# IamArmanNikkhah/viewport-entropy-toolkit

Measured on AMD Instinct MI355X. Metric: viewport samples/sec, higher is better.
Workload: dtype f64 (u32 block-floating-point table weights, u64 fixed-point histogram); 1 GPU; config3: 1 video(s) x 1024 users x 30000 frames, tile_counts=[500], spatial, use_weight_distribution=True, fov=120, W=100, H=200; users=1024, frames=30000, mode=spatial, videos_per_gpu=1, batched_launch=False, parallelism=one video per GPU x1

## Files before the change

include/vet.h:

```cpp
#ifndef VET_H_
#define VET_H_

#include <stddef.h>
#include <stdint.h>

#ifdef __cplusplus
extern "C" {
#endif

#define VET_VERSION 141
#define VET_STREAM_LEGACY ((void *)1)
#define VET_TABLE_SAMPLES_PER_DIRECTION 2

enum {
    VET_OK = 0,
    VET_ERR_INVALID = -1,
    VET_ERR_DEVICE = -2,
    VET_ERR_RANGE = -3,
    VET_ERR_EMPTY = -4,
    VET_ERR_UNSUPPORTED = -5
};

typedef struct vet_ctx vet_ctx;
typedef struct vet_plan vet_plan;

int vet_version(void);
const char *vet_last_error(void);
int vet_device_count(void);
int vet_create(int device_id, vet_ctx **out);
int vet_destroy(vet_ctx *ctx);
int vet_synchronize(vet_ctx *ctx);
int vet_device_pci_bus_id(vet_ctx *ctx, char *buf, int len);
int vet_profile_enable(vet_ctx *ctx, int on);
int vet_test_no_row_cap(vet_ctx *ctx, int on);
int vet_profile_reset(vet_ctx *ctx);
int vet_profile_get(vet_ctx *ctx, int kernel_id, double *total_ms, int64_t *launches);
const char *vet_kernel_name(int kernel_id);

int vet_malloc(vet_ctx *ctx, size_t bytes, void **d_ptr);
int vet_free(vet_ctx *ctx, void *d_ptr);
int vet_memcpy_h2d(vet_ctx *ctx, void *d_dst, const void *h_src, size_t bytes);
int vet_memcpy_d2h(vet_ctx *ctx, void *h_dst, const void *d_src, size_t bytes);

typedef struct vet_plan_desc {
    int video_width, video_height;
    const double *h_lon_cos, *h_lon_sin;
    const double *h_lat_sin, *h_lat_cos;
    const double *h_dir_table;
    int64_t n_dirs;
    int n_lattices;
    const int *n_tiles;
    const double *const *h_tiles;
    const double *h_max_entropy;
    double fov_angle;
    double max_angular_distance;
    double power_factor;
    int use_weight_distribution;
    const uint16_t *const *h_bin_lut;
    const int *n_norm_tiles;
} vet_plan_desc;

int vet_plan_create(vet_ctx *ctx, const vet_plan_desc *desc, vet_plan **out);
int vet_plan_destroy(vet_plan *plan);
int64_t vet_plan_n_dirs(const vet_plan *plan);
int vet_plan_set_table_policy(vet_plan *plan, int policy);
int vet_plan_set_fp64(vet_plan *plan, int on);
int vet_plan_set_raw_weights(vet_plan *plan, int on);
int vet_plan_table_stride(const vet_plan *plan, int lattice);
int64_t vet_plan_table_rows(const vet_plan *plan);
int vet_plan_table_cap(const vet_plan *plan, int lattice, int64_t *overflow_rows);
int vet_plan_last_formulation(const vet_plan *plan, int lattice);
int vet_plan_error_bounds(vet_plan *plan, int lattice, double *table_bound, double *sweep_bound);
int vet_plan_read_dirs(vet_plan *plan, double *h_xyz );
int vet_plan_read_nearest(vet_plan *plan, int lattice, int32_t *h_nearest );
int vet_plan_read_table(vet_plan *plan, int lattice, uint32_t *h_w, uint16_t *h_tile, uint32_t *h_meta, uint32_t *h_ovf_w,
                        uint16_t *h_ovf_tile, uint32_t *h_ovf_of_row);

int vet_spatial_entropy(vet_plan *plan, const double *d_mu, const double *d_mv,
                        int n_users, int n_frames,
                        double *d_entropy, int32_t *d_assign, double *d_weights,
                        int32_t *d_present, int32_t *d_status, void *stream);
int vet_spatial_entropy_ids(vet_plan *plan, const int32_t *d_ids, int n_users, int n_frames,
                            double *d_entropy, int32_t *d_assign, double *d_weights,
                            int32_t *d_present, int32_t *d_status, void *stream);

int64_t vet_window_rows(int n_frames, int window, int stride);
int vet_spatial_entropy_windowed(vet_plan *plan, const double *d_mu, const double *d_mv, int n_users, int n_frames,
                                 int window, int stride, double *d_entropy, double *d_weights, int32_t *d_samples,
                                 int32_t *d_status, void *stream);
int vet_spatial_entropy_windowed_ids(vet_plan *plan, const int32_t *d_ids, int n_users, int n_frames, int window, int stride,
                                     double *d_entropy, double *d_weights, int32_t *d_samples, int32_t *d_status,
                                     void *stream);
int vet_spatial_entropy_windowed_host(vet_plan *plan, const double *h_mu, const double *h_mv, const int32_t *h_ids,
                                      int n_users, int n_frames, int window, int stride, double *h_entropy,
                                      double *h_weights, int32_t *h_samples);

int vet_transition_entropy(vet_plan *plan, const double *d_mu, const double *d_mv,
                           int n_users, int n_frames,
                           double *d_entropy, int32_t *d_pairs, int32_t *d_srccount,
                           int32_t *d_common, int32_t *d_status, void *stream);
int vet_transition_entropy_ids(vet_plan *plan, const int32_t *d_ids, int n_users, int n_frames,
                               double *d_entropy, int32_t *d_pairs, int32_t *d_srccount,
                               int32_t *d_common, int32_t *d_status, void *stream);

typedef struct vet_video {
    const double *d_mu, *d_mv;
    int n_users, n_frames;
    double *d_entropy;
    int32_t *d_assign;
    int32_t *d_present;
} vet_video;
int vet_spatial_entropy_batch(vet_plan *plan, int n_videos, const vet_video *videos, int32_t *d_status,
                              void *stream);
int vet_spatial_entropy_batch_host(vet_plan *plan, int n_videos, const int *n_users, const int *n_frames,
                                   const double *h_mu, const double *h_mv, double *h_entropy,
                                   int32_t *h_assign, int32_t *h_present);
int vet_transition_entropy_batch(vet_plan *plan, int n_videos, const vet_video *videos, int32_t *d_status,
                                 void *stream);
int vet_transition_entropy_batch_host(vet_plan *plan, int n_videos, const int *n_users, const int *n_frames,
                                      const double *h_mu, const double *h_mv, double *h_entropy,
                                      int32_t *h_pairs, int32_t *h_common);

int vet_spatial_entropy_host(vet_plan *plan, const double *h_mu, const double *h_mv,
                             const int32_t *h_ids, int n_users, int n_frames,
                             double *h_entropy, int32_t *h_assign, double *h_weights,
                             int32_t *h_present);
int vet_transition_entropy_host(vet_plan *plan, const double *h_mu, const double *h_mv,
                                const int32_t *h_ids, int n_users, int n_frames,
                                double *h_entropy, int32_t *h_pairs, int32_t *h_srccount,
                                int32_t *h_common);

typedef struct vet_result vet_result;
int vet_spatial_entropy_host_resident(vet_plan *plan, const double *h_mu, const double *h_mv,
                                      const int32_t *h_ids, int n_users, int n_frames,
                                      double *h_entropy, int32_t *h_present, vet_result **out);
int vet_transition_entropy_host_resident(vet_plan *plan, const double *h_mu, const double *h_mv,
                                         const int32_t *h_ids, int n_users, int n_frames,
                                         double *h_entropy, int32_t *h_common, vet_result **out);
int vet_result_fetch(vet_result *result, int which, int64_t row0, int64_t n_rows, void *h_dst);
int vet_result_free(vet_result *result);

int vet_angular_distances(vet_ctx *ctx, const double *h_vectors, int64_t n_vectors, const double *h_tiles, int n_tiles,
                          double *h_out);

int vet_fb_tile_boundaries(vet_ctx *ctx, const double *h_tiles, int n_tiles, int max_edges,
                           double *h_edges, int32_t *h_count);

typedef struct vet_heatmap vet_heatmap;
int vet_heatmap_create(vet_ctx *ctx, const double *h_tiles , int n_tiles, int width,
                       int height, int video_width, int video_height, int marker_radius, vet_heatmap **out);
int vet_heatmap_destroy(vet_heatmap *hm);
int vet_heatmap_read_map(vet_heatmap *hm, int32_t *h_map );
int vet_heatmap_render(vet_heatmap *hm, const double *d_weights , const int32_t *d_present ,
                       const double *d_mu, const double *d_mv ,
                       int n_users, int n_frames, uint8_t *d_rgb , void *stream);
int vet_heatmap_render_result(vet_heatmap *hm, vet_result *r, const int32_t *h_present ,
                              const double *h_mu, const double *h_mv , int n_users,
                              int64_t row0, int64_t n_rows, uint8_t *h_rgb);
int vet_heatmap_render_counts(vet_heatmap *hm, const int32_t *d_counts , const int32_t *d_present ,
                              const double *d_mu, const double *d_mv ,
                              int n_users, int n_frames, uint8_t *d_rgb , void *stream);
int vet_heatmap_render_transition_result(vet_heatmap *hm, vet_result *r, const int32_t *h_present ,
                                         const double *h_mu, const double *h_mv , int n_users,
                                         int64_t row0, int64_t n_rows, uint8_t *h_rgb);
int vet_heatmap_create_latlon(vet_ctx *ctx, int tile_width, int tile_height, int width, int height, int video_width,
                              int video_height, int marker_radius, vet_heatmap **out);
int vet_heatmap_render_binned(vet_heatmap *hm, vet_plan *plan, const double *d_mu, const double *d_mv ,
                              int n_users, int n_frames, int markers, uint8_t *d_rgb , void *stream);
int vet_heatmap_render_binned_host(vet_heatmap *hm, vet_plan *plan, const double *h_mu, const double *h_mv ,
                                   int n_users, int n_frames, int markers, uint8_t *h_rgb );

typedef struct vet_tiling vet_tiling;
int vet_tiling_create(vet_ctx *ctx, const double *h_arcs , int n_arcs,
                      const double *h_centres , int n_centres, int width, int height,
                      vet_tiling **out);
int vet_tiling_destroy(vet_tiling *tl);
int vet_tiling_render(vet_tiling *tl, const double *h_cameras, int n_frames, const uint8_t *background, uint8_t *d_rgb,
                      void *stream);
int vet_tiling_render_host(vet_tiling *tl, const double *h_cameras, int n_frames, const uint8_t *background,
                           uint8_t *h_rgb);

#define VET_CSV_OK 0
#define VET_CSV_FALLBACK 1
#define VET_CSV_IO 2
typedef struct vet_track {
    double *time, *mu, *mv;
    int64_t n_rows;
    int status;
} vet_track;
int vet_csv_read_tracks(int n_files, const char *const *paths, vet_track *tracks, int n_threads);
void vet_csv_free_tracks(int n_files, vet_track *tracks);

#ifdef __cplusplus
}
#endif
#endif
```

viewport-entropy-toolkit_amd/csrc/vet_context.hip:

```cpp
#include "vet_host.hpp"
#include "vet_finalize.hpp"

#include <cstdarg>
#include <cstdio>
#include <cstdlib>
#include <cstring>

namespace vh {

namespace {
thread_local std::string g_err;
const char* const kKernelNames[KID_COUNT] = {"k_grid_dirs", "k_nearest_lut", "k_spatial", "k_transition",
                                             "k_finalize", "k_wtab", "k_weights"};

int env_flag(const char* name) { return getenv(name) ? 1 : 0; }
}

int fail(int code, const char* fmt, ...) {
    char buf[512];
    va_list ap;
    va_start(ap, fmt);
    vsnprintf(buf, sizeof buf, fmt, ap);
    va_end(ap);
    g_err = buf;
// ... 33 lines not shown
    HIP_TRY(hipMalloc(&c->ws, want));
    c->ws_bytes = want;
    return VET_OK;
}

int pooled(vet_ctx* c, int slot, size_t bytes, void** out) {
    if (bytes == 0) bytes = 8;
    if (c->pool_cap[slot] < bytes) {
        if (c->pool[slot]) {
            HIP_TRY(hipDeviceSynchronize());
            HIP_TRY(hipFree(c->pool[slot]));
        }
        c->pool[slot] = nullptr; c->pool_cap[slot] = 0;
        const size_t want = bytes + bytes / 8;
        HIP_TRY(hipMalloc(&c->pool[slot], want));
        c->pool_cap[slot] = want;
    }
    *out = c->pool[slot];
    return VET_OK;
}

int BatchBlob::acquire(vet_ctx* ctx, size_t nbytes) {
    c = ctx; bytes = nbytes ? nbytes : 8;
    BatchStage& t = c->stage[c->stage_next];
    c->stage_next = (c->stage_next + 1) % kBatchStages;
    if (t.pending) {
        HIP_TRY(hipEventSynchronize(t.done));
        t.pending = false;
    }
    if (!t.done) HIP_TRY(hipEventCreateWithFlags(&t.done, hipEventDisableTiming));
    if (t.cap < bytes) {
        if (t.h) { HIP_TRY(hipHostFree(t.h)); t.h = nullptr; }
        if (t.d) { HIP_TRY(hipFree(t.d)); t.d = nullptr; }
        t.cap = 0;
        const size_t want = bytes + bytes / 8;
        HIP_TRY(hipHostMalloc(&t.h, want, hipHostMallocDefault));
        HIP_TRY(hipMalloc(&t.d, want));
        t.cap = want;
    }
    st = &t;
    return VET_OK;
}

int BatchBlob::upload(hipStream_t stream) {
    s = stream;
    uploaded = true;
    HIP_TRY(hipMemcpyAsync(st->d, st->h, bytes, hipMemcpyHostToDevice, s));
    return VET_OK;
}

BatchBlob::~BatchBlob() {
    if (st && uploaded && hipEventRecord(st->done, s) == hipSuccess) st->pending = true;
}

int grid_for(long work, int block, int n_cu) {
    long b = (work + block - 1) / block;
    long cap = (long)n_cu * 8;
    if (b > cap) b = cap;
    if (b < 1) b = 1;
    return (int)b;
}

int check_run_args(const vet_plan* pl, int U, int T, const void* out) {
    if (!pl) return fail(VET_ERR_INVALID, "plan is NULL");
    if (U <= 0 || T <= 0) return fail(VET_ERR_INVALID, "n_users and n_frames must be positive (got %d, %d)", U, T);
    if (!out) return fail(VET_ERR_INVALID, "entropy output pointer is NULL");
    return VET_OK;
}

}

using namespace vh;

extern "C" {

int vet_version(void) { return VET_VERSION; }
const char* vet_last_error(void) { return vh::last_error(); }
const char* vet_kernel_name(int kid) { return (kid >= 0 && kid < KID_COUNT) ? kKernelNames[kid] : ""; }

int vet_device_count(void) {
    int n = 0;
    if (hipGetDeviceCount(&n) != hipSuccess) return 0;
    return n;
}

int vet_create(int device_id, vet_ctx** out) {
    if (!out) return fail(VET_ERR_INVALID, "out is NULL");
    int n = 0;
    hipError_t e = hipGetDeviceCount(&n);
    if (e != hipSuccess || n <= 0)
        return fail(VET_ERR_DEVICE, "no HIP device available (%s); this library has no CPU path",
                    e == hipSuccess ? "0 devices" : hipGetErrorString(e));
    if (device_id < 0 || device_id >= n) return fail(VET_ERR_INVALID, "device_id %d out of range [0,%d)", device_id, n);
    HIP_TRY(hipSetDevice(device_id));
    hipDeviceProp_t prop;
    HIP_TRY(hipGetDeviceProperties(&prop, device_id));
    vet_ctx* c = new vet_ctx();
    c->device = device_id;
    c->tune.from_environment();
    c->n_cu = prop.multiProcessorCount > 0 ? prop.multiProcessorCount : 256;
    c->lds_max = prop.sharedMemPerBlock >= 160 * 1024 ? 80 * 1024 : (size_t)prop.sharedMemPerBlock;
    e = hipStreamCreateWithFlags(&c->stream, hipStreamNonBlocking);
    if (e == hipSuccess) e = hipMalloc((void**)&c->d_log2, 4097 * sizeof(double));
    if (e == hipSuccess) {
        hipLaunchKernelGGL(vet::k_log2_table, dim3(17), dim3(256), 0, c->stream, c->d_log2, 4097);
        e = hipStreamSynchronize(c->stream);
    }
    if (e != hipSuccess) {
        if (c->d_log2) (void)hipFree(c->d_log2);
        if (c->stream) (void)hipStreamDestroy(c->stream);
        delete c;
        return fail(VET_ERR_DEVICE, "context set-up failed: %s", hipGetErrorString(e));
    }
    *out = c;
    return VET_OK;
}

int vet_device_pci_bus_id(vet_ctx* c, char* buf, int len) {
    if (!c || !buf || len < 16) return fail(VET_ERR_INVALID, "ctx or buf is NULL, or len < 16");
    HIP_TRY(hipDeviceGetPCIBusId(buf, len, c->device));
    return VET_OK;
}

int vet_destroy(vet_ctx* c) {
    if (!c) return VET_OK;
    (void)hipSetDevice(c->device);
    (void)hipStreamSynchronize(c->stream);
    for (auto& ep : c->pending) { (void)hipEventDestroy(ep.a); (void)hipEventDestroy(ep.b); }
    for (auto e : c->free_events) (void)hipEventDestroy(e);
    if (c->ws) (void)hipFree(c->ws);
    if (c->d_log2) (void)hipFree(c->d_log2);
    for (void* q : c->pool) if (q) (void)hipFree(q);
    for (auto& t : c->stage) {
        if (t.h) (void)hipHostFree(t.h);
        if (t.d) (void)hipFree(t.d);
        if (t.done) (void)hipEventDestroy(t.done);
    }
    (void)hipStreamDestroy(c->stream);
    delete c;
    return VET_OK;
}

int vet_synchronize(vet_ctx* c) {
    if (!c) return fail(VET_ERR_INVALID, "ctx is NULL");
    HIP_TRY(hipStreamSynchronize(c->stream));
    return VET_OK;
}

int vet_test_no_row_cap(vet_ctx* c, int on) {
    if (!c) return fail(VET_ERR_INVALID, "ctx is NULL");
    c->tune.no_row_cap = on != 0;
    return VET_OK;
}
int vet_profile_enable(vet_ctx* c, int on) {
    if (!c) return fail(VET_ERR_INVALID, "ctx is NULL");
    c->profiling = on != 0;
    return VET_OK;
}
int vet_profile_reset(vet_ctx* c) {
    if (!c) return fail(VET_ERR_INVALID, "ctx is NULL");
    int rc = collect_profile(c);
    if (rc) return rc;
    for (int i = 0; i < KID_COUNT; ++i) { c->prof_ms[i] = 0; c->prof_n[i] = 0; }
    return VET_OK;
}
int vet_profile_get(vet_ctx* c, int kid, double* total_ms, int64_t* launches) {
    if (!c || kid < 0 || kid >= KID_COUNT) return fail(VET_ERR_INVALID, "bad ctx or kernel id");
    int rc = collect_profile(c);
    if (rc) return rc;
    if (total_ms) *total_ms = c->prof_ms[kid];
    if (launches) *launches = c->prof_n[kid];
    return VET_OK;
}

int vet_malloc(vet_ctx* c, size_t bytes, void** d_ptr) {
    if (!c || !d_ptr) return fail(VET_ERR_INVALID, "ctx or d_ptr is NULL");
    HIP_TRY(hipSetDevice(c->device));
    HIP_TRY(hipMalloc(d_ptr, bytes ? bytes : 8));
    return VET_OK;
}
int vet_free(vet_ctx* c, void* d_ptr) {
    if (!c) return fail(VET_ERR_INVALID, "ctx is NULL");
    if (d_ptr) HIP_TRY(hipFree(d_ptr));
    return VET_OK;
}
int vet_memcpy_h2d(vet_ctx* c, void* d, const void* h, size_t bytes) {
    if (!c) return fail(VET_ERR_INVALID, "ctx is NULL");
    HIP_TRY(hipMemcpyAsync(d, h, bytes, hipMemcpyHostToDevice, c->stream));
    HIP_TRY(hipStreamSynchronize(c->stream));
    return VET_OK;
}
int vet_memcpy_d2h(vet_ctx* c, void* h, const void* d, size_t bytes) {
    if (!c) return fail(VET_ERR_INVALID, "ctx is NULL");
    HIP_TRY(hipMemcpyAsync(h, d, bytes, hipMemcpyDeviceToHost, c->stream));
    HIP_TRY(hipStreamSynchronize(c->stream));
    return VET_OK;
}

}
```

viewport-entropy-toolkit_amd/csrc/vet_host.hpp:

```cpp
#pragma once
#include "../../include/vet.h"
#include "vet_layout.hpp"

#include <hip/hip_runtime.h>

#include <cstdint>
#include <memory>
#include <string>
#include <vector>

namespace vh {

int fail(int code, const char* fmt, ...);
const char* last_error();

#define HIP_TRY(expr)                                                                             \
    do {                                                                                          \
        hipError_t e_ = (expr);                                                                   \
        if (e_ != hipSuccess)                                                                     \
            return vh::fail(VET_ERR_DEVICE, "%s failed: %s (%s:%d)", #expr, hipGetErrorString(e_), \
                            __FILE__, __LINE__);                                                  \
    } while (0)

struct DevBuf {
    void* p = nullptr;
    ~DevBuf() { if (p) (void)hipFree(p); }
    hipError_t alloc(size_t b) { return hipMalloc(&p, b ? b : 8); }
};

enum { KID_GRID = 0, KID_NEAREST = 1, KID_SPATIAL = 2, KID_TRANSITION = 3, KID_FINALIZE = 4, KID_WTAB = 5, KID_WEIGHTS = 6, KID_COUNT = 7 };

struct EventPair {
    int kid;
    hipEvent_t a, b;
};

struct WeightsCore {
    int device = 0;
    size_t lds_max = 64 * 1024;
    int n_cu = 256;
    std::shared_ptr<void> dir_unit;
    std::shared_ptr<void> tiles0;
    int n0 = 0;
    int64_t n_dirs = 0;
    double cos_cull = 0.0, max_ang = 0.0, power = 2.0;
    struct Exact {
        int state = 0;
        int stride = 0, n_rows = 0;
        std::shared_ptr<void> alias;
        std::shared_ptr<void> idx;
        std::shared_ptr<void> w;
        std::shared_ptr<void> len;
    } ex;
};

struct BatchStage {
    void* h = nullptr;
    void* d = nullptr;
    size_t cap = 0;
    hipEvent_t done = nullptr;
    bool pending = false;
};
constexpr int kBatchStages = 4;

struct Tuning {
    int no_fused = 0;
    int fused_single = 0;
    int t_global = 0;
    std::string lut_timeline;
    int no_exact_rows = 0;
    int no_row_cap = 0;
    void from_environment();
};

}

struct vet_ctx {
    int device = 0;
    hipStream_t stream = nullptr;
    int n_cu = 256;
    size_t lds_max = 64 * 1024;
    vh::Tuning tune;
    void* ws = nullptr;
    size_t ws_bytes = 0;
    double* d_log2 = nullptr;
    bool attrs_set = false;
    void* pool[12] = {};
    size_t pool_cap[12] = {};
    vh::BatchStage stage[vh::kBatchStages];
    int stage_next = 0;
    bool profiling = false;
    std::vector<vh::EventPair> pending;
    std::vector<hipEvent_t> free_events;
    double prof_ms[vh::KID_COUNT] = {};
    int64_t prof_n[vh::KID_COUNT] = {};
};

namespace vh {

struct Lattice {
    int n = 0;
    double* d_tiles = nullptr;
    std::vector<double> h_unit;
    uint16_t* d_nearest = nullptr;
    double hmax = 0.0;
    uint32_t* d_tab_w = nullptr;
    uint16_t* d_tab_i = nullptr;
    uint32_t* d_tab_meta = nullptr;
    uint8_t* d_row_s = nullptr;
    uint16_t* d_row_e = nullptr;
    bool fp_table = false;
    bool stats_done = false;
    double crit_tab = 0.0;
    double crit_base = 0.0;
    long ultra = 0;
    int markers = 0;
    int last_form = -1;
    int stride = 0;
    bool capped = false;
    int n_ovf = 0;
    uint32_t* d_ovf_w = nullptr;
    uint16_t* d_ovf_i = nullptr;
    uint32_t* d_ovf_of_row = nullptr;
    int gs_log2 = 4;
    bool interleaved = false;
    bool binned = false;
    int norm_n = 0;
    WeightsCore::Exact ex;
};

}

struct vet_plan {
    vet_ctx* ctx = nullptr;
    int W = 0, H = 0;
    bool grid = false;
    int64_t n_dirs = 0;
    double* d_dir_raw = nullptr;
    double* d_dir_unit = nullptr;
    std::vector<vh::Lattice> lat;
    double fov = 120.0, max_ang = 0.0, power = 2.0;
    int weighted = 1;
    double cos_cull = 0.0;
    int table_policy = 0;
    bool raw_weights = false;
    uint32_t* d_alias = nullptr;
    bool mirror = false;
    uint2* d_dirrec = nullptr;
    int n_rows = 0;
    int* d_canon = nullptr;
    struct Fused {
        int state = 0;
        int R = 0, stride = 0, gs_log2 = 4;
        bool interleaved = false;
        vet::FusedLayout lay;
        uint32_t* d_meta = nullptr;
        uint2* d_dirrec = nullptr;
        uint8_t* d_row_s = nullptr;
        uint32_t* d_w = nullptr;
        uint16_t* d_i = nullptr;
    } fused;
    std::shared_ptr<vh::WeightsCore> wcore;
    bool stats_all = false;
    bool ultra = false;
    bool fp64 = false;
    size_t exact_bytes = 0;
};

namespace vh {

struct ProfScope {
    vet_ctx* c;
    hipStream_t s;
    int kid;
    hipEvent_t a = nullptr, b = nullptr;
    ProfScope(vet_ctx* c_, hipStream_t s_, int kid_) : c(c_), s(s_), kid(kid_) {
        if (!c->profiling) return;
        auto get = [&]() {
            hipEvent_t e = nullptr;
            if (!c->free_events.empty()) { e = c->free_events.back(); c->free_events.pop_back(); }
            else (void)hipEventCreate(&e);
            return e;
        };
        a = get(); b = get();
        (void)hipEventRecord(a, s);
    }
    ~ProfScope() {
        if (!a) return;
        (void)hipEventRecord(b, s);
        c->pending.push_back({kid, a, b});
    }
};

struct BatchBlob {
    vet_ctx* c = nullptr;
    BatchStage* st = nullptr;
    hipStream_t s = nullptr;
    size_t bytes = 0;
    bool uploaded = false;
    int acquire(vet_ctx* ctx, size_t nbytes);
    void* host() const { return st->h; }
    void* dev() const { return st->d; }
    int upload(hipStream_t stream);
    ~BatchBlob();
};

int ensure_ws(vet_ctx* c, size_t bytes);
int pooled(vet_ctx* c, int slot, size_t bytes, void** out);
int grid_for(long work, int block, int n_cu);
int check_run_args(const vet_plan* pl, int U, int T, const void* out);

constexpr size_t kMaxTableBytes = (size_t)24 << 30;
constexpr double kContractMargin = 1e-7;
constexpr size_t kWholeLds = 160 * 1024 - 512;

int ensure_alias(vet_plan* pl);
int ensure_all_stats(vet_plan* pl, hipStream_t s);
int ensure_wtab(vet_plan* pl, int k, hipStream_t s);
int ensure_fused(vet_plan* pl, hipStream_t s);
bool any_binned(const vet_plan* pl);

int weights_pass_ids(const WeightsCore& w, const int32_t* d_ids, int U, int T, double* d_weights, hipStream_t s, vet_ctx* prof);
int ensure_exact_weights(vet_plan* pl, hipStream_t s);
int ensure_exact_rows(vet_plan* pl, int k, hipStream_t s);
const WeightsCore::Exact& exact_rows(const vet_plan* pl, int k);
int exact_frame_rows(vet_plan* pl, int k, const double* d_mu, const double* d_mv, const int32_t* d_ids, int U, int T, double* out,
                     hipStream_t s);
int sample_ids(const vet_plan* pl, const double* d_mu, const double* d_mv, long n, int32_t* d_out, hipStream_t s);

struct HeatmapGeom {
    const uint16_t* d_map = nullptr;
    int n = 0, W = 0, H = 0;
    int VW = 0, VH = 0, radius = 0;
};
int heatmap_map(vet_ctx* c, const double* d_unit_tiles, int n, int W, int H, uint16_t* d_map, hipStream_t s);
template <typename Wt>
int heatmap_render(vet_ctx* c, const HeatmapGeom& g, const Wt* d_weights, const int32_t* d_present, const double* d_mu,
                   const double* d_mv, int U, int T, uint32_t* d_pal, uint8_t* d_rgb, hipStream_t s);
struct BinLayout {
    bool ok = false, pack = false;
    int words = 0, FPW = 0;
    size_t lds = 0;
};
BinLayout heatmap_bin_layout(int n, int U);
int heatmap_map_latlon(vet_ctx* c, int tile_width, int tile_height, int W, int H, uint16_t* d_map, hipStream_t s);
int heatmap_bin_chunk(int n);
int heatmap_render_binned(vet_ctx* c, const HeatmapGeom& g, int n_lat, const uint16_t* d_lut, const double* d_mu,
                          const double* d_mv, int U, int T, bool markers, uint32_t* d_pal, uint8_t* d_rgb, hipStream_t s);

struct TilingCam {
    double F[3], r[3], u[3], nd[3];
    double s;
    double X0, Y0;
};
struct TilingGeom {
    const double* d_pts = nullptr;
    const double* d_centres = nullptr;
    long n_arcs = 0, n_centres = 0;
    int W = 0, H = 0;
    uint32_t colour[6] = {};
};
int tiling_chords(vet_ctx* c, const double* d_arcs, long n_arcs, double* d_pts, hipStream_t s);
int tiling_render(vet_ctx* c, const TilingGeom& g, const TilingCam* d_cam, int T, uint32_t* d_flags, uint8_t* d_rgb,
                  hipStream_t s);

int spatial_set_attrs(vet_ctx* c);
int transition_set_attrs(vet_ctx* c);
int window_set_attrs(vet_ctx* c);

}
```

viewport-entropy-toolkit_amd/csrc/vet_layout.hpp:

```cpp
#pragma once
#include <hip/hip_runtime.h>
#include <stdint.h>

namespace vet {

constexpr int WAVE = 64;
constexpr int MAX_LATTICES = 8;

constexpr int TAB_X = 16;
constexpr uint32_t MARKER_BITS = 0x80000000u;
constexpr int ROW_BITS = 19;
constexpr uint32_t ROW_MASK = (1u << ROW_BITS) - 1;
constexpr unsigned DEDUP_MAX_DIRS = (1u << ROW_BITS) - 1;
constexpr int DEDUP_MIN_USERS = 128;

constexpr int ROW_BLOCK = 64;
constexpr int MAX_CAP_BLOCKS = 3;
constexpr uint32_t META_OVERFLOW = 1u << 15;
constexpr uint32_t NO_OVERFLOW = 0xFFFFFFFFu;
__host__ __device__ __forceinline__ int lut_ovf_slots(int UC, int n_ovf, bool dedup) {
    if (n_ovf <= 0) return 0;
    const int most = dedup ? (2 * n_ovf > DEDUP_MIN_USERS ? 2 * n_ovf : DEDUP_MIN_USERS) : UC;
    return most < UC ? most : UC;
}

struct FusedLayout {
    int K;
    int n[MAX_LATTICES];
    int off[MAX_LATTICES];
    int Hs, N;
    int CF;
    double hmax[MAX_LATTICES];
};
__host__ __device__ __forceinline__ int fused_pos(const FusedLayout& L, int k, int i) {
    const int h = L.n[k] >> 1;
    if (i < h) return L.off[k] + i;
    if (i >= L.n[k] - h) return L.N - 1 - (L.off[k] + (L.n[k] - 1 - i));
    return 2 * L.K + L.Hs + k;
}

}
```

viewport-entropy-toolkit_amd/csrc/vet_plan.hip:

```cpp
#include "vet_host.hpp"
#include "vet_plan_kernels.hpp"
#include "vet_weight_table.hpp"
#include "vet_geometry.hpp"

#include <algorithm>
#include <array>
#include <cmath>
#include <cstring>
#include <limits>

namespace vh {

int ensure_alias(vet_plan* pl) {
    if (pl->d_alias) return VET_OK;
    vet_ctx* c = pl->ctx;
    const long D = (long)pl->n_dirs;
    if (D <= 0 || D >= (long)0x7FFFFFFF) return fail(VET_ERR_UNSUPPORTED, "direction table of %ld entries", D);
    bool mirror = pl->weighted;
    for (const auto& L : pl->lat) {
        if (L.binned || L.h_unit.empty()) { mirror = false; break; }
        for (int i = 0; i < L.n && mirror; ++i) {
            const double* a = &L.h_unit[3 * (size_t)i];
            const double* b = &L.h_unit[3 * (size_t)(L.n - 1 - i)];
            mirror = a[0] == b[0] && a[1] == -b[1] && a[2] == -b[2];
// ... 61 lines not shown
        (void)hipFree(d_crit);
        return fail(VET_ERR_DEVICE, "hipMalloc of the row shift table failed");
    }
    hipError_t e = hipMemsetAsync(d_crit, 0, 24, s);
    vet::StatsParams p{};
    p.dir_unit = pl->d_dir_unit; p.D = (long)pl->n_dirs;
    p.tiles = L.d_tiles; p.n = L.n;
    p.cos_cull = pl->cos_cull;
    p.wc.max_ang = pl->max_ang; p.wc.inv_max = 1.0 / pl->max_ang; p.wc.power = pl->power; p.wc.shift = 0;
    p.row_s = L.d_row_s; p.row_e = L.d_row_e; p.crit = d_crit;
    const int blocks = grid_for((long)pl->n_dirs * vet::WAVE, 256, c->n_cu * 2);
    {
        ProfScope ps(c, s, KID_WTAB);
        hipLaunchKernelGGL(vet::k_row_stats, dim3(blocks), dim3(256), 0, s, p);
    }
    unsigned long long bits[3] = {0, 0, 0};
    if (e == hipSuccess) e = hipMemcpyAsync(bits, d_crit, 24, hipMemcpyDeviceToHost, s);
    if (e == hipSuccess) e = hipStreamSynchronize(s);
    (void)hipFree(d_crit);
    if (e != hipSuccess) return fail(VET_ERR_DEVICE, "k_row_stats failed: %s", hipGetErrorString(e));
    memcpy(&L.crit_tab, &bits[0], 8);
    memcpy(&L.crit_base, &bits[1], 8);
    L.ultra = (long)bits[2];
    L.stats_done = true;
    return VET_OK;
}

int ensure_all_stats(vet_plan* pl, hipStream_t s) {
    if (pl->stats_all) return VET_OK;
    bool ultra = false;
    for (int k = 0; k < (int)pl->lat.size(); ++k) {
        if (!pl->weighted || pl->lat[k].binned) continue;
        int rc = ensure_stats(pl, k, s);
        if (rc) return rc;
        ultra = ultra || pl->lat[k].ultra > 0;
    }
    pl->ultra = ultra;
    pl->stats_all = true;
    return VET_OK;
}

int ensure_wtab(vet_plan* pl, int k, hipStream_t s) {
    Lattice& L = pl->lat[k];
    if (L.stride != 0) return VET_OK;
    vet_ctx* c = pl->ctx;
    int rc = ensure_all_stats(pl, s);
    if (rc) return rc;
    rc = ensure_alias(pl);
    if (rc) return rc;
    int* d_max = nullptr;
    HIP_TRY(hipMalloc((void**)&d_max, 2 * sizeof(int)));
    struct FreeMax { int* p; ~FreeMax() { (void)hipFree(p); } } free_max{d_max};
    hipError_t e = hipMemsetAsync(d_max, 0, 2 * sizeof(int), s);
    vet::WtabParams p{};
    const long R = pl->n_rows;
    p.dir_unit = pl->d_dir_unit; p.D = R;
    p.canon = pl->d_canon; p.shift_by_dir = 1; p.nl = 0;
    p.tiles = L.d_tiles; p.n = L.n;
    p.cos_cull = pl->cos_cull;
    p.wc.max_ang = pl->max_ang; p.wc.inv_max = 1.0 / pl->max_ang; p.wc.power = pl->power; p.wc.shift = 0;
    L.fp_table = pl->ultra || !(L.crit_tab <= kContractMargin);
    p.stride = 0; p.w = nullptr; p.idx = nullptr; p.meta = nullptr; p.row_s = L.d_row_s; p.row_e = L.d_row_e; p.fp = L.fp_table ? 1 : 0;
    p.maxcount = d_max; p.markers = nullptr; p.gs_log2 = -1;
    const int blocks = grid_for(R * vet::WAVE, 256, c->n_cu * 2);
    {
        ProfScope ps(c, s, KID_WTAB);
        hipLaunchKernelGGL(vet::k_wtab<false>, dim3(blocks), dim3(256), 0, s, p);
    }
    int longest = 0;
    if (e == hipSuccess) e = hipMemcpyAsync(&longest, d_max, sizeof(int), hipMemcpyDeviceToHost, s);
    if (e == hipSuccess) e = hipStreamSynchronize(s);
    if (e != hipSuccess) return fail(VET_ERR_DEVICE, "k_wtab<count> failed: %s", hipGetErrorString(e));
    int stride = ((longest > 0 ? longest : 1) + 63) / 64 * 64;
    const size_t rows = (size_t)R + 1;
    int cap = stride, n_ovf = 0;
    std::vector<uint32_t> ovf_of_row;
    if (!L.fp_table && pl->lat.size() == 1 && stride > vet::ROW_BLOCK && 4 * longest >= 3 * 64 && !c->tune.no_row_cap) {
        DevBuf d_len;
        HIP_TRY(d_len.alloc((size_t)R * sizeof(int)));
        p.row_len = (int*)d_len.p; p.gs_log2 = -1;
        {
            ProfScope ps(c, s, KID_WTAB);
            hipLaunchKernelGGL(vet::k_wtab<true>, dim3(blocks), dim3(256), 0, s, p);
        }
        std::vector<int> len((size_t)R);
        HIP_TRY(hipMemcpyAsync(len.data(), d_len.p, (size_t)R * sizeof(int), hipMemcpyDeviceToHost, s));
        HIP_TRY(hipStreamSynchronize(s));
        p.row_len = nullptr;
        int shortest = stride, most = 0;
        for (int v : len) { shortest = std::min(shortest, v); most = std::max(most, v); }
        for (int cnd = vet::ROW_BLOCK; cnd < stride && cnd <= vet::MAX_CAP_BLOCKS * vet::ROW_BLOCK; cnd += vet::ROW_BLOCK) {
            long longer = 0;
            for (int v : len) longer += v > cnd ? 1 : 0;
            if (longer * 32 > R) continue;
            if (shortest > cnd - vet::ROW_BLOCK && most <= cnd + vet::ROW_BLOCK) {
                cap = cnd;
                ovf_of_row.assign((size_t)R, vet::NO_OVERFLOW);
                for (long r = 0; r < R; ++r)
                    if (len[(size_t)r] > cap) ovf_of_row[(size_t)r] = (uint32_t)n_ovf++;
            }
            break;
        }
    }
    const bool capped = cap < stride;
    stride = cap;
    const size_t ovf_rows = capped ? (size_t)n_ovf + 1 : 0;
    const size_t bytes = rows * stride * 6 + rows * 4 + ovf_rows * vet::ROW_BLOCK * 6 + (capped ? (size_t)R * 4 : 0);
    size_t free_b = 0, total_b = 0;
    if (hipMemGetInfo(&free_b, &total_b) != hipSuccess) free_b = kMaxTableBytes;
    if (stride > 65535 || bytes > kMaxTableBytes || rows * (size_t)stride >= ((size_t)1 << 32) || bytes + ((size_t)64 << 20) > free_b) { L.stride = -1; return VET_OK; }
    auto drop = [&]() {
        if (L.d_tab_w) { (void)hipFree(L.d_tab_w); L.d_tab_w = nullptr; }
        if (L.d_tab_i) { (void)hipFree(L.d_tab_i); L.d_tab_i = nullptr; }
        if (L.d_tab_meta) { (void)hipFree(L.d_tab_meta); L.d_tab_meta = nullptr; }
        if (L.d_ovf_w) { (void)hipFree(L.d_ovf_w); L.d_ovf_w = nullptr; }
        if (L.d_ovf_i) { (void)hipFree(L.d_ovf_i); L.d_ovf_i = nullptr; }
        if (L.d_ovf_of_row) { (void)hipFree(L.d_ovf_of_row); L.d_ovf_of_row = nullptr; }
    };
    drop();
    if (hipMalloc((void**)&L.d_tab_w, rows * stride * 4) != hipSuccess ||
        hipMalloc((void**)&L.d_tab_i, rows * stride * 2) != hipSuccess ||
        hipMalloc((void**)&L.d_tab_meta, rows * 4) != hipSuccess ||
        (capped && (hipMalloc((void**)&L.d_ovf_w, ovf_rows * vet::ROW_BLOCK * 4) != hipSuccess ||
                    hipMalloc((void**)&L.d_ovf_i, ovf_rows * vet::ROW_BLOCK * 2) != hipSuccess ||
                    hipMalloc((void**)&L.d_ovf_of_row, (size_t)R * 4) != hipSuccess))) {
        (void)hipGetLastError();
        drop();
        L.stride = -1;
        return VET_OK;
    }
    struct DropOnError { decltype(drop)& d; bool armed = true; ~DropOnError() { if (armed) d(); } } guard{drop};
    L.gs_log2 = 1;
    while (L.gs_log2 < 4 && (4 << L.gs_log2) < longest) ++L.gs_log2;
    L.interleaved = L.gs_log2 == 4 && stride % 64 == 0 && 4 * longest >= 3 * 64;
    if (capped) {
        HIP_TRY(hipMemcpyAsync(L.d_ovf_of_row, ovf_of_row.data(), (size_t)R * 4, hipMemcpyHostToDevice, s));
        p.cap = cap; p.ovf_of_row = L.d_ovf_of_row; p.ow = L.d_ovf_w; p.oi = L.d_ovf_i; p.n_ovf = n_ovf;
    }
    p.stride = stride; p.w = L.d_tab_w; p.idx = L.d_tab_i; p.meta = L.d_tab_meta; p.maxcount = nullptr;
    p.markers = L.fp_table ? d_max + 1 : nullptr;
    p.gs_log2 = L.interleaved ? L.gs_log2 : -1;
    {
        ProfScope ps(c, s, KID_WTAB);
        hipLaunchKernelGGL(vet::k_wtab<true>, dim3(blocks), dim3(256), 0, s, p);
    }
    HIP_TRY(hipGetLastError());
    if (k == 0 && (uint64_t)pl->n_rows <= vet::DEDUP_MAX_DIRS) {
        if (!pl->d_dirrec) HIP_TRY(hipMalloc((void**)&pl->d_dirrec, (size_t)pl->n_dirs * sizeof(uint2)));
        ProfScope ps(c, s, KID_WTAB);
        hipLaunchKernelGGL(vet::k_dirrec, dim3(grid_for(pl->n_dirs, 256, c->n_cu)), dim3(256), 0, s, pl->d_alias,
                           L.d_nearest, L.d_tab_meta, (long)pl->n_dirs, pl->d_dirrec);
        HIP_TRY(hipGetLastError());
    }
    int markers = 0;
    HIP_TRY(hipMemcpyAsync(&markers, d_max + 1, sizeof(int), hipMemcpyDeviceToHost, s));
    HIP_TRY(hipStreamSynchronize(s));
    guard.armed = false;
    L.markers = markers;
    L.capped = capped; L.n_ovf = capped ? n_ovf : 0;
    L.stride = stride;
    return VET_OK;
}

int ensure_exact_rows(vet_plan* pl, int k, hipStream_t s) {
    WeightsCore::Exact& X = k == 0 ? pl->wcore->ex : pl->lat[k].ex;
    if (X.state != 0) return VET_OK;
    vet_ctx* c = pl->ctx;
    const Lattice& L = pl->lat[k];
    if (!pl->weighted || L.binned || !L.d_tiles || c->tune.no_exact_rows) { X.state = -1; return VET_OK; }
    int rc = ensure_alias(pl);
    if (rc) return rc;
    const long R = pl->n_rows;
    if (R <= 0) { X.state = -1; return VET_OK; }
    DevBuf d_max;
    HIP_TRY(d_max.alloc(sizeof(int)));
    HIP_TRY(hipMemsetAsync(d_max.p, 0, sizeof(int), s));
    vet::WtabParams p{};
    p.dir_unit = pl->d_dir_unit; p.D = R;
    p.canon = pl->d_canon; p.shift_by_dir = 1; p.nl = 0;
    p.tiles = L.d_tiles; p.n = L.n;
    p.cos_cull = pl->cos_cull;
    p.wc.max_ang = pl->max_ang; p.wc.inv_max = 1.0 / pl->max_ang; p.wc.power = pl->power; p.wc.shift = 0;
    p.maxcount = (int*)d_max.p; p.gs_log2 = -1;
    const int blocks = grid_for(R * vet::WAVE, 256, c->n_cu * 2);
    hipLaunchKernelGGL(vet::k_wtab<false>, dim3(blocks), dim3(256), 0, s, p);
    HIP_TRY(hipGetLastError());
    int longest = 0;
    HIP_TRY(hipMemcpyAsync(&longest, d_max.p, sizeof(int), hipMemcpyDeviceToHost, s));
    HIP_TRY(hipStreamSynchronize(s));
    const int stride = ((longest > 0 ? longest : 1) + 63) / 64 * 64;
    const size_t D = k == 0 ? (size_t)pl->n_dirs : 0, entries = (size_t)R * stride, bytes = entries * 10 + (size_t)R * 4 + D * 4;
    size_t free_b = 0, total_b = 0;
    if (hipMemGetInfo(&free_b, &total_b) != hipSuccess) free_b = 0;
    const size_t total = pl->exact_bytes + bytes;
    if (total > ((size_t)8 << 30) || total > (free_b + pl->exact_bytes) / 4 || stride > 65535) { X.state = -1; return VET_OK; }
    auto dev_free = [](void* q) { if (q) (void)hipFree(q); };
    auto dev_alloc = [&](size_t b) {
        void* q = nullptr;
        if (hipMalloc(&q, b ? b : 8) != hipSuccess) { (void)hipGetLastError(); q = nullptr; }
        return std::shared_ptr<void>(q, dev_free);
    };
    auto alias = k == 0 ? dev_alloc(D * 4) : std::shared_ptr<void>();
    auto idx = dev_alloc(entries * 2), w = dev_alloc(entries * 8), len = dev_alloc((size_t)R * 4);
    if ((k == 0 && !alias) || !idx || !w || !len) { X.state = -1; return VET_OK; }
    if (k == 0) HIP_TRY(hipMemcpyAsync(alias.get(), pl->d_alias, D * 4, hipMemcpyDeviceToDevice, s));
    vet::WexactParams q{};
    q.dir_unit = pl->d_dir_unit; q.canon = pl->d_canon; q.R = R; q.tiles = L.d_tiles; q.n = L.n;
    q.cos_cull = pl->cos_cull; q.wc = p.wc; q.stride = stride;
    q.idx = (uint16_t*)idx.get(); q.w = (double*)w.get(); q.len = (uint32_t*)len.get();
    {
        ProfScope ps(c, s, KID_WTAB);
        hipLaunchKernelGGL(vet::k_wexact, dim3(blocks), dim3(256), 0, s, q);
    }
    HIP_TRY(hipGetLastError());
    HIP_TRY(hipStreamSynchronize(s));
    X.alias = alias; X.idx = idx; X.w = w; X.len = len;
    X.stride = stride; X.n_rows = (int)R;
    X.state = 1;
    pl->exact_bytes = total;
    return VET_OK;
}

int ensure_exact_weights(vet_plan* pl, hipStream_t s) { return ensure_exact_rows(pl, 0, s); }

const WeightsCore::Exact& exact_rows(const vet_plan* pl, int k) { return k == 0 ? pl->wcore->ex : pl->lat[k].ex; }

bool any_binned(const vet_plan* pl) {
    for (const auto& L : pl->lat) if (L.binned) return true;
    return false;
}

int ensure_fused(vet_plan* pl, hipStream_t s) {
    auto& F = pl->fused;
    if (F.state != 0) return VET_OK;
    vet_ctx* c = pl->ctx;
    const int K = (int)pl->lat.size();
    auto unusable = [&]() { F.state = -1; return VET_OK; };
    if (K == 1 && !c->tune.fused_single) return unusable();
    if (!pl->weighted || K > vet::MAX_LATTICES || any_binned(pl) || c->tune.no_fused) return unusable();
    if ((uint64_t)pl->n_dirs > vet::DEDUP_MAX_DIRS) return unusable();
    int rc = ensure_all_stats(pl, s);
    if (rc) return rc;
    if (pl->ultra) return unusable();
    for (const auto& L : pl->lat)
        if (!(L.crit_tab <= kContractMargin) || !L.d_row_s) return unusable();
    rc = ensure_alias(pl);
    if (rc) return rc;
    const size_t D = (size_t)pl->n_dirs;
    const int R = pl->n_rows;
    if (R == 0) return unusable();
    vet::FusedLayout& lay = F.lay;
    lay.K = K; lay.Hs = 0; lay.CF = 0;
    for (int k = 0; k < K; ++k) {
        lay.n[k] = pl->lat[k].n; lay.off[k] = 2 * K + lay.Hs; lay.Hs += pl->lat[k].n >> 1; lay.hmax[k] = pl->lat[k].hmax;
        lay.CF += (pl->lat[k].n + vet::WAVE - 1) / vet::WAVE;
    }
    lay.N = 2 * (lay.Hs + K) + 4 * K;
    if (lay.N > 65535 || lay.N < 32) return unusable();

    auto drop = [&]() {
        for (void** q : {(void**)&F.d_row_s, (void**)&F.d_w, (void**)&F.d_i, (void**)&F.d_meta, (void**)&F.d_dirrec})
            if (*q) { (void)hipFree(*q); *q = nullptr; }
    };
    struct DropOnExit { decltype(drop)& d; bool armed = true; ~DropOnExit() { if (armed) d(); } } guard{drop};
    DevBuf ptrs_d, delta_d, max_d;
    HIP_TRY(ptrs_d.alloc(sizeof(void*) * vet::MAX_LATTICES));
    HIP_TRY(delta_d.alloc(sizeof(int) * vet::MAX_LATTICES));
    HIP_TRY(max_d.alloc(sizeof(int)));
    HIP_TRY(hipMalloc((void**)&F.d_row_s, (size_t)R + 1));
    const uint8_t* ptrs[vet::MAX_LATTICES] = {};
    for (int k = 0; k < K; ++k) ptrs[k] = pl->lat[k].d_row_s;
    HIP_TRY(hipMemcpyAsync(ptrs_d.p, ptrs, sizeof(ptrs), hipMemcpyHostToDevice, s));
    HIP_TRY(hipMemsetAsync(delta_d.p, 0, sizeof(int) * vet::MAX_LATTICES, s));
    HIP_TRY(hipMemsetAsync(max_d.p, 0, sizeof(int), s));
    HIP_TRY(hipMemsetAsync(F.d_row_s + R, vet::TAB_X, 1, s));
    hipLaunchKernelGGL(vet::k_fuse_shifts, dim3(grid_for(R, 256, c->n_cu)), dim3(256), 0, s, (const int*)pl->d_canon, R, K,
                       (const uint8_t* const*)ptrs_d.p, F.d_row_s, (int*)delta_d.p);
    vet::WtabParams p{};
    p.dir_unit = pl->d_dir_unit; p.D = R;
    p.tiles = nullptr; p.n = 0;
    p.cos_cull = pl->cos_cull;
    p.wc.max_ang = pl->max_ang; p.wc.inv_max = 1.0 / pl->max_ang; p.wc.power = pl->power; p.wc.shift = 0;
    p.stride = 0; p.w = nullptr; p.idx = nullptr; p.meta = nullptr; p.row_s = F.d_row_s; p.row_e = nullptr; p.fp = 0;
    p.markers = nullptr; p.maxcount = (int*)max_d.p; p.gs_log2 = -1;
    p.canon = pl->d_canon; p.shift_by_dir = 0; p.nl = K; p.Hs = lay.Hs; p.N = lay.N;
    for (int k = 0; k < 8; ++k) { p.tiles_v[k] = k < K ? pl->lat[k].d_tiles : nullptr; p.n_v[k] = k < K ? lay.n[k] : 0; p.off_v[k] = k < K ? lay.off[k] : 0; }
    const int blocks = grid_for((long)R * vet::WAVE, 256, c->n_cu * 2);
    {
        ProfScope ps(c, s, KID_WTAB);
        hipLaunchKernelGGL(vet::k_wtab<false>, dim3(blocks), dim3(256), 0, s, p);
    }
    int longest = 0, delta[vet::MAX_LATTICES] = {};
    HIP_TRY(hipMemcpyAsync(&longest, max_d.p, sizeof(int), hipMemcpyDeviceToHost, s));
    HIP_TRY(hipMemcpyAsync(delta, delta_d.p, sizeof(delta), hipMemcpyDeviceToHost, s));
    HIP_TRY(hipStreamSynchronize(s));
    for (int k = 0; k < K; ++k) {
        if (delta[k] == 0) continue;
        DevBuf crit;
        HIP_TRY(crit.alloc(24));
        HIP_TRY(hipMemsetAsync(crit.p, 0, 24, s));
        vet::StatsParams sp{};
        sp.dir_unit = pl->d_dir_unit; sp.D = R;
        sp.tiles = pl->lat[k].d_tiles; sp.n = pl->lat[k].n;
        sp.cos_cull = pl->cos_cull;
        sp.wc.max_ang = pl->max_ang; sp.wc.inv_max = 1.0 / pl->max_ang; sp.wc.power = pl->power; sp.wc.shift = 0;
        sp.row_s = nullptr; sp.row_e = nullptr; sp.crit = (unsigned long long*)crit.p;
        sp.canon = pl->d_canon; sp.shift_in = F.d_row_s;
        hipLaunchKernelGGL(vet::k_row_stats, dim3(grid_for((long)R * vet::WAVE, 256, c->n_cu * 2)), dim3(256), 0, s, sp);
        unsigned long long bits = 0;
// ... 45 lines not shown

extern "C" {

int vet_plan_create(vet_ctx* c, const vet_plan_desc* d, vet_plan** out) {
    if (!c || !d || !out) return fail(VET_ERR_INVALID, "ctx, desc or out is NULL");
    const bool grid = d->h_lon_cos && d->h_lon_sin && d->h_lat_sin && d->h_lat_cos;
    if (!grid && !(d->h_dir_table && d->n_dirs > 0))
        return fail(VET_ERR_INVALID, "plan needs the four axis tables or an explicit direction table");
    if (grid && (d->video_width <= 0 || d->video_height <= 0))
        return fail(VET_ERR_INVALID, "Video dimensions must be positive");
    if (d->n_lattices <= 0 || !d->n_tiles || !d->h_tiles || !d->h_max_entropy)
        return fail(VET_ERR_INVALID, "Must specify at least one tile count");
    if (!(d->fov_angle > 0.0 && d->fov_angle <= 360.0))
        return fail(VET_ERR_INVALID, "FOV angle must be between 0 and 360 degrees");
    if (!(d->power_factor > 0.0)) return fail(VET_ERR_INVALID, "Power factor must be positive");
    for (int k = 0; k < d->n_lattices; ++k) {
        const bool binned = d->h_bin_lut && d->h_bin_lut[k];
        if (d->n_tiles[k] <= 0 || d->n_tiles[k] > 65535 || (!binned && !d->h_tiles[k]))
            return fail(VET_ERR_INVALID, "lattice %d: tile count %d outside [1, 65535]", k, d->n_tiles[k]);
    }
    HIP_TRY(hipSetDevice(c->device));
    hipStream_t s = c->stream;
    vet_plan* pl = new vet_plan();
    pl->ctx = c;
    pl->grid = grid;
    pl->W = d->video_width; pl->H = d->video_height;
    pl->fov = d->fov_angle; pl->max_ang = d->max_angular_distance; pl->power = d->power_factor;
    pl->weighted = d->use_weight_distribution ? 1 : 0;
    pl->cos_cull = pl->max_ang >= 3.14159 ? -2.0 : std::cos(pl->max_ang) - 1e-9;
    pl->n_dirs = grid ? (int64_t)(pl->W + 1) * (pl->H + 1) : d->n_dirs;
    if (pl->n_dirs >= (1LL << 31)) { delete pl; return fail(VET_ERR_UNSUPPORTED, "direction table too large"); }

    auto cleanup = [&](int rc) { vet_plan_destroy(pl); return rc; };
#define PLAN_TRY(expr)                                                                           \
    do {                                                                                         \
        hipError_t e_ = (expr);                                                                  \
        if (e_ != hipSuccess)                                                                    \
            return cleanup(fail(VET_ERR_DEVICE, "%s failed: %s", #expr, hipGetErrorString(e_))); \
    } while (0)

    PLAN_TRY(hipMalloc((void**)&pl->d_dir_raw, (size_t)pl->n_dirs * 3 * sizeof(double)));
    PLAN_TRY(hipMalloc((void**)&pl->d_dir_unit, (size_t)pl->n_dirs * 3 * sizeof(double)));
    if (grid) {
        const size_t nw = (size_t)pl->W + 1, nh = (size_t)pl->H + 1;
        double* d_axes = nullptr;
        PLAN_TRY(hipMalloc((void**)&d_axes, (2 * nw + 2 * nh) * sizeof(double)));
        hipError_t e1 = hipMemcpyAsync(d_axes, d->h_lon_cos, nw * 8, hipMemcpyHostToDevice, s);
        hipError_t e2 = hipMemcpyAsync(d_axes + nw, d->h_lon_sin, nw * 8, hipMemcpyHostToDevice, s);
        hipError_t e3 = hipMemcpyAsync(d_axes + 2 * nw, d->h_lat_sin, nh * 8, hipMemcpyHostToDevice, s);
        hipError_t e4 = hipMemcpyAsync(d_axes + 2 * nw + nh, d->h_lat_cos, nh * 8, hipMemcpyHostToDevice, s);
        if (e1 || e2 || e3 || e4) { (void)hipFree(d_axes); return cleanup(fail(VET_ERR_DEVICE, "axis table upload failed")); }
        {
            ProfScope ps(c, s, KID_GRID);
            hipLaunchKernelGGL(vet::k_grid_dirs, dim3(grid_for(pl->n_dirs, 256, c->n_cu)), dim3(256), 0, s, d_axes,
                               d_axes + nw, d_axes + 2 * nw, d_axes + 2 * nw + nh, pl->W, pl->H, pl->d_dir_raw,
                               pl->d_dir_unit);
        }
        hipError_t e5 = hipStreamSynchronize(s);
        (void)hipFree(d_axes);
        if (e5 != hipSuccess) return cleanup(fail(VET_ERR_DEVICE, "k_grid_dirs failed: %s", hipGetErrorString(e5)));
    } else {
        PLAN_TRY(hipMemcpyAsync(pl->d_dir_raw, d->h_dir_table, (size_t)pl->n_dirs * 24, hipMemcpyHostToDevice, s));
        hipLaunchKernelGGL(vet::k_unit_dirs, dim3(grid_for(pl->n_dirs, 256, c->n_cu)), dim3(256), 0, s, pl->d_dir_raw,
                           (long)pl->n_dirs, pl->d_dir_unit);
        PLAN_TRY(hipStreamSynchronize(s));
    }
    pl->lat.resize(d->n_lattices);
    for (int k = 0; k < d->n_lattices; ++k) {
        Lattice& L = pl->lat[k];
        L.n = d->n_tiles[k];
        L.hmax = d->h_max_entropy[k];
        L.norm_n = d->n_norm_tiles ? d->n_norm_tiles[k] : L.n;
        if (d->h_bin_lut && d->h_bin_lut[k]) {
            L.binned = true;
            for (int64_t i = 0; i < pl->n_dirs; ++i)
                if (d->h_bin_lut[k][i] >= L.n)
                    return cleanup(fail(VET_ERR_INVALID, "lattice %d: bin %u of direction %lld >= %d bins", k,
                                        (unsigned)d->h_bin_lut[k][i], (long long)i, L.n));
            PLAN_TRY(hipMalloc((void**)&L.d_nearest, ((size_t)pl->n_dirs + 1) * sizeof(uint16_t)));
            PLAN_TRY(hipMemsetAsync(L.d_nearest + pl->n_dirs, 0, sizeof(uint16_t), s));
            PLAN_TRY(hipMemcpyAsync(L.d_nearest, d->h_bin_lut[k], (size_t)pl->n_dirs * sizeof(uint16_t),
                                    hipMemcpyHostToDevice, s));
            PLAN_TRY(hipStreamSynchronize(s));
            continue;
        }
        std::vector<double> unit((size_t)L.n * 3);
        for (int t = 0; t < L.n; ++t) {
            const double x = d->h_tiles[k][3 * t], y = d->h_tiles[k][3 * t + 1], z = d->h_tiles[k][3 * t + 2];
            const double len = std::sqrt(x * x + y * y + z * z);
            if (!(len > 0.0)) return cleanup(fail(VET_ERR_INVALID, "Vector cannot have zero length (lattice %d tile %d)", k, t));
            unit[3 * t] = x / len; unit[3 * t + 1] = y / len; unit[3 * t + 2] = z / len;
        }
        PLAN_TRY(hipMalloc((void**)&L.d_tiles, unit.size() * sizeof(double)));
        PLAN_TRY(hipMalloc((void**)&L.d_nearest, ((size_t)pl->n_dirs + 1) * sizeof(uint16_t)));
        PLAN_TRY(hipMemsetAsync(L.d_nearest + pl->n_dirs, 0, sizeof(uint16_t), s));
        PLAN_TRY(hipMemcpyAsync(L.d_tiles, unit.data(), unit.size() * sizeof(double), hipMemcpyHostToDevice, s));
        PLAN_TRY(hipStreamSynchronize(s));
        L.h_unit = unit;
        const size_t lds = (size_t)L.n * 3 * sizeof(double);
        if (lds > 160 * 1024 - 1024) return cleanup(fail(VET_ERR_UNSUPPORTED, "lattice of %d tiles exceeds the LDS tile cache", L.n));
        if (lds > 64 * 1024)
            PLAN_TRY(hipFuncSetAttribute((const void*)vet::k_nearest_lut, hipFuncAttributeMaxDynamicSharedMemorySize, (int)lds));
        {
            ProfScope ps(c, s, KID_NEAREST);
            hipLaunchKernelGGL(vet::k_nearest_lut, dim3(grid_for(pl->n_dirs, 64, c->n_cu * 4)), dim3(64), lds, s,
                               pl->d_dir_unit, (long)pl->n_dirs, L.d_tiles, L.n, L.d_nearest);
        }
        PLAN_TRY(hipGetLastError());
    }
    PLAN_TRY(hipStreamSynchronize(s));
    if (!c->attrs_set) {
        int rc = spatial_set_attrs(c);
        if (!rc) rc = transition_set_attrs(c);
        if (!rc) rc = window_set_attrs(c);
        if (rc) return cleanup(rc);
        c->attrs_set = true;
    }
#undef PLAN_TRY
    {
        auto dev_free = [](void* q) { if (q) (void)hipFree(q); };
        pl->wcore = std::make_shared<vh::WeightsCore>();
        vh::WeightsCore& w = *pl->wcore;
        w.device = c->device; w.lds_max = c->lds_max; w.n_cu = c->n_cu;
        w.dir_unit = std::shared_ptr<void>((void*)pl->d_dir_unit, dev_free);
        if (pl->lat[0].d_tiles) w.tiles0 = std::shared_ptr<void>((void*)pl->lat[0].d_tiles, dev_free);
        w.n0 = pl->lat[0].n; w.n_dirs = pl->n_dirs;
        w.cos_cull = pl->cos_cull; w.max_ang = pl->max_ang; w.power = pl->power;
    }
    *out = pl;
    return VET_OK;
}

int vet_plan_destroy(vet_plan* pl) {
    if (!pl) return VET_OK;
    (void)hipSetDevice(pl->ctx->device);
    (void)hipStreamSynchronize(pl->ctx->stream);
    if (pl->d_dir_raw) (void)hipFree(pl->d_dir_raw);
    if (pl->d_dir_unit && !(pl->wcore && pl->wcore->dir_unit)) (void)hipFree(pl->d_dir_unit);
    for (auto& L : pl->lat) {
        if (L.d_tiles && !(&L == &pl->lat[0] && pl->wcore && pl->wcore->tiles0)) (void)hipFree(L.d_tiles);
        if (L.d_nearest) (void)hipFree(L.d_nearest);
        if (L.d_tab_w) (void)hipFree(L.d_tab_w);
        if (L.d_tab_i) (void)hipFree(L.d_tab_i);
        if (L.d_tab_meta) (void)hipFree(L.d_tab_meta);
        if (L.d_ovf_w) (void)hipFree(L.d_ovf_w);
        if (L.d_ovf_i) (void)hipFree(L.d_ovf_i);
        if (L.d_ovf_of_row) (void)hipFree(L.d_ovf_of_row);
        if (L.d_row_s) (void)hipFree(L.d_row_s);
        if (L.d_row_e) (void)hipFree(L.d_row_e);
    }
    if (pl->d_alias) (void)hipFree(pl->d_alias);
    if (pl->d_canon) (void)hipFree(pl->d_canon);
    if (pl->d_dirrec) (void)hipFree(pl->d_dirrec);
    {
        auto& F = pl->fused;
        for (void* q : {(void*)F.d_row_s, (void*)F.d_w, (void*)F.d_i, (void*)F.d_meta, (void*)F.d_dirrec})
            if (q) (void)hipFree(q);
    }
    delete pl;
    return VET_OK;
}

int64_t vet_plan_n_dirs(const vet_plan* pl) { return pl ? pl->n_dirs : 0; }

int vet_plan_set_table_policy(vet_plan* pl, int policy) {
    if (!pl) return fail(VET_ERR_INVALID, "plan is NULL");
    pl->table_policy = policy > 0 ? 1 : (policy < 0 ? -1 : 0);
    return VET_OK;
}

int vet_plan_set_fp64(vet_plan* pl, int on) {
    if (!pl) return fail(VET_ERR_INVALID, "plan is NULL");
    pl->fp64 = on != 0;
    return VET_OK;
}

int vet_plan_set_raw_weights(vet_plan* pl, int on) {
    if (!pl) return fail(VET_ERR_INVALID, "plan is NULL");
    pl->raw_weights = on != 0;
    return VET_OK;
}

int64_t vet_plan_table_rows(const vet_plan* pl) { return pl ? pl->n_rows : 0; }

int vet_plan_table_stride(const vet_plan* pl, int k) {
    if (!pl || k < 0 || k >= (int)pl->lat.size()) return 0;
    if (pl->lat[k].stride == 0 && pl->fused.state == 1) return pl->fused.stride;
    return pl->lat[k].stride;
}

int vet_plan_table_cap(const vet_plan* pl, int k, int64_t* overflow_rows) {
    if (overflow_rows) *overflow_rows = 0;
    if (!pl || k < 0 || k >= (int)pl->lat.size() || pl->lat[k].stride <= 0) return 0;
    if (overflow_rows) *overflow_rows = pl->lat[k].n_ovf;
    return pl->lat[k].stride;
}

int vet_plan_read_table(vet_plan* pl, int k, uint32_t* h_w, uint16_t* h_tile, uint32_t* h_meta, uint32_t* h_ovf_w,
                        uint16_t* h_ovf_tile, uint32_t* h_ovf_of_row) {
    if (!pl) return fail(VET_ERR_INVALID, "plan is NULL");
    if (k < 0 || k >= (int)pl->lat.size()) return fail(VET_ERR_INVALID, "lattice index %d out of range", k);
    const vh::Lattice& L = pl->lat[k];
    if (L.stride <= 0) return fail(VET_ERR_INVALID, "lattice %d has no table of its own", k);
    HIP_TRY(hipSetDevice(pl->ctx->device));
    const size_t rows = (size_t)pl->n_rows + 1, ovf = (size_t)L.n_ovf + 1;
    if (h_w) HIP_TRY(hipMemcpy(h_w, L.d_tab_w, rows * L.stride * 4, hipMemcpyDeviceToHost));
    if (h_tile) HIP_TRY(hipMemcpy(h_tile, L.d_tab_i, rows * L.stride * 2, hipMemcpyDeviceToHost));
    if (h_meta) HIP_TRY(hipMemcpy(h_meta, L.d_tab_meta, rows * 4, hipMemcpyDeviceToHost));
    if ((h_ovf_w || h_ovf_tile || h_ovf_of_row) && !L.capped) return fail(VET_ERR_INVALID, "lattice %d has no overflow table", k);
    if (h_ovf_w) HIP_TRY(hipMemcpy(h_ovf_w, L.d_ovf_w, ovf * vet::ROW_BLOCK * 4, hipMemcpyDeviceToHost));
    if (h_ovf_tile) HIP_TRY(hipMemcpy(h_ovf_tile, L.d_ovf_i, ovf * vet::ROW_BLOCK * 2, hipMemcpyDeviceToHost));
    if (h_ovf_of_row) HIP_TRY(hipMemcpy(h_ovf_of_row, L.d_ovf_of_row, (size_t)pl->n_rows * 4, hipMemcpyDeviceToHost));
    return VET_OK;
}

int vet_angular_distances(vet_ctx* c, const double* h_vectors, int64_t m, const double* h_tiles, int n, double* h_out) {
    if (!c || !h_vectors || !h_tiles || !h_out) return fail(VET_ERR_INVALID, "ctx, vectors, tiles or output is NULL");
    if (m <= 0 || n <= 0) return fail(VET_ERR_INVALID, "need m > 0 vectors and n > 0 tile centres");
    HIP_TRY(hipSetDevice(c->device));
    hipStream_t s = c->stream;
    DevBuf vecs, tiles, out;
    HIP_TRY(vecs.alloc((size_t)m * 24));
    HIP_TRY(tiles.alloc((size_t)n * 24));
    HIP_TRY(out.alloc((size_t)m * n * 8));
    HIP_TRY(hipMemcpyAsync(vecs.p, h_vectors, (size_t)m * 24, hipMemcpyHostToDevice, s));
    HIP_TRY(hipMemcpyAsync(tiles.p, h_tiles, (size_t)n * 24, hipMemcpyHostToDevice, s));
    hipLaunchKernelGGL(vet::k_angular_distances, dim3(grid_for((long)m * n, 256, c->n_cu)), dim3(256), 0, s, (const double*)vecs.p,
                       (long)m, (const double*)tiles.p, n, (double*)out.p);
    HIP_TRY(hipGetLastError());
    HIP_TRY(hipMemcpyAsync(h_out, out.p, (size_t)m * n * 8, hipMemcpyDeviceToHost, s));
    HIP_TRY(hipStreamSynchronize(s));
    return VET_OK;
}

int vet_fb_tile_boundaries(vet_ctx* c, const double* h_tiles, int n, int max_edges, double* h_edges, int32_t* h_count) {
    if (!c || !h_tiles || !h_edges || !h_count) return fail(VET_ERR_INVALID, "ctx, tiles or an output is NULL");
    if (n <= 0 || max_edges <= 0) return fail(VET_ERR_INVALID, "need n > 0 tiles and max_edges > 0");
    HIP_TRY(hipSetDevice(c->device));
    hipStream_t s = c->stream;
    const size_t eb = (size_t)n * max_edges * 6 * sizeof(double);
    DevBuf tiles, edges, count, err;
    HIP_TRY(tiles.alloc((size_t)n * 24));
    HIP_TRY(edges.alloc(eb));
    HIP_TRY(count.alloc((size_t)n * 4));
    HIP_TRY(err.alloc(4));
    HIP_TRY(hipMemcpyAsync(tiles.p, h_tiles, (size_t)n * 24, hipMemcpyHostToDevice, s));
    HIP_TRY(hipMemsetAsync(edges.p, 0xFF, eb, s));
    HIP_TRY(hipMemsetAsync(err.p, 0, 4, s));
    hipLaunchKernelGGL(vet::k_fb_boundaries, dim3((n + 63) / 64), dim3(64), 0, s, (const double*)tiles.p, n, max_edges,
                       (double*)edges.p, (int32_t*)count.p, (int32_t*)err.p);
    HIP_TRY(hipGetLastError());
    int32_t bad = 0;
    HIP_TRY(hipMemcpyAsync(h_edges, edges.p, eb, hipMemcpyDeviceToHost, s));
    HIP_TRY(hipMemcpyAsync(h_count, count.p, (size_t)n * 4, hipMemcpyDeviceToHost, s));
    HIP_TRY(hipMemcpyAsync(&bad, err.p, 4, hipMemcpyDeviceToHost, s));
    HIP_TRY(hipStreamSynchronize(s));
    if (bad) return fail(VET_ERR_UNSUPPORTED, "%d tile(s) with more than %d neighbours or more than %d edges", bad,
                         vet::FB_MAX_NEIGHBOURS, max_edges);
    return VET_OK;
}

int vet_plan_last_formulation(const vet_plan* pl, int k) {
    if (!pl || k < 0 || k >= (int)pl->lat.size()) return -1;
    return pl->lat[k].last_form;
}

int vet_plan_error_bounds(vet_plan* pl, int k, double* table_bound, double* sweep_bound) {
    if (!pl) return fail(VET_ERR_INVALID, "plan is NULL");
    if (k < 0 || k >= (int)pl->lat.size()) return fail(VET_ERR_INVALID, "lattice index %d out of range", k);
    if (pl->lat[k].binned) return fail(VET_ERR_INVALID, "lattice %d is binned (integer counts, exact)", k);
    HIP_TRY(hipSetDevice(pl->ctx->device));
    int rc = ensure_all_stats(pl, pl->ctx->stream);
    if (rc) return rc;
    const double inf = std::numeric_limits<double>::infinity();
    if (table_bound) *table_bound = pl->ultra ? inf : pl->lat[k].crit_tab;
    if (sweep_bound) *sweep_bound = pl->ultra ? inf : pl->lat[k].crit_base * std::ldexp(1.0, -52);
    return VET_OK;
}

int vet_plan_read_dirs(vet_plan* pl, double* h_xyz) {
    if (!pl || !h_xyz) return fail(VET_ERR_INVALID, "plan or output is NULL");
    HIP_TRY(hipMemcpy(h_xyz, pl->d_dir_raw, (size_t)pl->n_dirs * 24, hipMemcpyDeviceToHost));
    return VET_OK;
}

int vet_plan_read_nearest(vet_plan* pl, int k, int32_t* h_nearest) {
    if (!pl || !h_nearest) return fail(VET_ERR_INVALID, "plan or output is NULL");
    if (k < 0 || k >= (int)pl->lat.size()) return fail(VET_ERR_INVALID, "lattice index %d out of range", k);
    std::vector<uint16_t> tmp((size_t)pl->n_dirs);
    HIP_TRY(hipMemcpy(tmp.data(), pl->lat[k].d_nearest, tmp.size() * 2, hipMemcpyDeviceToHost));
    for (size_t i = 0; i < tmp.size(); ++i) h_nearest[i] = tmp[i];
    return VET_OK;
}

}
```

viewport-entropy-toolkit_amd/csrc/vet_spatial.hip:

```cpp
#include "vet_host.hpp"
#include "vet_finalize.hpp"
#include "vet_spatial_sweep.hpp"
#include "vet_weights_pass.hpp"
#include "vet_spatial_dtable.hpp"
#include "vet_spatial_lut.hpp"
#include "vet_spatial_u.hpp"

#include <algorithm>
#include <cmath>
#include <cstring>

namespace vh {

namespace {

struct Geometry {
    int NW, FPW, G, UC, R;
    size_t lds;
};

int sweep_geometry(size_t lds_max, int n, int U, Geometry* g, bool one_frame = false) {
    g->R = n > vet::WAVE ? 2 : 1;
    g->G = (n + vet::WAVE * g->R - 1) / (vet::WAVE * g->R);
    if (g->G >= 4) { g->NW = g->G > 16 ? 16 : g->G; g->FPW = 1; }
    else { g->NW = 4; g->FPW = 4 / g->G; }
    if (one_frame) g->FPW = 1;
    g->UC = U < 1024 ? U : 1024;
    auto lds_of = [&](int fpw, int uc) {
        size_t b = (size_t)fpw * n * 8;
        b += (size_t)fpw * uc * 24;
        b += (size_t)g->NW * vet::WAVE * (g->R + 1) * (8 + 2);
        b += (size_t)2 * fpw * 4 + 64;
        return b;
    };
    while (lds_of(g->FPW, g->UC) > lds_max && g->FPW > 1) g->FPW /= 2;
    while (lds_of(g->FPW, g->UC) > lds_max && g->UC > 64) g->UC /= 2;
    g->lds = lds_of(g->FPW, g->UC);
    if (g->lds > lds_max)
        return fail(VET_ERR_UNSUPPORTED, "lattice of %d tiles does not fit the LDS histogram (%zu B)", n, g->lds);
    return VET_OK;
}

int spatial_geometry(const vet_ctx* c, int n, int U, bool weighted, Geometry* g, bool one_frame = false) {
    if (!weighted) {
        g->R = 1; g->G = 1; g->UC = 0;
        g->NW = 4;
        g->FPW = U >= 2048 ? 2 : (U >= 512 ? 4 : (U >= 128 ? 8 : 32));
        while ((size_t)g->FPW * n * 4 > c->lds_max && g->FPW > 1) g->FPW /= 2;
        g->lds = (size_t)g->FPW * n * 4;
        if (g->lds > c->lds_max)
            return fail(VET_ERR_UNSUPPORTED, "lattice of %d tiles does not fit the LDS histogram (%zu B)", n, g->lds);
        return VET_OK;
    }
    return sweep_geometry(c->lds_max, n, U, g, one_frame);
}

constexpr int kULdsThreads = 1024;
size_t u_lds_bytes(const vet_plan* pl, int U, int n, int fb) {
    return (((size_t)pl->n_dirs * 2 + 15) & ~(size_t)15) + (size_t)(U + 1) * 8 +
           ((((size_t)fb * n + 1) & ~(size_t)1) * 4) + (size_t)fb * (kULdsThreads / 64) * 8 + fb * 4 + 16;
}
int u_lds_frames(const vet_plan* pl, int U, int n, int fb) {
    while (fb > 1 && u_lds_bytes(pl, U, n, fb) > pl->ctx->lds_max) fb /= 2;
    return fb;
}
long u_lds_grid(const vet_ctx* c, long n_blocks) {
    long grid = (long)c->n_cu * 2;
    if (grid > n_blocks) grid = n_blocks;
    const long rounds = (n_blocks + grid - 1) / grid;
    return (n_blocks + rounds - 1) / rounds;
}

int weight_mode(const vet_plan* pl) {
    const bool fast_acos = pl->max_ang <= 1.0471975511965979;
    if (fast_acos && pl->power == 2.0) return 1;
    if (fast_acos && pl->power == 1.0) return 2;
    return 0;
}

template <bool FROM_IDS>
const void* spatial_w_kernel(int wmode, int R, bool precise = false) {
    if (precise) return R == 1 ? (const void*)vet::k_spatial_w<FROM_IDS, 0, 1, true> : (const void*)vet::k_spatial_w<FROM_IDS, 0, 2, true>;
#define VET_PICK(W, RR) if (wmode == W && R == RR) return (const void*)vet::k_spatial_w<FROM_IDS, W, RR, false>
    VET_PICK(0, 1); VET_PICK(0, 2); VET_PICK(1, 1); VET_PICK(1, 2); VET_PICK(2, 1); VET_PICK(2, 2);
#undef VET_PICK
    return nullptr;
}

template <bool FROM_IDS>
const void* lut_kernel_fused(bool il, bool occ8, bool dedup, bool narrow = false) {
    if (narrow) {
#define VET_PICKN(I, O, D) if (il == I && occ8 == O && dedup == D) return (const void*)vet::k_spatial_lut<FROM_IDS, 2, I, O, D, false, true>
        VET_PICKN(false, false, false); VET_PICKN(false, false, true); VET_PICKN(false, true, true);
        VET_PICKN(true, false, false); VET_PICKN(true, false, true); VET_PICKN(true, true, true);
#undef VET_PICKN
        return nullptr;
    }
    if (occ8) return nullptr;
#define VET_PICK(I, D) if (il == I && dedup == D) return (const void*)vet::k_spatial_lut<FROM_IDS, 4, I, false, D, false, true>
    VET_PICK(false, false); VET_PICK(true, false); VET_PICK(false, true); VET_PICK(true, true);
#undef VET_PICK
    return nullptr;
}

template <bool FROM_IDS>
const void* lut_kernel(bool il, bool occ8, bool dedup, bool fpt = false, int nb = 0) {
    if (nb) {
        if (!il || !occ8 || fpt) return nullptr;
#define VET_PICKC(N, D) if (nb == N && dedup == D) return (const void*)vet::k_spatial_lut<FROM_IDS, 2, true, true, D, false, false, N>
        VET_PICKC(1, false); VET_PICKC(1, true); VET_PICKC(2, false); VET_PICKC(2, true); VET_PICKC(3, false); VET_PICKC(3, true);
#undef VET_PICKC
        static_assert(vet::MAX_CAP_BLOCKS == 3, "one fixed-trip kernel per block count");
        return nullptr;
    }
    if (fpt) {
#define VET_PICKF(I, D) if (il == I && dedup == D) return (const void*)vet::k_spatial_lut<FROM_IDS, 2, I, false, D, true>
        VET_PICKF(false, false); VET_PICKF(true, false); VET_PICKF(false, true); VET_PICKF(true, true);
#undef VET_PICKF
        return nullptr;
    }
#define VET_PICK(I, O, D) if (il == I && occ8 == O && dedup == D) return (const void*)vet::k_spatial_lut<FROM_IDS, 2, I, O, D, false>
    VET_PICK(false, false, false); VET_PICK(false, true, false); VET_PICK(true, false, false); VET_PICK(true, true, false);
    VET_PICK(false, false, true); VET_PICK(false, true, true); VET_PICK(true, false, true); VET_PICK(true, true, true);
#undef VET_PICK
    return nullptr;
}

int lut_frames_per_wg(int U, long total_frames, int n_cu, int n_sum) {
    long f = 1024 / (U > 0 ? U : 1);
    const long by_grid = total_frames / (4L * n_cu);
    if (f > by_grid) f = by_grid;
    if (f > 4) f = 4;
    int fpw = 1;
    while (2 * fpw <= f) fpw *= 2;
    while (fpw > 1 && (size_t)fpw * n_sum * 8 > 20 * 1024) fpw /= 2;
    const long slots = 8L * n_cu;
    auto cost = [&](int f) { const long wgs = (total_frames + f - 1) / f; return (double)((wgs + slots - 1) / slots) * (f + 0.6); };
    for (int f = fpw / 2; f >= 1; f /= 2)
        if (cost(f) < cost(fpw)) fpw = f;
    return fpw;
}

enum { F_TABLE = 0, F_SWEEP = 1, F_PRECISE = 2, F_FTABLE = 3, F_DTABLE = 4 };

bool table_requested(const vet_plan* pl, long samples, int U) {
    if (!pl->weighted || pl->table_policy < 0 || any_binned(pl) || U >= 65536) return false;
    if ((int)pl->lat.size() > vet::MAX_LATTICES) return false;
    return pl->table_policy > 0 || samples >= (long)VET_TABLE_SAMPLES_PER_DIRECTION * (long)pl->n_dirs;
}

int sweep_shift(int U) {
    int ubits = 0;
    while ((1L << ubits) < (long)U) ++ubits;
    return ubits > 10 ? ubits - 10 : 0;
}

int sweep_formulation(const vet_plan* pl, const Lattice& L, int U) {
    if (pl->ultra) return F_PRECISE;
    double step = std::ldexp(1.0, sweep_shift(U) - 52);
    if (weight_mode(pl) != 0 && step < 4e-14) step = 4e-14;
    return L.crit_base * step <= kContractMargin ? F_SWEEP : F_PRECISE;
}

int weights_nw(size_t lds_max, int n) {
    int nw = 4;
    while (nw > 1 && (size_t)nw * n * 8 > lds_max) nw /= 2;
    return nw;
}

int fp64_formulation(vet_plan* pl, int k, bool want_table, hipStream_t s, int* out) {
    *out = F_PRECISE;
    if (!want_table) return VET_OK;
    int rc = ensure_exact_rows(pl, k, s);
    if (rc) return rc;
    const int n = pl->lat[k].n;
    if (exact_rows(pl, k).state == 1 && vet::dtable_lds_bytes(weights_nw(pl->ctx->lds_max, n), n) <= pl->ctx->lds_max)
        *out = F_DTABLE;
    return VET_OK;
}

template <bool FROM_IDS>
int launch_dtable(vet_plan* pl, const int* lat_idx, int K, int nw, const vet::SampleSrc& src, int U, int T, double* d_mean,
                  double* d_ent_k, int32_t* d_assign, double* d_weights, int32_t* d_present, int32_t* d_status, hipStream_t s) {
    vet_ctx* c = pl->ctx;
    if (T <= 0) return VET_OK;
    vet::DtableParams q{};
    q.src = src; q.U = U; q.T = T;
    q.alias = pl->d_alias; q.nearest = pl->lat[0].d_nearest;
    q.K = K; q.n_sum = 0;
    int max_stride = 0;
    auto chunk_class = [](int stride) { const int c = stride / vet::WAVE; return c <= 1 ? 1 : c <= 2 ? 2 : c <= 4 ? 4 : 0; };
    for (int j = 0; j < K; ++j) {
        const Lattice& L = pl->lat[lat_idx[j]];
        const WeightsCore::Exact& X = exact_rows(pl, lat_idx[j]);
        q.off[j] = q.n_sum; q.hmax[j] = L.hmax; q.chunk[j] = chunk_class(X.stride);
        q.lat[j] = vet::ExactRows{(const uint16_t*)X.idx.get(), (const double*)X.w.get(), (const uint32_t*)X.len.get(), X.stride, L.n};
        q.n_sum += L.n;
        max_stride = std::max(max_stride, X.stride);
    }
    q.entropy = d_mean; q.ent_k = d_ent_k;
    const bool first = lat_idx[0] == 0;
    q.assign = first ? d_assign : nullptr; q.weights = first ? d_weights : nullptr;
    q.present = first ? d_present : nullptr; q.status = first ? d_status : nullptr;
    const size_t lds = vet::dtable_lds_bytes(nw, q.n_sum);
    if (lds > c->lds_max) return fail(VET_ERR_UNSUPPORTED, "dtable: %zu B of LDS", lds);
    const int cls = chunk_class(max_stride);
    const void* fn = cls == 1 ? (const void*)vet::k_spatial_dtable<FROM_IDS, 1>
                   : cls == 2 ? (const void*)vet::k_spatial_dtable<FROM_IDS, 2>
                   : cls == 4 ? (const void*)vet::k_spatial_dtable<FROM_IDS, 4> : (const void*)vet::k_spatial_dtable<FROM_IDS, 0>;
    void* args[] = {(void*)&q};
    ProfScope ps(c, s, KID_SPATIAL);
    HIP_TRY(hipLaunchKernel(fn, dim3((unsigned)T), dim3(nw * vet::WAVE), args, lds, s));
    HIP_TRY(hipGetLastError());
    return VET_OK;
}

int choose_formulation(vet_plan* pl, int k, bool want_table, int U, hipStream_t s, int* out) {
    Lattice& L = pl->lat[k];
    int rc = ensure_all_stats(pl, s);
    if (rc) return rc;
    if (want_table) {
        rc = ensure_wtab(pl, k, s);
        if (rc) return rc;
        if (L.stride > 0) { *out = L.fp_table ? F_FTABLE : F_TABLE; return VET_OK; }
    }
    *out = sweep_formulation(pl, L, U);
    return VET_OK;
}

bool dedup_fused(int users) { return users >= vet::DEDUP_MIN_USERS; }
bool dedup_lattices(const vet_plan* pl, int users) {
    return (uint64_t)pl->n_rows <= vet::DEDUP_MAX_DIRS && pl->d_dirrec && dedup_fused(users);
}

template <bool FROM_IDS>
int launch_lut(vet_plan* pl, const int* lat_idx, int K, const vet::SampleSrc& src, int U, int T,
               const vet::VideoDesc* d_videos, int n_videos, int blocks_batch, size_t lds_batch, int batch_max_users,
               double* d_entropy, int32_t* d_assign, double* d_weights, int32_t* d_present, int32_t* d_status,
               hipStream_t s, bool* launched, uint32_t* d_resolve = nullptr) {
    vet_ctx* c = pl->ctx;
    *launched = false;
    vet::LutParams q{};
    q.resolve = d_resolve;
    q.dedup_min_users = vet::DEDUP_MIN_USERS;
    q.videos = d_videos; q.n_videos = n_videos;
    q.src = src; q.U = U; q.T = T;
    q.nearest = pl->lat[lat_idx[0]].d_nearest;
    q.alias = pl->d_alias;
    q.dirrec = pl->d_dirrec;
    q.rec_meta = lat_idx[0] == 0 ? 1 : 0;
    q.K = K; q.n_sum = 0;
    bool il = false;
    const bool fpt = pl->lat[lat_idx[0]].fp_table;
    for (int k = 0; k < K; ++k) {
        const Lattice& L = pl->lat[lat_idx[k]];
        q.lat[k].tab_w = L.d_tab_w; q.lat[k].tab_i = L.d_tab_i; q.lat[k].tab_meta = L.d_tab_meta;
        q.lat[k].stride = L.stride;
        q.lat[k].gs_log2 = L.gs_log2; q.lat[k].interleaved = L.interleaved ? 1 : 0;
        q.lat[k].n = L.n; q.lat[k].hmax = L.hmax;
        q.lat[k].zrow = (uint32_t)pl->n_rows;
        q.lat[k].ovf_w = L.d_ovf_w; q.lat[k].ovf_i = L.d_ovf_i; q.lat[k].ovf_of_row = L.d_ovf_of_row; q.lat[k].n_ovf = L.n_ovf;
        q.n_sum += L.n;
        il = il || L.interleaved;
    }
    const Lattice& L0 = pl->lat[lat_idx[0]];
    const int nb = L0.capped ? L0.stride / vet::ROW_BLOCK : 0;
    if (nb && (K != 1 || lat_idx[0] != 0)) return fail(VET_ERR_UNSUPPORTED, "capped rows in a launch of several lattices");
    q.entropy = d_entropy; q.assign = d_assign; q.weights = d_weights; q.present = d_present;
    q.status = d_status;
    const bool dedup = dedup_lattices(pl, d_videos ? batch_max_users : U);
    int blocks = blocks_batch;
    const int threads = 256;
    size_t lds = lds_batch;
    bool occ8 = true;
    q.sort_words = (fpt && dedup && 2 * pl->n_rows <= 65536) ? (int)((2 * pl->n_rows + 31) / 32) : 0;
    if (!d_videos) {
        q.UC = U < 2048 ? U : 2048;
        int fpw = lut_frames_per_wg(U, T, c->n_cu, q.n_sum);
        for (;; fpw /= 2) {
            lds = vet::lut_lds_bytes(U, q.UC, fpw, q.n_sum, dedup, d_resolve != nullptr, fpt ? threads / 64 : 1, q.sort_words,
                                     nb ? vet::lut_ovf_slots(q.UC, L0.n_ovf, dedup) : 0);
            if (lds <= c->lds_max || fpw == 1) break;
        }
        if (lds > c->lds_max) return VET_OK;
        q.FPW = fpw;
        blocks = (T + fpw - 1) / fpw;
        occ8 = K == 1;
    } else {
        q.FPW = 1; q.UC = 1;
    }
    ProfScope ps(c, s, KID_SPATIAL);
    void* args[] = {(void*)&q};
    const void* fn = lut_kernel<FROM_IDS>(il, occ8 && !fpt, dedup, fpt, nb);
    if (!fn) return fail(VET_ERR_UNSUPPORTED, "no table kernel for this launch");
    HIP_TRY(hipLaunchKernel(fn, dim3((unsigned)blocks), dim3(threads), args, lds, s));
    HIP_TRY(hipGetLastError());
    *launched = true;
    return VET_OK;
}

template <bool FROM_IDS>
int launch_lut_fused(vet_plan* pl, const vet::SampleSrc& src, int U, int T, const vet::VideoDesc* d_videos, int n_videos,
                     int blocks_batch, size_t lds_batch, int batch_max_users, double* d_entropy, int32_t* d_assign,
                     double* d_weights, int32_t* d_present, int32_t* d_status, hipStream_t s, bool* launched) {
    vet_ctx* c = pl->ctx;
    const auto& F = pl->fused;
    *launched = false;
    vet::LutParams q{};
    q.dedup_min_users = vet::DEDUP_MIN_USERS;
    q.videos = d_videos; q.n_videos = n_videos;
    q.src = src; q.U = U; q.T = T;
    q.nearest = pl->lat[0].d_nearest; q.alias = nullptr; q.dirrec = F.d_dirrec; q.rec_meta = 1;
    q.K = 1; q.n_sum = F.lay.N;
    q.lat[0].tab_w = F.d_w; q.lat[0].tab_i = F.d_i; q.lat[0].tab_meta = F.d_meta;
    q.lat[0].stride = F.stride; q.lat[0].gs_log2 = F.gs_log2; q.lat[0].interleaved = F.interleaved ? 1 : 0;
    q.lat[0].n = F.lay.N; q.lat[0].hmax = 0.0; q.lat[0].zrow = (uint32_t)F.R;
    q.lay = F.lay;
    q.entropy = d_entropy; q.assign = d_assign; q.weights = d_weights; q.present = d_present; q.status = d_status;
    const bool dedup = dedup_fused(d_videos ? batch_max_users : U);
    int blocks = blocks_batch, threads = 256;
    size_t lds = lds_batch;
    if (!d_videos) {
        q.UC = U < 2048 ? U : 2048;
        int fpw = lut_frames_per_wg(U, T, c->n_cu, q.n_sum);
        for (;; fpw /= 2) {
            lds = vet::lut_lds_bytes(U, q.UC, fpw, q.n_sum, dedup);
            if (lds <= c->lds_max || fpw == 1) break;
        }
        if (lds > c->lds_max) return VET_OK;
        q.FPW = fpw;
        blocks = (T + fpw - 1) / fpw;
    } else {
        q.FPW = 1; q.UC = 1;
    }
    const bool occ8 = F.gs_log2 == 3 && !d_videos && dedup;
#if VET_STAGE_CYCLES
    DevBuf dbg, tl;
    HIP_TRY(dbg.alloc(64));
    HIP_TRY(hipMemsetAsync(dbg.p, 0, 64, s));
    const char* tl_path = c->tune.lut_timeline.empty() ? nullptr : c->tune.lut_timeline.c_str();
    const long n_items_tl = blocks;
    if (tl_path) {
        HIP_TRY(tl.alloc((size_t)n_items_tl * 48));
        HIP_TRY(hipMemsetAsync(tl.p, 0, (size_t)n_items_tl * 48, s));
        q.timeline = (unsigned long long*)tl.p;
    } else {
        q.dbg = (unsigned long long*)dbg.p;
    }
#endif
    {
        ProfScope ps(c, s, KID_SPATIAL);
        void* args[] = {(void*)&q};
        HIP_TRY(hipLaunchKernel(lut_kernel_fused<FROM_IDS>(F.interleaved, occ8, dedup, F.gs_log2 == 3), dim3((unsigned)blocks), dim3(threads), args, lds, s));
        HIP_TRY(hipGetLastError());
    }
#if VET_STAGE_CYCLES
    if (tl_path) {
        std::vector<unsigned long long> h((size_t)n_items_tl * 6);
        HIP_TRY(hipMemcpyAsync(h.data(), tl.p, h.size() * 8, hipMemcpyDeviceToHost, s));
        HIP_TRY(hipStreamSynchronize(s));
        if (FILE* f = fopen(tl_path, "wb")) { fwrite(h.data(), 8, h.size(), f); fclose(f); }
    } else
    {
        unsigned long long t[8] = {};
        HIP_TRY(hipMemcpyAsync(t, dbg.p, 64, hipMemcpyDeviceToHost, s));
        HIP_TRY(hipStreamSynchronize(s));
        fprintf(stderr, "[k_spatial_lut fused] blocks %d FPW %d lds %zu | cycles per workgroup (thread 0): samples->set %.0f  lists %.0f  walk %.0f  entropy %.0f"
                        " | samples->set = init %.0f + sample loads %.0f + record gathers %.0f + inserts %.0f (+ barrier)\n",
                blocks, q.FPW, lds, (double)t[0] / blocks, (double)t[1] / blocks, (double)t[2] / blocks, (double)t[3] / blocks,
                (double)t[4] / blocks, (double)t[5] / blocks, (double)t[6] / blocks, (double)t[7] / blocks);
    }
#endif
    *launched = true;
    return VET_OK;
}

size_t batch_video_geometry(const vet_ctx* c, int U, long total_frames, int n_sum, bool dedup, int* fpw_out, int* uc_out,
                            int priv = 1, int sort_words = 0, int n_ovf = 0) {
    const int UC = U < 2048 ? U : 2048;
    int fpw = lut_frames_per_wg(U, total_frames, c->n_cu, n_sum);
    size_t lds = 0;
    for (;; fpw /= 2) {
        lds = vet::lut_lds_bytes(U, UC, fpw, n_sum, dedup, false, priv, sort_words, vet::lut_ovf_slots(UC, n_ovf, dedup));
        if (lds <= c->lds_max || fpw == 1) break;
    }
    *fpw_out = fpw; *uc_out = UC;
    return lds <= c->lds_max ? lds : 0;
}

int resolve_list_for(vet_plan* pl, const int* lat_idx, int K, int T, hipStream_t s, uint32_t** out) {
    *out = nullptr;
    bool any = false;
    for (int k = 0; k < K; ++k) any = any || (pl->lat[lat_idx[k]].fp_table && pl->lat[lat_idx[k]].markers > 0);
    if (!any) return VET_OK;
    void* buf = nullptr;
    int rc = pooled(pl->ctx, 9, ((size_t)T + 1) * sizeof(uint32_t), &buf);
    if (rc) return rc;
    HIP_TRY(hipMemsetAsync(buf, 0, sizeof(uint32_t), s));
    *out = (uint32_t*)buf;
    return VET_OK;
}

template <bool FROM_IDS>
int resolve_frames(vet_plan* pl, const int* lat_idx, int K, const vet::SampleSrc& src, int U, int T, double* out,
                   double* d_weights, const uint32_t* d_list, double* ws, hipStream_t s) {
    vet_ctx* c = pl->ctx;
    for (int k = 0; k < K; ++k) {
        const Lattice& L = pl->lat[lat_idx[k]];
        Geometry g;
        int rc = spatial_geometry(c, L.n, U, true, &g, true);
        if (rc) return rc;
        vet::SpatialParams p{};
        p.src = src; p.U = U; p.T = T;
        p.dir_unit = pl->d_dir_unit; p.nearest = L.d_nearest; p.tiles = L.d_tiles; p.n = L.n;
        p.cos_cull = pl->cos_cull;
        p.wc.max_ang = pl->max_ang; p.wc.inv_max = 1.0 / pl->max_ang; p.wc.power = pl->power; p.wc.shift = 0;
        p.hmax = L.hmax;
        p.ent_k = K == 1 ? out : ws + (size_t)k * T;
        p.assign = nullptr; p.present = nullptr; p.status = nullptr;
        p.weights = (k == 0 && lat_idx[0] == 0) ? d_weights : nullptr;
        p.FPW = 1; p.G = g.G; p.UC = g.UC;
        p.log2_tab = c->d_log2; p.full_norm = 0; p.norm_n = L.norm_n;
        p.frame_list = d_list;
        long grid = (long)c->n_cu * 4;
        if (grid > T) grid = T;
        void* args[] = {(void*)&p};
        ProfScope ps(c, s, KID_SPATIAL);
        auto lds_of = [&](int uc) { return g.lds - (size_t)g.UC * 24 + (size_t)uc * 28 + 16; };
        int uc = g.UC;
        while (lds_of(uc) > c->lds_max && uc > 64) uc /= 2;
        const size_t lds = lds_of(uc);
        if (lds > c->lds_max) return fail(VET_ERR_UNSUPPORTED, "resolver: %zu B of LDS", lds);
        p.UC = uc;
        HIP_TRY(hipLaunchKernel(spatial_w_kernel<FROM_IDS>(0, g.R, true), dim3((unsigned)grid), dim3(g.NW * vet::WAVE), args, lds, s));
    }
    if (K > 1) {
        ProfScope ps(c, s, KID_FINALIZE);
        hipLaunchKernelGGL(vet::k_finalize_list, dim3(grid_for(T, 256, c->n_cu)), dim3(256), 0, s, (const double*)ws, K, (long)T,
                           d_list, out);
        HIP_TRY(hipGetLastError());
    }
    return VET_OK;
}

template <bool FROM_IDS>
int launch_weights_pass(const WeightsCore& w, const vet::SampleSrc& src, int U, int T, double* d_weights, hipStream_t s,
                        vet_ctx* prof) {
    if (T <= 0) return VET_OK;
    if (w.ex.state == 1) {
        const int nw = weights_nw(w.lds_max, w.n0);
        if ((size_t)nw * w.n0 * 8 <= w.lds_max) {
            vet::WeightsGatherParams q{};
            q.src = src; q.U = U; q.T = T;
            q.alias = (const uint32_t*)w.ex.alias.get(); q.idx = (const uint16_t*)w.ex.idx.get();
            q.w = (const double*)w.ex.w.get(); q.len = (const uint32_t*)w.ex.len.get();
            q.stride = w.ex.stride; q.n = w.n0; q.out = d_weights;
            const int chunks = w.ex.stride / vet::WAVE;
            const void* fn = chunks <= 1 ? (const void*)vet::k_weights_gather<FROM_IDS, 1>
                           : chunks <= 2 ? (const void*)vet::k_weights_gather<FROM_IDS, 2>
                           : chunks <= 4 ? (const void*)vet::k_weights_gather<FROM_IDS, 4> : (const void*)vet::k_weights_gather<FROM_IDS, 0>;
            void* args[] = {(void*)&q};
            const size_t lds = (size_t)nw * w.n0 * 8;
            if (prof) {
                ProfScope ps(prof, s, KID_WEIGHTS);
                HIP_TRY(hipLaunchKernel(fn, dim3((unsigned)T), dim3(nw * vet::WAVE), args, lds, s));
            } else {
                HIP_TRY(hipLaunchKernel(fn, dim3((unsigned)T), dim3(nw * vet::WAVE), args, lds, s));
            }
            HIP_TRY(hipGetLastError());
            return VET_OK;
        }
    }
    Geometry g;
    int rc = sweep_geometry(w.lds_max, w.n0, U, &g);
    if (rc) return rc;
    vet::SpatialParams p{};
    p.src = src; p.U = U; p.T = T;
    p.dir_unit = (const double*)w.dir_unit.get(); p.nearest = nullptr; p.tiles = (const double*)w.tiles0.get(); p.n = w.n0;
    p.cos_cull = w.cos_cull;
    p.wc.max_ang = w.max_ang; p.wc.inv_max = 1.0 / w.max_ang; p.wc.power = w.power; p.wc.shift = 0;
    p.hmax = 1.0;
    p.ent_k = nullptr; p.assign = nullptr; p.present = nullptr; p.status = nullptr;
    p.weights = d_weights;
    p.FPW = g.FPW; p.G = g.G; p.UC = g.UC;
    p.norm_n = w.n0; p.frame_list = nullptr;
    const int blocks = (T + g.FPW - 1) / g.FPW;
    void* args[] = {(void*)&p};
    if (prof) {
        ProfScope ps(prof, s, KID_WEIGHTS);
        HIP_TRY(hipLaunchKernel(spatial_w_kernel<FROM_IDS>(0, g.R, true), dim3(blocks), dim3(g.NW * vet::WAVE), args, g.lds, s));
    } else {
        HIP_TRY(hipLaunchKernel(spatial_w_kernel<FROM_IDS>(0, g.R, true), dim3(blocks), dim3(g.NW * vet::WAVE), args, g.lds, s));
    }
    HIP_TRY(hipGetLastError());
    return VET_OK;
}

template <bool FROM_IDS>
int launch_spatial_main(vet_plan* pl, const vet::SampleSrc& src, int U, int T, double* d_entropy, int32_t* d_assign,
                        double* d_weights, int32_t* d_present, int32_t* d_status, hipStream_t s, double* d_wexact = nullptr,
                        bool* wrote_wexact = nullptr);

template <bool FROM_IDS>
int launch_spatial(vet_plan* pl, const vet::SampleSrc& src, int U, int T, double* d_entropy, int32_t* d_assign,
                   double* d_weights, int32_t* d_present, int32_t* d_status, hipStream_t s) {
    const bool exact = d_weights && pl->weighted && !pl->lat[0].binned && !pl->raw_weights;
    bool wrote = false;
    int rc = launch_spatial_main<FROM_IDS>(pl, src, U, T, d_entropy, d_assign, exact ? nullptr : d_weights, d_present, d_status, s,
                                           exact ? d_weights : nullptr, &wrote);
    if (rc || !exact || wrote) return rc;
    rc = ensure_exact_weights(pl, s);
    if (rc) return rc;
    return launch_weights_pass<FROM_IDS>(*pl->wcore, src, U, T, d_weights, s, pl->ctx);
}

template <bool FROM_IDS>
int launch_spatial_main(vet_plan* pl, const vet::SampleSrc& src, int U, int T, double* d_entropy, int32_t* d_assign,
                        double* d_weights, int32_t* d_present, int32_t* d_status, hipStream_t s, double* d_wexact,
                        bool* wrote_wexact) {
    vet_ctx* c = pl->ctx;
    const int K = (int)pl->lat.size();
    double* ent_k = d_entropy;
    int form[64];
    if (K > 64) return fail(VET_ERR_UNSUPPORTED, "more than 64 lattices in one plan");
    const bool want_table = table_requested(pl, (long)U * T, U);
    const bool fp64 = pl->fp64 && pl->weighted;
    double* const w0 = d_wexact ? d_wexact : d_weights;
    if (want_table && pl->weighted && !fp64) {
        int rc = ensure_fused(pl, s);
        if (rc) return rc;
        if (pl->fused.state == 1) {
            bool launched = false;
            rc = launch_lut_fused<FROM_IDS>(pl, src, U, T, nullptr, 0, 0, 0, 0, d_entropy, d_assign, d_weights, d_present,
                                            d_status, s, &launched);
            if (launched) for (int k = 0; k < K; ++k) pl->lat[k].last_form = F_TABLE;
            if (rc || launched) return rc;
// ... 295 lines not shown
        fb_max = std::max(fb_max, fb);
        frame0[v] = v ? frame0[v - 1] + videos[v - 1].n_frames : 0;
        outs[v] = x.d_entropy;
        vet::VideoDesc& d = desc[v];
        d.mu = x.d_mu; d.mv = x.d_mv; d.U = x.n_users; d.T = x.n_frames;
        d.entropy = x.d_entropy; d.assign = x.d_assign; d.present = x.d_present;
        d.FPW = fb; d.UC = 0; d.block0 = block; d.pad_ = 0;
        block += (x.n_frames + fb - 1) / fb;
    }
    frame0[n_videos] = frames;
    const size_t lds = u_lds_bytes(pl, max_users, n_max, fb_max);
    if (lds > c->lds_max) return VET_OK;
    double* ws = nullptr;
    if (K > 1) {
        int rc = ensure_ws(c, (size_t)K * frames * sizeof(double));
        if (rc) return rc;
        ws = (double*)c->ws;
        for (int k = 0; k < K; ++k)
            for (int v = 0; v < n_videos; ++v) {
                vet::VideoDesc& d = desc[(size_t)k * n_videos + v];
                d = desc[v];
                d.entropy = ws + (size_t)k * frames + frame0[v];
                if (k) { d.assign = nullptr; d.present = nullptr; }
            }
    }
    const size_t desc_b = desc.size() * sizeof(vet::VideoDesc), f0_b = frame0.size() * 8, outs_b = outs.size() * 8;
    BatchBlob blob;
    int rc = blob.acquire(c, desc_b + f0_b + outs_b);
    if (rc) return rc;
    memcpy(blob.host(), desc.data(), desc_b);
    memcpy((char*)blob.host() + desc_b, frame0.data(), f0_b);
    memcpy((char*)blob.host() + desc_b + f0_b, outs.data(), outs_b);
    char* base = (char*)blob.dev();
    long* d_frame0 = (long*)(base + desc_b);
    double** d_outs = (double**)(base + desc_b + f0_b);
    rc = blob.upload(s);
    if (rc) return rc;
    for (int k = 0; k < K; ++k) {
        const Lattice& L = pl->lat[k];
        vet::SpatialParams q{};
        q.src = vet::SampleSrc{nullptr, nullptr, nullptr, pl->W, pl->H, (long)pl->n_dirs};
        q.U = max_users; q.T = 0;
        q.nearest = L.d_nearest; q.n = L.n; q.hmax = L.hmax;
        q.status = k == 0 ? d_status : nullptr;
        q.FPW = fb_max;
        q.log2_tab = c->d_log2;
        q.full_norm = (L.binned && pl->weighted) ? 1 : 0;
        q.norm_n = L.norm_n;
        q.videos = (const vet::VideoDesc*)base + (size_t)k * n_videos;
        q.n_videos = n_videos; q.n_blocks = block;
        const long grid = u_lds_grid(c, block);
        ProfScope ps(c, s, KID_SPATIAL);
        const void* fn = pairs ? (const void*)vet::k_spatial_u_lds<false, true, true> : (const void*)vet::k_spatial_u_lds<false, false, true>;
        void* args[] = {(void*)&q};
        HIP_TRY(hipLaunchKernel(fn, dim3((unsigned)grid), dim3(kULdsThreads), args, lds, s));
        HIP_TRY(hipGetLastError());
    }
    if (K > 1) {
        ProfScope ps(c, s, KID_FINALIZE);
        hipLaunchKernelGGL(vet::k_finalize_batch, dim3(grid_for(frames, 256, c->n_cu)), dim3(256), 0, s, (const double*)ws, K, frames,
                           (const long*)d_frame0, (double* const*)d_outs, n_videos);
        HIP_TRY(hipGetLastError());
    }
    *launched = true;
    return VET_OK;
}

int vet_spatial_entropy_batch(vet_plan* pl, int n_videos, const vet_video* videos, int32_t* d_status, void* stream) {
    if (!pl) return fail(VET_ERR_INVALID, "plan is NULL");
    if (n_videos <= 0 || !videos) return fail(VET_ERR_INVALID, "need at least one video");
    if (!pl->grid) return fail(VET_ERR_INVALID, "plan has no pixel grid");
    vet_ctx* c = pl->ctx;
    hipStream_t s = stream ? (hipStream_t)stream : c->stream;
    const int K = (int)pl->lat.size();
    long total = 0, total_frames = 0;
    for (int v = 0; v < n_videos; ++v) {
        const vet_video& x = videos[v];
        if (x.n_users <= 0 || x.n_frames <= 0 || !x.d_mu || !x.d_mv || !x.d_entropy)
            return fail(VET_ERR_INVALID, "video %d: bad shape or NULL pointer", v);
        total += (long)x.n_users * x.n_frames;
        total_frames += x.n_frames;
    }
    int max_users = 0;
    for (int v = 0; v < n_videos; ++v) max_users = videos[v].n_users > max_users ? videos[v].n_users : max_users;
    if (!pl->weighted || any_binned(pl)) {
        bool all_counts = true;
        for (const auto& L : pl->lat) all_counts = all_counts && (!pl->weighted || L.binned);
        if (all_counts) {
            bool launched = false;
            int rc = batch_unweighted(pl, n_videos, videos, d_status, s, &launched);
            if (rc || launched) return rc;
        }
    }
    bool table = !(pl->fp64 && pl->weighted) && table_requested(pl, total, max_users);
    if (table) {
        int rc = ensure_fused(pl, s);
        if (rc) return rc;
        if (pl->fused.state == 1) {
            const int N = pl->fused.lay.N;
            const bool dedup = dedup_fused(max_users);
            std::vector<vet::VideoDesc> desc(n_videos);
            int block = 0;
            size_t lds_max = 0;
            bool fits = true;
            for (int v = 0; v < n_videos && fits; ++v) {
                const vet_video& x = videos[v];
                vet::VideoDesc& d = desc[v];
                d.mu = x.d_mu; d.mv = x.d_mv; d.U = x.n_users; d.T = x.n_frames;
                d.entropy = x.d_entropy; d.assign = x.d_assign; d.present = x.d_present;
                const size_t lds = batch_video_geometry(c, d.U, total_frames, N, dedup, &d.FPW, &d.UC);
                if (lds == 0) fits = false;
                d.block0 = block; d.pad_ = 0;
                block += (d.T + d.FPW - 1) / d.FPW;
                lds_max = lds > lds_max ? lds : lds_max;
            }
            if (fits) {
                BatchBlob blob;
                rc = upload_descriptors(c, desc, s, blob);
                if (rc) return rc;
                void* d_desc = blob.dev();
                const vet::SampleSrc src{nullptr, nullptr, nullptr, pl->W, pl->H, (long)pl->n_dirs};
                bool launched = false;
                rc = launch_lut_fused<false>(pl, src, 0, 0, (const vet::VideoDesc*)d_desc, n_videos, block, lds_max, max_users,
                                             nullptr, nullptr, nullptr, nullptr, d_status, s, &launched);
                if (launched) for (int k = 0; k < K; ++k) pl->lat[k].last_form = F_TABLE;
                if (rc || launched) return rc;
            }
        }
    }
    int form0 = F_SWEEP;
    for (int k = 0; k < K && table; ++k) {
        int form = F_SWEEP;
        int rc = choose_formulation(pl, k, true, max_users, s, &form);
        if (rc) return rc;
        if (k == 0) form0 = form;
        table = (form == F_TABLE || form == F_FTABLE) && form == form0;
        table = table && pl->lat[k].markers == 0;
    }
    int n_sum = 0;
    for (int k = 0; k < K; ++k) n_sum += pl->lat[k].n;
    std::vector<vet::VideoDesc> desc;
    size_t lds_max = 0;
    if (table) {
        const bool dedup = dedup_lattices(pl, max_users);
        desc.resize(n_videos);
        int block = 0;
        for (int v = 0; v < n_videos && table; ++v) {
            const vet_video& x = videos[v];
            vet::VideoDesc& d = desc[v];
            d.mu = x.d_mu; d.mv = x.d_mv; d.U = x.n_users; d.T = x.n_frames;
            d.entropy = x.d_entropy; d.assign = x.d_assign; d.present = x.d_present;
            const size_t lds = batch_video_geometry(c, d.U, total_frames, n_sum, dedup, &d.FPW, &d.UC, form0 == F_FTABLE ? 4 : 1,
                                                    (form0 == F_FTABLE && dedup && 2 * pl->n_rows <= 65536) ? (int)((2 * pl->n_rows + 31) / 32) : 0,
                                                    pl->lat[0].capped ? pl->lat[0].n_ovf : 0);
            if (lds == 0) table = false;
            d.block0 = block; d.pad_ = 0;
            block += (d.T + d.FPW - 1) / d.FPW;
            lds_max = lds > lds_max ? lds : lds_max;
        }
        if (table) {
            BatchBlob blob;
            int rc = upload_descriptors(c, desc, s, blob);
            if (rc) return rc;
            void* d_desc = blob.dev();
            int idx[vet::MAX_LATTICES];
            for (int k = 0; k < K; ++k) idx[k] = k;
            const vet::SampleSrc src{nullptr, nullptr, nullptr, pl->W, pl->H, (long)pl->n_dirs};
            bool launched = false;
            for (int k = 0; k < K; ++k) pl->lat[k].last_form = form0;
            return launch_lut<false>(pl, idx, K, src, 0, 0, (const vet::VideoDesc*)d_desc, n_videos, block, lds_max, max_users, nullptr,
                                     nullptr, nullptr, nullptr, d_status, s, &launched);
        }
    }
    for (int v = 0; v < n_videos; ++v) {
        const vet_video& x = videos[v];
        int rc = vet_spatial_entropy(pl, x.d_mu, x.d_mv, x.n_users, x.n_frames, x.d_entropy, x.d_assign, nullptr,
                                     x.d_present, d_status, s);
        if (rc) return rc;
    }
    return VET_OK;
}

}
```

viewport-entropy-toolkit_amd/csrc/vet_spatial_lut.hpp:

```cpp
#pragma once
#include "vet_common.hpp"

#ifndef VET_STAGE_CYCLES
#define VET_STAGE_CYCLES 0
#endif

namespace vet {


#define VET_DPP(v, ctrl, rmask) __builtin_amdgcn_update_dpp(0, (v), (ctrl), (rmask), 0xF, true)
__device__ __forceinline__ double wave_total(double v) {
    auto step = [&](auto mov) {
        const long long b = __double_as_longlong(v);
        const int lo = mov((int)(b & 0xFFFFFFFFll)), hi = mov((int)(b >> 32));
        return __longlong_as_double(((long long)hi << 32) | (unsigned)lo);
    };
    v += step([](int x) { return VET_DPP(x, 0xB1, 0xF); });
    v += step([](int x) { return VET_DPP(x, 0x4E, 0xF); });
    v += step([](int x) { return VET_DPP(x, 0x141, 0xF); });
    v += step([](int x) { return VET_DPP(x, 0x140, 0xF); });
    v += step([](int x) { return VET_DPP(x, 0x142, 0xA); });
    v += step([](int x) { return VET_DPP(x, 0x143, 0xC); });
    const long long b = __double_as_longlong(v);
    const int lo = __builtin_amdgcn_readlane((int)(b & 0xFFFFFFFFll), 63), hi = __builtin_amdgcn_readlane((int)(b >> 32), 63);
    return __longlong_as_double(((long long)hi << 32) | (unsigned)lo);
}
__device__ __forceinline__ unsigned long long wave_total(unsigned long long v) {
    auto step = [&](auto mov) {
        const int lo = mov((int)(v & 0xFFFFFFFFull)), hi = mov((int)(v >> 32));
        return ((unsigned long long)(unsigned)hi << 32) | (unsigned)lo;
    };
    v += step([](int x) { return VET_DPP(x, 0xB1, 0xF); });
    v += step([](int x) { return VET_DPP(x, 0x4E, 0xF); });
    v += step([](int x) { return VET_DPP(x, 0x141, 0xF); });
    v += step([](int x) { return VET_DPP(x, 0x140, 0xF); });
    v += step([](int x) { return VET_DPP(x, 0x142, 0xA); });
    v += step([](int x) { return VET_DPP(x, 0x143, 0xC); });
    const unsigned lo = (unsigned)__builtin_amdgcn_readlane((int)(v & 0xFFFFFFFFull), 63);
    const unsigned hi = (unsigned)__builtin_amdgcn_readlane((int)(v >> 32), 63);
    return ((unsigned long long)hi << 32) | lo;
}

template <bool HIGH>
__device__ __forceinline__ uint32_t lds_slot(uint32_t pair, int step, uint32_t base) {
    uint32_t a;
    if (HIGH) asm("v_mad_i32_i16 %0, %1, %2, %3 op_sel:[1,0,0,0]" : "=v"(a) : "v"(pair), "v"(step), "v"(base));
    else asm("v_mad_i32_i16 %0, %1, %2, %3" : "=v"(a) : "v"(pair), "v"(step), "v"(base));
    return a;
}
__device__ __forceinline__ void lds_add_u64(uint32_t lds_byte_address, unsigned long long v) {
    __hip_atomic_fetch_add((__attribute__((address_space(3))) unsigned long long*)(size_t)lds_byte_address, v, __ATOMIC_RELAXED,
                           __HIP_MEMORY_SCOPE_WORKGROUP);
}

template <int UN, bool INTERLEAVED, bool DEDUP, bool FPT, int GSL_IL = 4, int NB = 0>
__device__ __forceinline__ void walk_rows(const uint32_t* frows, const uint32_t* fmeta, int nu,
                                          unsigned long long* hrow, int n,
                                          const uint32_t* __restrict__ tab_w, const uint16_t* __restrict__ tab_i,
                                          int stride, int gs_log2_rt, uint32_t zero_row,
                                          uint32_t* marked = nullptr, int bit0 = 0) {
    const int NW = blockDim.x >> 6, lane = lane_id(), wv = wave_id();
    if constexpr (NB > 0) {
        static_assert(!FPT && INTERLEAVED && GSL_IL == 4, "capped rows: integer tables with 16-lane rows");
        constexpr int UPW = WAVE >> 4;
        int lane_here = lane;
        asm volatile("" : "+v"(lane_here));
        const int sub = lane_here >> 4, sl = lane_here & 15, step = NW * UPW;
        for (int j0 = wv * UPW; j0 < nu; j0 += UN * step) {
            uint32_t row[UN], mult[UN], hb32[UN];
            int sgn[UN];
#pragma unroll
            for (int k = 0; k < UN; ++k) {
                const int j = j0 + k * step + sub;
                const bool on = j < nu;
                const uint32_t pk = on ? frows[j] : 0u, m = on ? fmeta[j] : 0u;
                const uint32_t key = DEDUP ? pk >> 12 : pk;
                const bool flip = ((DEDUP ? key >> ROW_BITS : key >> 31) & 1u) != 0u;
                const uint32_t rid = DEDUP ? key & ROW_MASK : key & 0x7FFFFFFFu;
                row[k] = (on ? rid * (uint32_t)(NB * ROW_BLOCK) : zero_row) + (uint32_t)(4 * sl);
                const uint32_t cnt = DEDUP ? pk & 0xFFFu : (on ? 1u : 0u);
                mult[k] = cnt << ((m >> 16) & 0x1Fu);
                sgn[k] = flip ? -8 : 8;
                hb32[k] = (uint32_t)(size_t)(__attribute__((address_space(3))) char*)((char*)hrow + (flip ? (n - 1) * 8 : 0));
            }
#pragma unroll
            for (int b = 0; b < NB; ++b) {
                uint4 w[UN];
                uint2 tp[UN];
#pragma unroll
                for (int k = 0; k < UN; ++k) {
                    w[k] = *(const uint4*)(tab_w + row[k] + b * ROW_BLOCK);
                    tp[k] = *(const uint2*)(tab_i + row[k] + b * ROW_BLOCK);
                }
#pragma unroll
                for (int k = 0; k < UN; ++k) {
                    lds_add_u64(lds_slot<false>(tp[k].x, sgn[k], hb32[k]), (unsigned long long)w[k].x * mult[k]);
                    lds_add_u64(lds_slot<true>(tp[k].x, sgn[k], hb32[k]), (unsigned long long)w[k].y * mult[k]);
                    lds_add_u64(lds_slot<false>(tp[k].y, sgn[k], hb32[k]), (unsigned long long)w[k].z * mult[k]);
                    lds_add_u64(lds_slot<true>(tp[k].y, sgn[k], hb32[k]), (unsigned long long)w[k].w * mult[k]);
                }
            }
        }
        return;
    }
    const int gs_log2 = INTERLEAVED ? GSL_IL : gs_log2_rt;
    const int GS = 1 << gs_log2, UPW = WAVE >> gs_log2;
    const int sub = lane >> gs_log2, sl = lane & (GS - 1);
    const int step = NW * UPW;
    const int cut = INTERLEAVED ? min(4 * sl, 3 * GS - 1) : 4 * sl;
    for (int j0 = wv * UPW; j0 < nu; j0 += UN * step) {
        uint32_t row[UN];
        int lim[UN], sgn[UN];
        char* hb[UN];
        uint32_t mult[UN];
        double scale[UN];
        int longest = 0;
#pragma unroll
        for (int k = 0; k < UN; ++k) {
            const int j = j0 + k * step + sub;
            const bool on = j < nu;
            const uint32_t pk = on ? frows[j] : 0u, m = on ? fmeta[j] : 0u;
            const uint32_t key = DEDUP ? pk >> 12 : pk;
            const bool flip = ((DEDUP ? key >> ROW_BITS : key >> 31) & 1u) != 0u;
            const uint32_t rid = DEDUP ? key & ROW_MASK : key & 0x7FFFFFFFu;
            row[k] = on ? rid * (uint32_t)stride : zero_row;
            const int len = (int)(m & 0xFFFFu);
            lim[k] = len - cut;
            const uint32_t cnt = DEDUP ? pk & 0xFFFu : (on ? 1u : 0u);
            mult[k] = FPT ? cnt : cnt << ((m >> 16) & 0xFFFu);
            if (FPT) scale[k] = ldexp((double)cnt, -(int)((m >> 16) & 0xFFFu));
            sgn[k] = flip ? -8 : 8;
            hb[k] = (char*)hrow + (flip ? (n - 1) * 8 : 0);
            longest = max(longest, len);
        }
        for (int eb = 0; eb < longest; eb += 4 * GS) {
            uint32_t r[UN];
            bool any = false;
#pragma unroll
            for (int k = 0; k < UN; ++k) {
                const bool on = eb < lim[k];
                r[k] = (on ? row[k] : zero_row) + (uint32_t)(eb + 4 * sl);
                any = any || on;
            }
            if (!any) continue;
            uint4 w[UN];
            ushort4 t[UN];
#pragma unroll
            for (int k = 0; k < UN; ++k) {
                w[k] = *(const uint4*)(tab_w + r[k]);
                t[k] = *(const ushort4*)(tab_i + r[k]);
            }
#pragma unroll
            for (int k = 0; k < UN; ++k) {
                if (FPT) {
                    if (marked) {
                        const uint32_t wk[4] = {w[k].x, w[k].y, w[k].z, w[k].w};
                        const int tk[4] = {(int)t[k].x, (int)t[k].y, (int)t[k].z, (int)t[k].w};
#pragma unroll
                        for (int c = 0; c < 4; ++c)
                            if (wk[c] == MARKER_BITS) {
                                const int bit = bit0 + (sgn[k] < 0 ? n - 1 - tk[c] : tk[c]);
                                atomicOr(&marked[bit >> 5], 1u << (bit & 31));
                            }
                    }
                    atomicAdd((double*)(hb[k] + (int)t[k].x * sgn[k]), (double)__uint_as_float(w[k].x) * scale[k]);
                    atomicAdd((double*)(hb[k] + (int)t[k].y * sgn[k]), (double)__uint_as_float(w[k].y) * scale[k]);
                    atomicAdd((double*)(hb[k] + (int)t[k].z * sgn[k]), (double)__uint_as_float(w[k].z) * scale[k]);
                    atomicAdd((double*)(hb[k] + (int)t[k].w * sgn[k]), (double)__uint_as_float(w[k].w) * scale[k]);
                } else {
                    const uint32_t hb32 = (uint32_t)(size_t)(__attribute__((address_space(3))) char*)hb[k];
                    const uint2 tp = *(const uint2*)&t[k];
                    lds_add_u64(lds_slot<false>(tp.x, sgn[k], hb32), (unsigned long long)w[k].x * mult[k]);
                    lds_add_u64(lds_slot<true>(tp.x, sgn[k], hb32), (unsigned long long)w[k].y * mult[k]);
                    lds_add_u64(lds_slot<false>(tp.y, sgn[k], hb32), (unsigned long long)w[k].z * mult[k]);
                    lds_add_u64(lds_slot<true>(tp.y, sgn[k], hb32), (unsigned long long)w[k].w * mult[k]);
                }
            }
        }
    }
}

struct LutLattice {
    const uint32_t* tab_w;
    const uint16_t* tab_i;
    const uint32_t* tab_meta;
    int stride, gs_log2, n, interleaved;
    double hmax;
    uint32_t zrow;
    const uint32_t* ovf_w;
    const uint16_t* ovf_i;
    const uint32_t* ovf_of_row;
    int n_ovf;
};

struct VideoDesc {
    const double* mu;
    const double* mv;
    int U, T;
    double* entropy;
    int32_t* assign;
    int32_t* present;
    int FPW, UC, block0, pad_;
};

struct LutParams {
    const VideoDesc* videos;
    int n_videos;
    SampleSrc src;
    int U, T;
    const uint16_t* nearest;
    const uint32_t* alias;
    const uint2* dirrec;
    int rec_meta;
    int K;
    int n_sum;
    LutLattice lat[MAX_LATTICES];
    double* entropy;
    int32_t* assign;
    double* weights;
    int32_t* present;
    int32_t* status;
    int FPW, UC;
    int sort_words;
    int dedup_min_users;
    FusedLayout lay;
    unsigned long long* timeline;
    unsigned long long* dbg;
    uint32_t* resolve;
};

template <class V>
__device__ __forceinline__ double lattice_entropy_int(int n, V val, double hmax, double* wrow, double inv_unit) {
    const int lane = lane_id();
    unsigned long long hi = 0ull, lo = 0ull;
    double L = 0.0;
    for (int t = lane; t < n; t += WAVE) {
        const unsigned long long v = val(t);
        hi += v >> 32; lo += v & 0xFFFFFFFFull;
        const double vd = (double)v;
        if (v != 0ull) L += vd * log2(vd);
        if (wrow) __builtin_nontemporal_store(vd * inv_unit, wrow + t);
    }
    L = wave_total(L);
    hi = wave_total(hi); lo = wave_total(lo);
    const double S = (double)(hi + (lo >> 32)) * 4294967296.0 + (double)(lo & 0xFFFFFFFFull);
    if (!(S > 0.0)) return 0.0;
    double H = log2(S) - L / S;
    if (H < 1e-6) {
        double h = 0.0;
        for (int t = lane; t < n; t += WAVE) {
            const unsigned long long v = val(t);
            if (v != 0ull) { const double q = (double)v / S; h -= q * log2(q); }
        }
        H = wave_total(h);
    }
    return fmax(H, 0.0) / hmax;
}

template <class NOf, class HmaxOf>
__device__ __forceinline__ void lut_epilogue_int(const unsigned long long* hist, size_t frame_stride, int nf, long f0,
                                                 int K, NOf n_of, HmaxOf hmax_of, const int* np_of,
                                                 double* entropy, int32_t* present, double* weights, int32_t* status) {
    const int NW = blockDim.x >> 6, lane = lane_id(), wv = wave_id();
    const double inv_unit = 1.0 / (4294967296.0 * (double)(1u << TAB_X));
    for (int fl = wv; fl < nf; fl += NW) {
        const unsigned long long* hrow = hist + (size_t)fl * frame_stride;
        double total_entropy = 0.0;
        for (int k = 0; k < K; ++k) {
            const int n = n_of(k);
            total_entropy += lattice_entropy_int(n, [&](int t) { return hrow[t]; }, hmax_of(k),
                                                 (k == 0 && weights) ? weights + (f0 + fl) * (long)n : nullptr, inv_unit);
            hrow += n;
        }
        if (lane == 0) {
            const int np = np_of[fl];
            double e = total_entropy / (double)K;
            if (np == 0) {
                e = __builtin_nan("");
                if (status) atomicAdd(&status[1], 1);
            }
            entropy[f0 + fl] = e;
            if (present) present[f0 + fl] = np;
        }
    }
}

__device__ __forceinline__ void lut_epilogue_fused(const unsigned long long* hist, int nf, long f0, const FusedLayout& lay,
                                                   const int* np_of, double* entropy, int32_t* present, double* weights,
                                                   int32_t* status) {
    const int NW = blockDim.x >> 6, lane = lane_id(), wv = wave_id();
    const double inv_unit = 1.0 / (4294967296.0 * (double)(1u << TAB_X));
    const int N = lay.N, K = lay.K;
    for (int fl = wv; fl < nf; fl += NW) {
        const unsigned long long* hrow = hist + (size_t)fl * N;
        double total_entropy = 0.0;
        for (int k = 0; k < K; ++k) {
            const int n = lay.n[k], hh = n >> 1;
            auto val = [&](int t) {
                const int pos = fused_pos(lay, k, t);
                unsigned long long v = hrow[pos];
                if (t >= hh && t < n - hh) v += hrow[N - 1 - pos];
                return v;
            };
            total_entropy += lattice_entropy_int(n, val, lay.hmax[k], (k == 0 && weights) ? weights + (f0 + fl) * (long)n : nullptr,
                                                 inv_unit);
        }
        if (lane == 0) {
            const int np = np_of[fl];
            double e = total_entropy / (double)K;
            if (np == 0) {
                e = __builtin_nan("");
                if (status) atomicAdd(&status[1], 1);
            }
            entropy[f0 + fl] = e;
            if (present) present[f0 + fl] = np;
        }
    }
}

__host__ __device__ __forceinline__ int lut_hash_slots(int UC) {
    int hs = 64;
    while (hs < 2 * UC) hs <<= 1;
    return hs;
}
__host__ __device__ __forceinline__ int lut_marked_words(int n_sum) { return (n_sum + 31) >> 5; }
__host__ __device__ __forceinline__ size_t lut_lds_bytes(int U, int UC, int FPW, int n_sum, bool dedup, bool marked = false,
                                                         int priv = 1, int sort_words = 0, int ovf_slots = 0) {
    const size_t hist = (size_t)FPW * n_sum * 8 * priv, hash = dedup ? (size_t)FPW * lut_hash_slots(UC) * 4 : 0;
    const size_t srt = sort_words ? ((size_t)sort_words + 256) * 4 : 0;
    size_t a = (dedup && U <= UC) ? (hist > hash ? hist : hash) : hist + hash;
    if (dedup && U <= UC && srt > a) a = srt;
    return ((a + 15) & ~(size_t)15) + (size_t)FPW * UC * 8 + (size_t)2 * FPW * 4 + 64 +
           (marked ? (size_t)FPW * lut_marked_words(n_sum) * 4 : 0) + (ovf_slots ? (size_t)FPW * (4 + (size_t)ovf_slots * 8) : 0);
}

template <bool FROM_IDS, int UN, bool IL, bool OCC8, bool DEDUP, bool FPT, bool FUSED = false, int NB = 0>
__global__ __launch_bounds__(256, OCC8 ? 8 : (FPT ? 6 : 7)) void k_spatial_lut(const LutParams p) {
    extern __shared__ __attribute__((aligned(16))) unsigned char smem[];
    SampleSrc src = p.src;
    int U = p.U, T = p.T, FPW = p.FPW, UC = p.UC;
    double* entropy = p.entropy;
    int32_t* assign = p.assign;
    int32_t* present = p.present;
    double* weights = p.weights;
    long blk = blockIdx.x;
    if (p.videos) {
        int lo = 0, hi = p.n_videos - 1;
        while (lo < hi) {
            const int mid = (lo + hi + 1) >> 1;
            if (p.videos[mid].block0 <= (int)blockIdx.x) lo = mid; else hi = mid - 1;
        }
        const VideoDesc& d = p.videos[lo];
        src.mu = d.mu; src.mv = d.mv;
        U = d.U; T = d.T; FPW = d.FPW; UC = d.UC;
        entropy = d.entropy; assign = d.assign; present = d.present; weights = nullptr;
        blk -= d.block0;
    }
    const int HS = DEDUP ? lut_hash_slots(UC) : 0;
    const bool merge = DEDUP && U >= p.dedup_min_users;
    const bool overlay = DEDUP && U <= UC;
    const int PRIV = FPT ? (int)(blockDim.x >> 6) : 1;
    const size_t hist_bytes = (size_t)FPW * p.n_sum * 8 * PRIV, hash_bytes = (size_t)FPW * HS * 4;
    const size_t sort_bytes = (FPT && overlay && p.sort_words) ? ((size_t)p.sort_words + 256) * 4 : 0;
    size_t a_bytes = overlay ? (hist_bytes > hash_bytes ? hist_bytes : hash_bytes) : hist_bytes + hash_bytes;
    if (sort_bytes > a_bytes) a_bytes = sort_bytes;
    unsigned long long* hist = (unsigned long long*)smem;
    uint32_t* hash = (uint32_t*)(smem + (overlay ? 0 : hist_bytes));
    uint32_t* rows = (uint32_t*)(smem + ((a_bytes + 15) & ~(size_t)15));
    uint32_t* meta = rows + (size_t)FPW * UC;
    int* cnt_chunk = (int*)(meta + (size_t)FPW * UC);
    int* cnt_frame = cnt_chunk + FPW;
    const int MW = lut_marked_words(p.n_sum);
    uint32_t* marked = (FPT && p.resolve) ? (uint32_t*)(cnt_frame + FPW) : nullptr;
    int* const ovf_cnt = cnt_frame + FPW;
    auto ovf_slots = [&]() { return NB ? lut_ovf_slots(UC, p.lat[0].n_ovf, DEDUP) : 0; };
    auto note_overflow = [&](int fl, uint32_t word, uint32_t m) {
        if (!(m & META_OVERFLOW)) return;
        const int OC = ovf_slots();
        uint32_t* ovf_rows = (uint32_t*)(ovf_cnt + FPW);
        const uint32_t o = p.lat[0].ovf_of_row[DEDUP ? (word >> 12) & ROW_MASK : word & 0x7FFFFFFFu];
        const int pos = atomicAdd(&ovf_cnt[fl], 1);
        if (pos < OC) {
            ovf_rows[(size_t)fl * OC + pos] = DEDUP ? (word & ~(ROW_MASK << 12)) | (o << 12) : (word & 0x80000000u) | o;
            ovf_rows[(size_t)(FPW + fl) * OC + pos] = m;
        }
    };
    const int NW = blockDim.x >> 6;
    const int tid = threadIdx.x, lane = lane_id(), wv = wave_id();
    const long f0 = blk * FPW;
    const int nf = (int)min((long)FPW, (long)T - f0);
#if VET_STAGE_CYCLES
    unsigned long long tdbg[8] = {0, 0, 0, 0, 0, 0, 0, 0}, tlast = p.dbg ? __builtin_readcyclecounter() : 0ull, tsub = tlast;
    if (p.timeline && tid == 0) {
        p.timeline[(long)blockIdx.x * 6 + 0] = wall_clock64();
        p.timeline[(long)blockIdx.x * 6 + 5] = (unsigned long long)__builtin_amdgcn_s_getreg((31 << 11) | 4)  |
                                  ((unsigned long long)__builtin_amdgcn_s_getreg((31 << 11) | 20)  << 32);
    }
    auto stage = [&](int i) {
        if (p.timeline && tid == 0) p.timeline[(long)blockIdx.x * 6 + 1 + i] = wall_clock64();
        if (p.dbg) { const unsigned long long now = __builtin_readcyclecounter(); tdbg[i] += now - tlast; tlast = now; tsub = now; }
    };
    auto sub = [&](int i, bool wait_vm) {
        if (p.dbg) {
            if (wait_vm) asm volatile("s_waitcnt vmcnt(0)" ::: "memory");
            const unsigned long long now = __builtin_readcyclecounter(); tdbg[4 + i] += now - tsub; tsub = now;
        }
    };
#else
    auto stage = [](int) {};
    auto sub = [](int, bool) {};
#endif
    if (!overlay)
        for (int i = tid; i < FPW * p.n_sum * PRIV; i += blockDim.x) hist[i] = 0ull;
    for (int i = tid; i < 2 * FPW; i += blockDim.x) cnt_chunk[i] = 0;
    if (FPT && marked)
        for (int i = tid; i < FPW * MW; i += blockDim.x) marked[i] = 0u;
    bool bad = false;
    const int hs_shift = 32 - (31 - __clz(HS | 1));
    for (int u0 = 0; u0 < U; u0 += UC) {
        const int uc = min(UC, U - u0);
        __syncthreads();
        for (int i = tid; i < FPW; i += blockDim.x) {
            cnt_chunk[i] = 0;
            if (NB && p.lat[0].n_ovf) ovf_cnt[i] = 0;
        }
        if (merge)
            for (int i = tid; i < FPW * HS; i += blockDim.x) hash[i] = EMPTY_KEY;
        __syncthreads();
        constexpr int SPT = 4;
        const int total = nf * uc;
        sub(0, false);
        for (int i0 = tid; i0 < total; i0 += SPT * (int)blockDim.x) {
            int id[SPT], fls[SPT];
            long idxs[SPT];
            if (FROM_IDS) {
#pragma unroll
                for (int k = 0; k < SPT; ++k) {
                    const int i = i0 + k * (int)blockDim.x;
                    fls[k] = i / uc;
                    idxs[k] = (f0 + fls[k]) * (long)U + u0 + (i - fls[k] * uc);
                    id[k] = -1;
                    if (i < total) {
                        const int v = src.ids[idxs[k]];
                        if (v >= src.n_dirs) bad = true; else if (v >= 0) id[k] = v;
                    }
                }
            } else {
                double a[SPT], b[SPT];
#pragma unroll
                for (int k = 0; k < SPT; ++k) {
                    const int i = i0 + k * (int)blockDim.x;
                    fls[k] = i / uc;
                    idxs[k] = (f0 + fls[k]) * (long)U + u0 + (i - fls[k] * uc);
                    a[k] = b[k] = __builtin_nan("");
                    if (i < total) {
                        a[k] = __builtin_nontemporal_load(src.mu + idxs[k]);
                        b[k] = __builtin_nontemporal_load(src.mv + idxs[k]);
                    }
                }
                sub(1, true);
#pragma unroll
                for (int k = 0; k < SPT; ++k) id[k] = grid_dir(a[k], b[k], src.W, src.H, bad);
            }
            uint32_t row[SPT], m0[SPT];
            int near[SPT];
#pragma unroll
            for (int k = 0; k < SPT; ++k) {
                row[k] = 0u; near[k] = -1; m0[k] = 0u;
                if (id[k] >= 0) {
                    if (DEDUP) {
                        const uint2 rec = p.dirrec[id[k]];
                        row[k] = (rec.x & ROW_MASK) | ((rec.x >> 31) << ROW_BITS);
                        near[k] = (int)(((rec.x >> ROW_BITS) & 0xFFFu) | ((rec.y >> 28) << 12));
                        m0[k] = rec.y & 0xFFFFFFFu;
                    } else if (p.dirrec) {
                        const uint2 rec = p.dirrec[id[k]];
                        row[k] = (rec.x & ROW_MASK) | (rec.x & 0x80000000u);
                        near[k] = (int)(((rec.x >> ROW_BITS) & 0xFFFu) | ((rec.y >> 28) << 12));
                        m0[k] = rec.y & 0xFFFFFFFu;
                    } else {
                        row[k] = p.alias[id[k]];
                        if (assign) near[k] = (int)p.nearest[id[k]];
                    }
                }
            }
            sub(2, true);
            if (assign) {
#pragma unroll
                for (int k = 0; k < SPT; ++k)
                    if (i0 + k * (int)blockDim.x < total) __builtin_nontemporal_store(near[k], assign + idxs[k]);
            }
#pragma unroll
            for (int k = 0; k < SPT; ++k) {
                const bool valid = id[k] >= 0;
                const int fl = fls[k];
                const int fl0 = __builtin_amdgcn_readfirstlane(fl);
                const bool uniform = __ballot(fl != fl0) == 0ull;
                bool won = false;
                unsigned h = 0;
                if (merge) {
                    if (valid) {
                        uint32_t* tab = hash + (size_t)fl * HS;
                        h = (row[k] * 2654435761u) >> hs_shift;
                        for (;;) {
                            unsigned cur = tab[h];
                            if (cur == EMPTY_KEY) {
                                cur = atomicCAS(&tab[h], EMPTY_KEY, (row[k] << 12) | 1u);
                                if (cur == EMPTY_KEY) { won = true; break; }
                            }
                            if ((cur >> 12) == row[k]) { atomicAdd(&tab[h], 1u); break; }
                            h = (h + 1) & (unsigned)(HS - 1);
                        }
                    }
                } else {
                    won = valid;
                }
                const unsigned long long mv_ = __ballot(valid), mw = __ballot(won);
                if (uniform) {
                    int base = 0;
                    if (lane == 0) {
                        if (mv_) atomicAdd(&cnt_frame[fl0], (int)__popcll(mv_));
                        if (mw) base = atomicAdd(&cnt_chunk[fl0], (int)__popcll(mw));
                    }
                    base = __builtin_amdgcn_readfirstlane(base);
                    if (won) {
                        const size_t pos = (size_t)fl0 * UC + base + below(mw);
                        rows[pos] = merge ? h : (DEDUP ? (row[k] << 12) | 1u : row[k]);
                        meta[pos] = m0[k];
                    }
                } else {
                    if (valid) atomicAdd(&cnt_frame[fl], 1);
                    if (won) {
                        const size_t pos = (size_t)fl * UC + atomicAdd(&cnt_chunk[fl], 1);
                        rows[pos] = merge ? h : (DEDUP ? (row[k] << 12) | 1u : row[k]);
                        meta[pos] = m0[k];
                    }
                }
            }
        }
        sub(3, false);
        __syncthreads();
        stage(0);
        if (DEDUP) {
            if (merge)
                for (int i = tid; i < nf * UC; i += blockDim.x) {
                    const int fl = i / UC, j = i - fl * UC;
                    if (j < cnt_chunk[fl]) {
                        const uint32_t word = hash[(size_t)fl * HS + rows[i]];
                        rows[i] = word;
                        if (NB) note_overflow(fl, word, meta[i]);
                    }
                }
            if (overlay && !FPT) {
                __syncthreads();
                for (int i = tid; i < FPW * p.n_sum; i += blockDim.x) hist[i] = 0ull;
            }
        }
        if (FPT) {
            __syncthreads();
            constexpr int EPT = 8;
            const bool by_bitmap = merge && overlay && p.sort_words > 0;
            for (int fl = 0; fl < nf; ++fl) {
                const int cnt = cnt_chunk[fl];
                uint32_t* fr = rows + (size_t)fl * UC;
                uint32_t* fm = meta + (size_t)fl * UC;
                uint32_t key[EPT];
                int rank[EPT];
#pragma unroll
                for (int q = 0; q < EPT; ++q) {
                    const int e = tid + q * (int)blockDim.x;
                    key[q] = e < cnt ? fr[e] : 0xFFFFFFFFu;
                    rank[q] = 0;
                }
                if (by_bitmap) {
                    uint32_t* bm = (uint32_t*)smem;
                    uint32_t* toff = bm + p.sort_words;
                    const int SW = p.sort_words, WPT = (SW + (int)blockDim.x - 1) / (int)blockDim.x;
                    for (int i = tid; i < SW; i += blockDim.x) bm[i] = 0u;
                    __syncthreads();
#pragma unroll
                    for (int q = 0; q < EPT; ++q)
                        if (tid + q * (int)blockDim.x < cnt) {
                            const uint32_t k20 = key[q] >> 12, bit = (k20 & ROW_MASK) * 2u + ((k20 >> ROW_BITS) & 1u);
                            atomicOr(&bm[bit >> 5], 1u << (bit & 31));
                        }
                    __syncthreads();
                    int mine = 0;
                    for (int w = tid * WPT; w < min(SW, (tid + 1) * WPT); ++w) mine += __popc(bm[w]);
                    int incl = mine;
#pragma unroll
                    for (int o = 1; o < WAVE; o <<= 1) {
                        const int up = __shfl_up(incl, o, WAVE);
                        if (lane >= o) incl += up;
                    }
                    int* wtot = (int*)(toff + 252);
                    __syncthreads();
                    if (lane == WAVE - 1) wtot[wv] = incl;
                    __syncthreads();
                    int before = 0;
                    for (int w2 = 0; w2 < wv; ++w2) before += wtot[w2];
                    __syncthreads();
                    toff[tid] = (uint32_t)(before + incl - mine);
                    __syncthreads();
#pragma unroll
                    for (int q = 0; q < EPT; ++q)
                        if (tid + q * (int)blockDim.x < cnt) {
                            const uint32_t k20 = key[q] >> 12, bit = (k20 & ROW_MASK) * 2u + ((k20 >> ROW_BITS) & 1u);
                            const int w = (int)(bit >> 5), t0 = w / WPT;
                            int r = (int)toff[t0];
                            for (int w2 = t0 * WPT; w2 < w; ++w2) r += __popc(bm[w2]);
                            rank[q] = r + __popc(bm[w] & ((1u << (bit & 31)) - 1u));
                        }
                } else {
                    for (int j = 0; j < cnt; ++j) {
                        const uint32_t other = fr[j];
#pragma unroll
                        for (int q = 0; q < EPT; ++q) {
                            const int e = tid + q * (int)blockDim.x;
                            rank[q] += (other < key[q] || (other == key[q] && j < e)) ? 1 : 0;
                        }
                    }
                }
                uint32_t mk[EPT];
#pragma unroll
                for (int q = 0; q < EPT; ++q) mk[q] = tid + q * (int)blockDim.x < cnt ? fm[tid + q * (int)blockDim.x] : 0u;
                __syncthreads();
#pragma unroll
                for (int q = 0; q < EPT; ++q)
                    if (tid + q * (int)blockDim.x < cnt) { fr[rank[q]] = key[q]; fm[rank[q]] = mk[q]; }
                __syncthreads();
            }
            if (overlay) {
                for (int i = tid; i < FPW * p.n_sum * PRIV; i += blockDim.x) hist[i] = 0ull;
                __syncthreads();
            }
        }
        int hoff = 0;
        stage(1);
        for (int k = 0; k < p.K; ++k) {
            const LutLattice& L = p.lat[k];
            if (k) __syncthreads();
            if (!(k == 0 && p.rec_meta && (DEDUP || p.dirrec)))
                for (int i = tid; i < nf * UC; i += blockDim.x) {
                    const int fl = i / UC, j = i - fl * UC;
                    if (j < cnt_chunk[fl]) meta[i] = L.tab_meta[DEDUP ? (rows[i] >> 12) & ROW_MASK : rows[i] & 0x7FFFFFFFu];
                }
            if (NB && !merge)
                for (int i = tid; i < nf * UC; i += blockDim.x) {
                    const int fl = i / UC, j = i - fl * UC;
                    if (j < cnt_chunk[fl]) note_overflow(fl, rows[i], meta[i]);
                }
            __syncthreads();
            constexpr int GSL_IL = (FUSED && UN == 2) ? 3 : 4;
            for (int fl = 0; fl < nf; ++fl)
                if constexpr (NB > 0) {
                    unsigned long long* hrow = hist + (size_t)fl * p.n_sum + hoff;
                    walk_rows<UN, true, DEDUP, false, 4, NB>(rows + (size_t)fl * UC, meta + (size_t)fl * UC, cnt_chunk[fl], hrow, L.n,
                                                             L.tab_w, L.tab_i, L.stride, 4, L.zrow * (uint32_t)(NB * ROW_BLOCK));
                    if (const int OC = ovf_slots()) {
                        const uint32_t* ovf_rows = (const uint32_t*)(ovf_cnt + FPW);
                        walk_rows<UN, true, DEDUP, false, 4, 1>(ovf_rows + (size_t)fl * OC, ovf_rows + (size_t)(FPW + fl) * OC,
                                                                min(ovf_cnt[fl], OC), hrow, L.n, L.ovf_w, L.ovf_i, ROW_BLOCK, 4,
                                                                (uint32_t)L.n_ovf * (uint32_t)ROW_BLOCK);
                    }
                } else if (IL && L.interleaved)
                    walk_rows<UN, true, DEDUP, FPT, GSL_IL>(rows + (size_t)fl * UC, meta + (size_t)fl * UC, cnt_chunk[fl],
                                               hist + ((size_t)fl * PRIV + (FPT ? wv : 0)) * p.n_sum + hoff, L.n, L.tab_w, L.tab_i, L.stride, L.gs_log2,
                                               L.zrow * (uint32_t)L.stride, marked ? marked + (size_t)fl * MW : nullptr, hoff);
                else
                    walk_rows<UN, false, DEDUP, FPT>(rows + (size_t)fl * UC, meta + (size_t)fl * UC, cnt_chunk[fl],
                                                hist + ((size_t)fl * PRIV + (FPT ? wv : 0)) * p.n_sum + hoff, L.n, L.tab_w, L.tab_i, L.stride, L.gs_log2,
                                                L.zrow * (uint32_t)L.stride, marked ? marked + (size_t)fl * MW : nullptr, hoff);
            hoff += L.n;
        }
    }
    __syncthreads();
    stage(2);
    if (FUSED) {
        lut_epilogue_fused(hist, nf, f0, p.lay, cnt_frame, entropy, present, weights, p.status);
    } else if (!FPT) {
        lut_epilogue_int(hist, (size_t)p.n_sum, nf, f0, p.K, [&](int k) { return p.lat[k].n; }, [&](int k) { return p.lat[k].hmax; },
                         cnt_frame, entropy, present, weights, p.status);
    } else
    for (int fl = wv; fl < nf; fl += NW) {
        const unsigned long long* hrow = hist + (size_t)fl * PRIV * p.n_sum;
        auto fp_value = [&](const unsigned long long* h, int t) {
            double v = 0.0;
            for (int w = 0; w < PRIV; ++w) v += __longlong_as_double((long long)h[(size_t)w * p.n_sum + t]);
            return v;
        };
        double total_entropy = 0.0;
        bool unresolved = false;
        int bit0 = 0;
        for (int k = 0; k < p.K; ++k) {
            const int n = p.lat[k].n;
            double totd = 0.0;
            for (int t = lane; t < n; t += WAVE) totd += fp_value(hrow, t);
            totd = wave_sum(totd);
            double h = 0.0;
            for (int t = lane; t < n; t += WAVE) {
                const double v = fp_value(hrow, t);
                if (v != 0.0) {
                    const double q = v / totd;
                    h -= q * log2(q);
                }
                if (k == 0 && weights) __builtin_nontemporal_store(v, weights + (f0 + fl) * (long)n + t);
                if (marked && v == 0.0) {
                    const int bit = bit0 + t;
                    unresolved = unresolved || ((marked[(size_t)fl * MW + (bit >> 5)] >> (bit & 31)) & 1u) != 0u;
                }
            }
            h = wave_sum(h);
            total_entropy += h / p.lat[k].hmax;
            hrow += n;
            bit0 += n;
        }
        if (marked && __ballot(unresolved) != 0ull && lane == 0)
            p.resolve[1 + atomicAdd(&p.resolve[0], 1u)] = (uint32_t)(f0 + fl);
        if (lane == 0) {
            const int np = cnt_frame[fl];
            double e = total_entropy / (double)p.K;
            if (np == 0) {
                e = __builtin_nan("");
                if (p.status) atomicAdd(&p.status[1], 1);
            }
            entropy[f0 + fl] = e;
            if (present) present[f0 + fl] = np;
        }
    }
#if VET_STAGE_CYCLES
    if (p.timeline && !p.dbg) stage(3);
    if (p.dbg) {
        stage(3);
        if (tid == 0)
            for (int i = 0; i < 8; ++i) atomicAdd(&p.dbg[i], tdbg[i]);
    }
#endif
    if (p.status) {
        const unsigned long long anybad = __ballot(bad);
        if (anybad && lane == 0) atomicAdd(&p.status[0], (int)__popcll(anybad));
    }
}

}
```

viewport-entropy-toolkit_amd/csrc/vet_weight_table.hpp:

```cpp
#pragma once
#include "vet_weights.hpp"

namespace vet {


#define VET_ULTRA_TINY 0x1p-1048

struct StatsParams {
    const double* dir_unit;
    long D;
    const double* tiles;
    int n;
    double cos_cull;
    WeightCfg wc;
    uint8_t* row_s;
    uint16_t* row_e;
    unsigned long long* crit;
    const int* canon;
    const uint8_t* shift_in;
};

constexpr uint16_t ROW_E_FORCE_OK = 0x8000u;

__global__ void k_row_stats(const StatsParams p) {
// ... 156 lines not shown
            if (lane == 0 && p.row_len) p.row_len[d] = count;
        } else if (FILL) {
            for (int pos = count + lane; pos < p.stride; pos += WAVE) {
                p.w[d * p.stride + pos] = 0u;
                p.idx[d * p.stride + pos] = (uint16_t)(pos % slots);
            }
            if (ovf != NO_OVERFLOW)
                for (int pos = count - p.cap + lane; pos < ROW_BLOCK; pos += WAVE) {
                    p.ow[(size_t)ovf * ROW_BLOCK + pos] = 0u;
                    p.oi[(size_t)ovf * ROW_BLOCK + pos] = (uint16_t)((p.cap + pos) % slots);
                }
            const int main_count = p.cap ? min(count, p.cap) : count;
            if (lane == 0) {
                if (p.meta) p.meta[d] = (uint32_t)main_count | (ovf != NO_OVERFLOW ? META_OVERFLOW : 0u) | ((uint32_t)row_shift << 16);
            }
            if (p.gs_log2 == 4 || p.gs_log2 == 3) {
                const int GSL = p.gs_log2, GS = 1 << GSL, B = 4 * GS;
                const bool active = lane < B;
                for (int eb = 0; eb < main_count; eb += B) {
                    if (!block_interleaved(main_count, eb, GSL)) continue;
                    __threadfence_block();
                    const bool real = active && eb + lane < main_count;
                    uint32_t wv = 0; uint16_t iv = 0;
                    if (real) { wv = p.w[d * p.stride + eb + lane]; iv = p.idx[d * p.stride + eb + lane]; }
                    asm volatile("s_waitcnt vmcnt(0)" ::: "memory");
                    const int cls = iv & 15;
                    int r = 0;
                    for (int c = 0; c < 16; ++c) {
                        const unsigned long long m = __ballot(real && cls == c);
                        if (real && cls == c) r = below(m);
                    }
                    int comp = (r * (16 >> GSL) + (cls >> GSL)) & 3, q = 0, used[4], freeb[5];
                    for (int k = 0; k < 4; ++k) {
                        const unsigned long long m = __ballot(real && comp == k);
                        if (real && comp == k) q = below(m);
                        used[k] = min(GS, (int)__popcll(m));
                    }
                    const bool placed = real && q < GS;
                    unsigned usedmask[4];
                    for (int k = 0; k < 4; ++k) {
                        usedmask[k] = 0;
                        for (int c = 0; c < 16; ++c)
                            if (__ballot(placed && comp == k && cls == c)) usedmask[k] |= 1u << c;
                    }
                    freeb[0] = 0;
                    for (int k = 0; k < 4; ++k) freeb[k + 1] = freeb[k] + GS - used[k];
                    const bool leftover = active && !placed;
                    const unsigned long long lm = __ballot(leftover);
                    if (leftover) {
                        const int j = below(lm);
                        int k = 0;
                        while (k < 3 && j >= freeb[k + 1]) ++k;
                        const int jj = j - freeb[k];
                        comp = k; q = used[k] + jj;
                        if (!real) {
                            int seen = 0, c = 0;
                            for (; c < 15; ++c) {
                                if (!((usedmask[k] >> c) & 1u)) { if (seen == jj) break; ++seen; }
                            }
                            iv = (uint16_t)c;
                        }
                    }
                    if (active) {
                        p.w[d * p.stride + eb + q * 4 + comp] = wv;
                        p.idx[d * p.stride + eb + q * 4 + comp] = iv;
                    }
                }
            }
        }
        longest = max(longest, count);
    }
    if (!FILL && lane == 0 && longest > *(volatile int*)p.maxcount) atomicMax(p.maxcount, longest);
    if (FILL && p.markers) {
        nmark = wave_sum(nmark);
        if (lane == 0 && nmark) atomicAdd(p.markers, nmark);
    }
    if (FILL && wave == 0 && p.ow)
        for (int pos = lane; pos < ROW_BLOCK; pos += WAVE) {
            p.ow[(size_t)p.n_ovf * ROW_BLOCK + pos] = 0u;
            p.oi[(size_t)p.n_ovf * ROW_BLOCK + pos] = (uint16_t)((pos >> 2) & 15);
        }
    if (FILL && wave == 0 && p.w) {
        for (int pos = lane; pos < p.stride; pos += WAVE) {
            p.w[p.D * p.stride + pos] = 0u;
            p.idx[p.D * p.stride + pos] = (uint16_t)(p.gs_log2 >= 3 ? (pos >> 2) & 15 : pos % slots);
        }
        if (lane == 0) {
            if (p.meta) p.meta[p.D] = p.fp ? 0u : (uint32_t)TAB_X << 16;
        }
    }
}


struct WexactParams {
    const double* dir_unit;
    const int* canon;
    long R;
    const double* tiles;
    int n;
    double cos_cull;
    WeightCfg wc;
    int stride;
    uint16_t* idx;
    double* w;
    uint32_t* len;
};
__global__ void k_wexact(const WexactParams p) {
    const int lane = lane_id();
    const long wave = ((long)blockIdx.x * blockDim.x + threadIdx.x) >> 6;
    const long nwaves = ((long)gridDim.x * blockDim.x) >> 6;
    for (long r = wave; r < p.R; r += nwaves) {
        const long dd = (long)p.canon[r];
        const double dx = p.dir_unit[3 * dd], dy = p.dir_unit[3 * dd + 1], dz = p.dir_unit[3 * dd + 2];
        int count = 0;
        for (int t0 = 0; t0 < p.n; t0 += WAVE) {
            const int t = t0 + lane;
            const bool valid = t < p.n;
            const int ts = valid ? t : 0;
            const double c = fma(dz, p.tiles[3 * ts + 2], fma(dy, p.tiles[3 * ts + 1], dx * p.tiles[3 * ts]));
            double wt = 0.0;
            const bool in = valid && (c > p.cos_cull) && fov_weight_cone(c, p.wc, wt);
            const unsigned long long mask = __ballot(in);
            if (in) {
                const size_t pos = (size_t)r * p.stride + count + below(mask);
                p.idx[pos] = (uint16_t)t;
                p.w[pos] = wt;
            }
            count += __popcll(mask);
        }
        if (lane == 0) p.len[r] = (uint32_t)count;
    }
}

__global__ void k_fuse_shifts(const int* __restrict__ canon, int R, int nl, const uint8_t* const* __restrict__ row_s,
                              uint8_t* __restrict__ out, int* __restrict__ delta) {
    for (int r = blockIdx.x * blockDim.x + threadIdx.x; r < R; r += gridDim.x * blockDim.x) {
        const int d = canon[r];
        int s = 0;
        for (int k = 0; k < nl; ++k) s = max(s, (int)row_s[k][d]);
        out[r] = (uint8_t)s;
        for (int k = 0; k < nl; ++k)
            if (s > (int)row_s[k][d]) atomicMax(&delta[k], s - (int)row_s[k][d]);
    }
}

__global__ void k_dirrec(const uint32_t* __restrict__ alias, const uint16_t* __restrict__ nearest,
                         const uint32_t* __restrict__ meta0, long D, uint2* __restrict__ rec) {
    for (long d = blockIdx.x * (long)blockDim.x + threadIdx.x; d < D; d += (long)gridDim.x * blockDim.x) {
        const uint32_t a = alias[d], near = nearest[d], row = a & 0x7FFFFu;
        rec[d] = make_uint2(row | ((near & 0xFFFu) << 19) | (a & 0x80000000u), (meta0[row] & 0xFFFFFFFu) | ((near >> 12) << 28));
    }
}

}
```

viewport-entropy-toolkit_amd/viewport_entropy_toolkit/_native.py:

```python

from __future__ import annotations

import ctypes as C
import os
import threading
from pathlib import Path
from typing import Optional, Sequence

import numpy as np

from . import _quantiser

_PKG_DIR = Path(__file__).resolve().parent
LIB_PATH = Path(os.environ.get("VET_HIP_LIBRARY", _PKG_DIR.parent / "lib" / "libvet_hip.so"))

VET_OK, VET_ERR_INVALID, VET_ERR_DEVICE, VET_ERR_RANGE, VET_ERR_EMPTY, VET_ERR_UNSUPPORTED = 0, -1, -2, -3, -4, -5
KERNEL_IDS = {"k_grid_dirs": 0, "k_nearest_lut": 1, "k_spatial": 2, "k_transition": 3, "k_finalize": 4,
              "k_wtab": 5, "k_weights": 6}


class NativeUnavailable(RuntimeError):
    """The HIP extension is missing or no MI355X is visible."""


class NativeError(RuntimeError):

    def __init__(self, code: int, message: str):
        super().__init__(message)
        self.code = code


class Video(C.Structure):
    _fields_ = [("d_mu", C.c_void_p), ("d_mv", C.c_void_p), ("n_users", C.c_int), ("n_frames", C.c_int),
                ("d_entropy", C.c_void_p), ("d_assign", C.c_void_p), ("d_present", C.c_void_p)]


class Track(C.Structure):
    _fields_ = [("time", C.POINTER(C.c_double)), ("mu", C.POINTER(C.c_double)), ("mv", C.POINTER(C.c_double)),
                ("n_rows", C.c_int64), ("status", C.c_int)]


VET_CSV_OK, VET_CSV_FALLBACK, VET_CSV_IO = 0, 1, 2


class _PlanDesc(C.Structure):
    _fields_ = [
        ("video_width", C.c_int), ("video_height", C.c_int),
        ("h_lon_cos", C.c_void_p), ("h_lon_sin", C.c_void_p),
        ("h_lat_sin", C.c_void_p), ("h_lat_cos", C.c_void_p),
        ("h_dir_table", C.c_void_p), ("n_dirs", C.c_int64),
        ("n_lattices", C.c_int), ("n_tiles", C.c_void_p),
        ("h_tiles", C.c_void_p), ("h_max_entropy", C.c_void_p),
        ("fov_angle", C.c_double), ("max_angular_distance", C.c_double),
        ("power_factor", C.c_double), ("use_weight_distribution", C.c_int),
        ("h_bin_lut", C.c_void_p), ("n_norm_tiles", C.c_void_p),
    ]


_P, _I, _I64, _D, _SZ = C.c_void_p, C.c_int, C.c_int64, C.c_double, C.c_size_t
SIGNATURES = {
    "vet_version": (_I, []),
    "vet_last_error": (C.c_char_p, []),
    "vet_device_count": (_I, []),
    "vet_create": (_I, [_I, C.POINTER(_P)]),
    "vet_destroy": (_I, [_P]),
    "vet_synchronize": (_I, [_P]),
    "vet_device_pci_bus_id": (_I, [_P, C.c_char_p, _I]),
    "vet_profile_enable": (_I, [_P, _I]),
    "vet_test_no_row_cap": (_I, [_P, _I]),
    "vet_profile_reset": (_I, [_P]),
    "vet_profile_get": (_I, [_P, _I, C.POINTER(_D), C.POINTER(_I64)]),
    "vet_kernel_name": (C.c_char_p, [_I]),
    "vet_malloc": (_I, [_P, _SZ, C.POINTER(_P)]),
    "vet_free": (_I, [_P, _P]),
    "vet_memcpy_h2d": (_I, [_P, _P, _P, _SZ]),
    "vet_memcpy_d2h": (_I, [_P, _P, _P, _SZ]),
    "vet_plan_create": (_I, [_P, C.POINTER(_PlanDesc), C.POINTER(_P)]),
    "vet_plan_destroy": (_I, [_P]),
    "vet_plan_n_dirs": (_I64, [_P]),
    "vet_plan_set_table_policy": (_I, [_P, _I]),
    "vet_plan_set_fp64": (_I, [_P, _I]),
    "vet_plan_set_raw_weights": (_I, [_P, _I]),
    "vet_plan_table_stride": (_I, [_P, _I]),
    "vet_plan_table_rows": (_I64, [_P]),
    "vet_plan_table_cap": (_I, [_P, _I, C.POINTER(_I64)]),
    "vet_plan_last_formulation": (_I, [_P, _I]),
    "vet_plan_error_bounds": (_I, [_P, _I, C.POINTER(_D), C.POINTER(_D)]),
    "vet_plan_read_dirs": (_I, [_P, _P]),
    "vet_plan_read_nearest": (_I, [_P, _I, _P]),
    "vet_plan_read_table": (_I, [_P, _I, _P, _P, _P, _P, _P, _P]),
    "vet_spatial_entropy": (_I, [_P, _P, _P, _I, _I, _P, _P, _P, _P, _P, _P]),
    "vet_spatial_entropy_ids": (_I, [_P, _P, _I, _I, _P, _P, _P, _P, _P, _P]),
    "vet_window_rows": (_I64, [_I, _I, _I]),
    "vet_spatial_entropy_windowed": (_I, [_P, _P, _P, _I, _I, _I, _I, _P, _P, _P, _P, _P]),
    "vet_spatial_entropy_windowed_ids": (_I, [_P, _P, _I, _I, _I, _I, _P, _P, _P, _P, _P]),
    "vet_spatial_entropy_windowed_host": (_I, [_P, _P, _P, _P, _I, _I, _I, _I, _P, _P, _P]),
    "vet_transition_entropy": (_I, [_P, _P, _P, _I, _I, _P, _P, _P, _P, _P, _P]),
    "vet_transition_entropy_ids": (_I, [_P, _P, _I, _I, _P, _P, _P, _P, _P, _P]),
    "vet_spatial_entropy_batch": (_I, [_P, _I, _P, _P, _P]),
    "vet_spatial_entropy_batch_host": (_I, [_P, _I, _P, _P, _P, _P, _P, _P, _P]),
    "vet_transition_entropy_batch": (_I, [_P, _I, _P, _P, _P]),
    "vet_transition_entropy_batch_host": (_I, [_P, _I, _P, _P, _P, _P, _P, _P, _P]),
    "vet_spatial_entropy_host": (_I, [_P, _P, _P, _P, _I, _I, _P, _P, _P, _P]),
    "vet_transition_entropy_host": (_I, [_P, _P, _P, _P, _I, _I, _P, _P, _P, _P]),
    "vet_spatial_entropy_host_resident": (_I, [_P, _P, _P, _P, _I, _I, _P, _P, C.POINTER(_P)]),
    "vet_transition_entropy_host_resident": (_I, [_P, _P, _P, _P, _I, _I, _P, _P, C.POINTER(_P)]),
    "vet_result_fetch": (_I, [_P, _I, _I64, _I64, _P]),
    "vet_result_free": (_I, [_P]),
    "vet_fb_tile_boundaries": (_I, [_P, _P, _I, _I, _P, _P]),
    "vet_angular_distances": (_I, [_P, _P, _I64, _P, _I, _P]),
    "vet_heatmap_create": (_I, [_P, _P, _I, _I, _I, _I, _I, _I, C.POINTER(_P)]),
    "vet_heatmap_destroy": (_I, [_P]),
    "vet_heatmap_read_map": (_I, [_P, _P]),
    "vet_heatmap_render": (_I, [_P, _P, _P, _P, _P, _I, _I, _P, _P]),
    "vet_heatmap_render_result": (_I, [_P, _P, _P, _P, _P, _I, _I64, _I64, _P]),
    "vet_heatmap_render_counts": (_I, [_P, _P, _P, _P, _P, _I, _I, _P, _P]),
    "vet_heatmap_render_transition_result": (_I, [_P, _P, _P, _P, _P, _I, _I64, _I64, _P]),
    "vet_heatmap_create_latlon": (_I, [_P, _I, _I, _I, _I, _I, _I, _I, C.POINTER(_P)]),
    "vet_heatmap_render_binned": (_I, [_P, _P, _P, _P, _I, _I, _I, _P, _P]),
    "vet_heatmap_render_binned_host": (_I, [_P, _P, _P, _P, _I, _I, _I, _P]),
    "vet_tiling_create": (_I, [_P, _P, _I, _P, _I, _I, _I, C.POINTER(_P)]),
    "vet_tiling_destroy": (_I, [_P]),
    "vet_tiling_render": (_I, [_P, _P, _I, _P, _P, _P]),
    "vet_tiling_render_host": (_I, [_P, _P, _I, _P, _P]),
    "vet_csv_read_tracks": (_I, [_I, C.POINTER(C.c_char_p), C.POINTER(Track), _I]),
    "vet_csv_free_tracks": (None, [_I, C.POINTER(Track)]),
}

FORMULATIONS = {0: "table", 1: "sweep", 2: "precise", 3: "ftable", 4: "dtable"}

_lib = None
_lib_lock = threading.Lock()


def _preload_hip_runtime() -> Optional[str]:
    if os.environ.get("VET_HIP_RUNTIME", "").lower() == "system":
        return None
    try:
        import importlib.util
        spec = importlib.util.find_spec("torch")
    except (ImportError, ValueError):
        spec = None
    if spec is None or not spec.origin:
        return None
    cand = Path(spec.origin).parent / "lib" / "libamdhip64.so"
    if not cand.exists():
        return None
    try:
        C.CDLL(str(cand), mode=C.RTLD_GLOBAL)
    except OSError:
        return None
    return str(cand)


HIP_RUNTIME_PRELOADED: Optional[str] = None


def load_library():
    global _lib, HIP_RUNTIME_PRELOADED
    with _lib_lock:
        if _lib is not None:
            return _lib
        if not LIB_PATH.exists():
            raise NativeUnavailable(
                f"HIP extension not found at {LIB_PATH}. Build it with "
                f"`make -C {_PKG_DIR.parent / 'csrc'}` (or __graft_entry__.build()); "
                "this package has no CPU compute path.")
        HIP_RUNTIME_PRELOADED = _preload_hip_runtime()
        try:
            lib = C.CDLL(str(LIB_PATH))
        except OSError as e:
            raise NativeUnavailable(f"cannot load {LIB_PATH}: {e}") from e
        for name, (res, args) in SIGNATURES.items():
            fn = getattr(lib, name)
            fn.restype, fn.argtypes = res, args
        _lib = lib
        return lib


def read_tracks(paths: Sequence, n_threads: int = 0):
    lib = load_library()
    n = len(paths)
    if n == 0:
        return []
    c_paths = (C.c_char_p * n)(*[os.fsencode(str(p)) for p in paths])
    tracks = (Track * n)()
    rc = lib.vet_csv_read_tracks(n, c_paths, tracks, int(n_threads))
    if rc != VET_OK:
        raise NativeError(rc, "vet_csv_read_tracks failed")
    try:
        out = []
        for t in tracks:
            if t.status == VET_CSV_OK:
                m = int(t.n_rows)
                cols = [np.frombuffer(C.string_at(ptr, m * 8), dtype=np.float64).copy() if m else np.empty(0)
                        for ptr in (t.time, t.mu, t.mv)]
                out.append((VET_CSV_OK, *cols))
            else:
                out.append((int(t.status), None, None, None))
        return out
    finally:
        lib.vet_csv_free_tracks(n, tracks)


def _check(lib, rc: int):
    if rc != VET_OK:
        msg = lib.vet_last_error()
        raise NativeError(rc, (msg or b"").decode("utf-8", "replace") or f"vet error {rc}")


def _ptr(a: Optional[np.ndarray]):
    return None if a is None else a.ctypes.data_as(C.c_void_p)


VET_STREAM_LEGACY = 1
TABLE_SAMPLES_PER_DIRECTION = 2


def _stream(handle):
    if handle is None:
        return None
    return C.c_void_p(VET_STREAM_LEGACY if int(handle) == 0 else int(handle))


class Engine:

    _default = None
    _default_lock = threading.Lock()

    def __init__(self, device_id: int = 0):
        self.lib = load_library()
        h = C.c_void_p()
        rc = self.lib.vet_create(device_id, C.byref(h))
        if rc == VET_ERR_DEVICE:
            raise NativeUnavailable((self.lib.vet_last_error() or b"").decode())
        _check(self.lib, rc)
        self.handle = h
        self.device_id = device_id

    @staticmethod
    def default_device_id(n_devices: int) -> int:
        for var in ("VET_DEVICE", "LOCAL_RANK"):
            raw = os.environ.get(var)
            if raw is None:
                continue
            try:
                dev = int(raw)
            except ValueError:
                raise NativeUnavailable(f"{var}={raw!r} is not a device index") from None
            if not 0 <= dev < n_devices:
                raise NativeUnavailable(
                    f"{var}={dev} names no visible device ({n_devices} visible): refusing to fall back to device 0 "
                    "(the ranks of a multi-GPU job would share one GPU); fix the launcher's device visibility or set VET_DEVICE")
            return dev
        return 0

    @classmethod
    def default(cls) -> "Engine":
        with cls._default_lock:
            if cls._default is None:
                n = load_library().vet_device_count()
                if n <= 0:
                    raise NativeUnavailable("no HIP device available; this package has no CPU compute path")
                cls._default = cls(cls.default_device_id(n))
            return cls._default

    def pci_bus_id(self) -> str:
        buf = C.create_string_buffer(64)
        _check(self.lib, self.lib.vet_device_pci_bus_id(self.handle, buf, 64))
        return buf.value.decode()

    def close(self):
        if getattr(self, "handle", None):
            self.lib.vet_destroy(self.handle)
            self.handle = None

    def synchronize(self):
        _check(self.lib, self.lib.vet_synchronize(self.handle))

    def fb_tile_boundaries(self, tiles: np.ndarray, max_edges: int = 16):
        tiles = np.ascontiguousarray(tiles, dtype=np.float64).reshape(-1, 3)
        n = len(tiles)
        edges = np.empty((n, max_edges, 2, 3), dtype=np.float64)
        count = np.empty(n, dtype=np.int32)
        _check(self.lib, self.lib.vet_fb_tile_boundaries(self.handle, _ptr(tiles), n, max_edges, _ptr(edges), _ptr(count)))
        return edges, count

    def angular_distances(self, vectors: np.ndarray, tiles: np.ndarray) -> np.ndarray:
        vectors = np.ascontiguousarray(vectors, dtype=np.float64).reshape(-1, 3)
        tiles = np.ascontiguousarray(tiles, dtype=np.float64).reshape(-1, 3)
        out = np.empty((len(vectors), len(tiles)), dtype=np.float64)
        if out.size:
            _check(self.lib, self.lib.vet_angular_distances(self.handle, _ptr(vectors), len(vectors), _ptr(tiles), len(tiles), _ptr(out)))
        return out

    def test_no_row_cap(self, on: bool = True):
        _check(self.lib, self.lib.vet_test_no_row_cap(self.handle, int(on)))

    def profile_enable(self, on: bool = True):
        _check(self.lib, self.lib.vet_profile_enable(self.handle, int(on)))

    def profile_reset(self):
        _check(self.lib, self.lib.vet_profile_reset(self.handle))

    def profile_get(self, kernel: str):
        ms, n = C.c_double(), C.c_int64()
        _check(self.lib, self.lib.vet_profile_get(self.handle, KERNEL_IDS[kernel], C.byref(ms), C.byref(n)))
        return ms.value, n.value


class DeviceResult:

    def __init__(self, lib, handle, n_rows, shapes, dtypes, engine=None):
        self.lib, self.handle, self.n_rows = lib, handle, int(n_rows)
        self.shapes, self.dtypes = shapes, dtypes
        self.engine = engine

    def rows(self, which: int, row0: int, n: int) -> np.ndarray:
        if self.handle is None:
            raise RuntimeError("the device-resident result has been released")
        out = np.empty((n,) + tuple(self.shapes[which]), dtype=self.dtypes[which])
        _check(self.lib, self.lib.vet_result_fetch(self.handle, which, row0, n, _ptr(out)))
        return out

    def close(self):
        if getattr(self, "handle", None):
            self.lib.vet_result_free(self.handle)
            self.handle = None

    def __del__(self):
        try:
            self.close()
        except Exception:
            pass


class Plan:

    def __init__(self, engine: Engine, tile_xyz: Sequence[np.ndarray], fov_angle: float, power_factor: float,
                 use_weight_distribution: bool, video_width: int = 0, video_height: int = 0,
                 dir_table: Optional[np.ndarray] = None, bin_luts: Optional[Sequence] = None,
                 bin_counts: Optional[Sequence[int]] = None, bin_max_entropy: Optional[Sequence[float]] = None,
                 bin_norm_tiles: Optional[Sequence[int]] = None):
        self.engine = engine
        self.lib = engine.lib
        bin_luts = list(bin_luts) if bin_luts is not None else [None] * len(tile_xyz)
        self.tiles = [np.ascontiguousarray(t, dtype=np.float64) if t is not None else np.zeros((1, 3))
                      for t in tile_xyz]
        self.n_tiles = [len(t) if b is None else int(bin_counts[k])
                        for k, (t, b) in enumerate(zip(self.tiles, bin_luts))]
        self.weighted = bool(use_weight_distribution)
        self.width, self.height = int(video_width), int(video_height)
        d = _PlanDesc()
        keep = []
        if dir_table is None:
            axes = _quantiser.axis_trig(self.width, self.height)
            keep.extend(axes)
            d.video_width, d.video_height = self.width, self.height
            d.h_lon_cos, d.h_lon_sin, d.h_lat_sin, d.h_lat_cos = (a.ctypes.data for a in axes)
        else:
            tab = np.ascontiguousarray(dir_table, dtype=np.float64).reshape(-1, 3)
            keep.append(tab)
            d.h_dir_table, d.n_dirs = tab.ctypes.data, len(tab)
        n_arr = np.asarray(self.n_tiles, dtype=np.int32)
        ptrs = (C.c_void_p * len(self.tiles))(*[t.ctypes.data for t in self.tiles])
        hmax = np.asarray([_quantiser.max_entropy(n) if b is None else float(bin_max_entropy[k])
                           for k, (n, b) in enumerate(zip(self.n_tiles, bin_luts))], dtype=np.float64)
        keep.extend([n_arr, ptrs, hmax])
        if any(b is not None for b in bin_luts):
            luts = [None if b is None else np.ascontiguousarray(b, dtype=np.uint16).reshape(-1) for b in bin_luts]
            lut_ptrs = (C.c_void_p * len(luts))(*[None if b is None else b.ctypes.data for b in luts])
            norm = np.asarray([n if b is None else int(bin_norm_tiles[k])
                               for k, (n, b) in enumerate(zip(self.n_tiles, bin_luts))], dtype=np.int32)
            keep.extend([luts, lut_ptrs, norm])
            d.h_bin_lut = C.cast(lut_ptrs, C.c_void_p)
            d.n_norm_tiles = norm.ctypes.data
        d.n_lattices = len(self.tiles)
        d.n_tiles = n_arr.ctypes.data
        d.h_tiles = C.cast(ptrs, C.c_void_p)
        d.h_max_entropy = hmax.ctypes.data
        d.fov_angle = float(fov_angle)
        d.max_angular_distance = float(np.radians(fov_angle / 2.0))
        d.power_factor = float(power_factor)
        d.use_weight_distribution = int(self.weighted)
        h = C.c_void_p()
        _check(self.lib, self.lib.vet_plan_create(engine.handle, C.byref(d), C.byref(h)))
        self.handle = h
        self.n_dirs = int(self.lib.vet_plan_n_dirs(h))

    def close(self):
        if getattr(self, "handle", None):
            self.lib.vet_plan_destroy(self.handle)
            self.handle = None

    def __del__(self):
        try:
            self.close()
        except Exception:
            pass

    def set_table_policy(self, policy: int):
        _check(self.lib, self.lib.vet_plan_set_table_policy(self.handle, int(policy)))

    def set_fp64(self, on: bool = True):
        _check(self.lib, self.lib.vet_plan_set_fp64(self.handle, 1 if on else 0))

    def set_raw_weights(self, on: bool = True):
        _check(self.lib, self.lib.vet_plan_set_raw_weights(self.handle, 1 if on else 0))

    def table_stride(self, lattice: int = 0) -> int:
        return int(self.lib.vet_plan_table_stride(self.handle, lattice))

    def table_rows(self) -> int:
        return int(self.lib.vet_plan_table_rows(self.handle))

    def table_cap(self, lattice: int = 0):
        n = C.c_int64()
        return int(self.lib.vet_plan_table_cap(self.handle, lattice, C.byref(n))), int(n.value)

    def last_formulation(self, lattice: int = 0) -> str:
        return FORMULATIONS.get(int(self.lib.vet_plan_last_formulation(self.handle, lattice)), "")

    def error_bounds(self, lattice: int = 0):
        a, b = C.c_double(), C.c_double()
        _check(self.lib, self.lib.vet_plan_error_bounds(self.handle, lattice, C.byref(a), C.byref(b)))
        return a.value, b.value

    def read_dirs(self) -> np.ndarray:
        out = np.empty((self.n_dirs, 3), dtype=np.float64)
        _check(self.lib, self.lib.vet_plan_read_dirs(self.handle, _ptr(out)))
        return out

    def read_nearest(self, lattice: int = 0) -> np.ndarray:
        out = np.empty(self.n_dirs, dtype=np.int32)
        _check(self.lib, self.lib.vet_plan_read_nearest(self.handle, lattice, _ptr(out)))
        return out

    def read_table(self, lattice: int = 0) -> dict:
        cap, n_ovf = self.table_cap(lattice)
        if cap <= 0:
            raise ValueError("the lattice has no table of its own (yet)")
        rows = self.table_rows()
        out = {"w": np.empty((rows + 1, cap), np.uint32), "tile": np.empty((rows + 1, cap), np.uint16),
               "meta": np.empty(rows + 1, np.uint32)}
        if n_ovf:
            out.update(ovf_w=np.empty((n_ovf + 1, 64), np.uint32), ovf_tile=np.empty((n_ovf + 1, 64), np.uint16),
                       ovf_of_row=np.empty(rows, np.uint32))
        _check(self.lib, self.lib.vet_plan_read_table(self.handle, lattice, _ptr(out["w"]), _ptr(out["tile"]), _ptr(out["meta"]),
                                                      _ptr(out["ovf_w"]) if "ovf_w" in out else None,
                                                      _ptr(out["ovf_tile"]) if "ovf_tile" in out else None,
                                                      _ptr(out["ovf_of_row"]) if "ovf_of_row" in out else None))
        return out

    @staticmethod
    def _samples(mu, mv, ids):
        if ids is not None:
            ids = np.ascontiguousarray(ids, dtype=np.int32)
            return None, None, ids, ids.shape
        mu = np.ascontiguousarray(mu, dtype=np.float64)
        mv = np.ascontiguousarray(mv, dtype=np.float64)
        if mu.shape != mv.shape or mu.ndim != 2:
            raise ValueError("mu and mv must be [n_frames, n_users] arrays of equal shape")
        return mu, mv, None, mu.shape

    def spatial(self, mu=None, mv=None, ids=None, want_assign=True, want_weights=False, check=True):
        mu, mv, ids, (T, U) = self._samples(mu, mv, ids)
        ent = np.empty(T, dtype=np.float64)
        assign = np.empty((T, U), dtype=np.int32) if want_assign else None
        weights = np.empty((T, self.n_tiles[0]), dtype=np.float64) if want_weights else None
        present = np.empty(T, dtype=np.int32)
        rc = self.lib.vet_spatial_entropy_host(self.handle, _ptr(mu), _ptr(mv), _ptr(ids), U, T, _ptr(ent),
                                               _ptr(assign), _ptr(weights), _ptr(present))
        if rc not in (VET_OK, VET_ERR_EMPTY, VET_ERR_RANGE) or (check and rc != VET_OK):
            _check(self.lib, rc)
        return dict(entropy=ent, assign=assign, weights=weights, present=present, code=rc)

    def spatial_windowed(self, mu=None, mv=None, ids=None, window=None, stride=1, want_weights=False, check=True):
        mu, mv, ids, (T, U) = self._samples(mu, mv, ids)
        if window is None:
            raise ValueError("window (a number of frames) is required")
        window, stride = int(window), int(stride)
        R = int(self.lib.vet_window_rows(T, window, stride))
        if R < 0:
            raise ValueError(f"need 1 <= window <= n_frames and stride >= 1 (got window={window}, stride={stride}, {T} frames)")
        ent = np.empty(R, dtype=np.float64)
        weights = np.empty((R, self.n_tiles[0]), dtype=np.float64) if want_weights else None
        samples = np.empty(R, dtype=np.int32)
        rc = self.lib.vet_spatial_entropy_windowed_host(self.handle, _ptr(mu), _ptr(mv), _ptr(ids), U, T, window, stride,
                                                        _ptr(ent), _ptr(weights), _ptr(samples))
        if rc not in (VET_OK, VET_ERR_EMPTY, VET_ERR_RANGE) or (check and rc != VET_OK):
            _check(self.lib, rc)
        return dict(entropy=ent, weights=weights, samples=samples, code=rc)

    def transition(self, mu=None, mv=None, ids=None, want_pairs=True, want_srccount=False, check=True):
        mu, mv, ids, (T, U) = self._samples(mu, mv, ids)
        R = max(T - 1, 0)
        ent = np.empty(R, dtype=np.float64)
        pairs = np.empty((R, U, 2), dtype=np.int32) if want_pairs else None
        src = np.empty((R, self.n_tiles[0]), dtype=np.int32) if want_srccount else None
        common = np.empty(R, dtype=np.int32)
        rc = self.lib.vet_transition_entropy_host(self.handle, _ptr(mu), _ptr(mv), _ptr(ids), U, T, _ptr(ent),
                                                  _ptr(pairs), _ptr(src), _ptr(common))
        if rc not in (VET_OK, VET_ERR_EMPTY, VET_ERR_RANGE) or (check and rc != VET_OK):
            _check(self.lib, rc)
        return dict(entropy=ent, pairs=pairs, srccount=src, common=common, code=rc)

    def spatial_resident(self, mu=None, mv=None, ids=None, check=True):
        mu, mv, ids, (T, U) = self._samples(mu, mv, ids)
        ent = np.empty(T, dtype=np.float64)
        present = np.empty(T, dtype=np.int32)
        h = C.c_void_p()
        rc = self.lib.vet_spatial_entropy_host_resident(self.handle, _ptr(mu), _ptr(mv), _ptr(ids), U, T, _ptr(ent),
                                                        _ptr(present), C.byref(h))
        result = DeviceResult(self.lib, h, T, [(U,), (self.n_tiles[0],)], [np.int32, np.float64], self.engine) if h.value else None
        if rc not in (VET_OK, VET_ERR_EMPTY, VET_ERR_RANGE) or (check and rc != VET_OK):
            if result is not None:
                result.close()
            _check(self.lib, rc)
        return dict(entropy=ent, present=present, result=result, code=rc)

    def transition_resident(self, mu=None, mv=None, ids=None, check=True):
        mu, mv, ids, (T, U) = self._samples(mu, mv, ids)
        R = max(T - 1, 0)
        ent = np.empty(R, dtype=np.float64)
        common = np.empty(R, dtype=np.int32)
        h = C.c_void_p()
        rc = self.lib.vet_transition_entropy_host_resident(self.handle, _ptr(mu), _ptr(mv), _ptr(ids), U, T, _ptr(ent),
                                                           _ptr(common), C.byref(h))
        result = DeviceResult(self.lib, h, R, [(U, 2), (self.n_tiles[0],)], [np.int32, np.int32], self.engine) if h.value else None
        if rc not in (VET_OK, VET_ERR_EMPTY, VET_ERR_RANGE) or (check and rc != VET_OK):
            if result is not None:
                result.close()
            _check(self.lib, rc)
        return dict(entropy=ent, common=common, result=result, code=rc)

    def spatial_batch(self, videos, want_assign=False, check=True):
        mus = [np.ascontiguousarray(m, dtype=np.float64) for m, _ in videos]
        mvs = [np.ascontiguousarray(v, dtype=np.float64) for _, v in videos]
        T = np.asarray([m.shape[0] for m in mus], dtype=np.int32)
        U = np.asarray([m.shape[1] for m in mus], dtype=np.int32)
        mu = np.concatenate([m.ravel() for m in mus])
        mv = np.concatenate([v.ravel() for v in mvs])
        ent = np.empty(int(T.sum()), dtype=np.float64)
        present = np.empty(int(T.sum()), dtype=np.int32)
        assign = np.empty(mu.size, dtype=np.int32) if want_assign else None
        rc = self.lib.vet_spatial_entropy_batch_host(self.handle, len(mus), _ptr(U), _ptr(T), _ptr(mu), _ptr(mv),
                                                     _ptr(ent), _ptr(assign), _ptr(present))
        if rc not in (VET_OK, VET_ERR_EMPTY, VET_ERR_RANGE) or (check and rc != VET_OK):
            _check(self.lib, rc)
        out, so, ro = [], 0, 0
        for t, u in zip(T.tolist(), U.tolist()):
            out.append(dict(entropy=ent[ro:ro + t], present=present[ro:ro + t],
                            assign=assign[so:so + t * u].reshape(t, u) if want_assign else None))
            so += t * u
            ro += t
        return out

    def transition_batch(self, videos, want_pairs=False, check=True):
        mus = [np.ascontiguousarray(m, dtype=np.float64) for m, _ in videos]
        mvs = [np.ascontiguousarray(v, dtype=np.float64) for _, v in videos]
        T = np.asarray([m.shape[0] for m in mus], dtype=np.int32)
        U = np.asarray([m.shape[1] for m in mus], dtype=np.int32)
        mu = np.concatenate([m.ravel() for m in mus])
        mv = np.concatenate([v.ravel() for v in mvs])
        R = int((T - 1).sum())
        ent = np.empty(R, dtype=np.float64)
        common = np.empty(R, dtype=np.int32)
        pairs = np.empty(int(((T - 1) * U).sum()) * 2, dtype=np.int32) if want_pairs else None
        rc = self.lib.vet_transition_entropy_batch_host(self.handle, len(mus), _ptr(U), _ptr(T), _ptr(mu), _ptr(mv),
                                                        _ptr(ent), _ptr(pairs), _ptr(common))
        if rc not in (VET_OK, VET_ERR_EMPTY, VET_ERR_RANGE) or (check and rc != VET_OK):
            _check(self.lib, rc)
# ... 193 lines not shown
```

Baseline: 29.51 billion samples/s.

## Pack direction records and per-user row list into one 32-bit word

Adds a compact 32-bit direction record (row, mirror bit, tile, shift, overflow flag) built at plan time when row and tile counts fit, and a capped dedup kernel variant that uses it. The kernel's per-user row list in shared memory stores a single walk word holding row, multiplicity and shift, so the separate meta array and its fill pass go away. This halves the record gather from global memory and the LDS footprint per row, which may allow more frames per workgroup. It adds a new kernel instantiation and packing and unpacking bit logic, and falls back to 8-byte records when the fields do not fit.

```diff
diff --git a/include/vet.h b/include/vet.h
--- a/include/vet.h
+++ b/include/vet.h
@@ -33,6 +33,7 @@
 int vet_device_pci_bus_id(vet_ctx *ctx, char *buf, int len);
 int vet_profile_enable(vet_ctx *ctx, int on);
 int vet_test_no_row_cap(vet_ctx *ctx, int on);
+int vet_test_rec8(vet_ctx *ctx, int on);
 int vet_profile_reset(vet_ctx *ctx);
 int vet_profile_get(vet_ctx *ctx, int kernel_id, double *total_ms, int64_t *launches);
 const char *vet_kernel_name(int kernel_id);
@@ -69,6 +70,8 @@
 int vet_plan_table_stride(const vet_plan *plan, int lattice);
 int64_t vet_plan_table_rows(const vet_plan *plan);
 int vet_plan_table_cap(const vet_plan *plan, int lattice, int64_t *overflow_rows);
+int vet_plan_record_bytes(const vet_plan *plan);
+int vet_plan_read_records(vet_plan *plan, uint32_t *h_rec32);
 int vet_plan_last_formulation(const vet_plan *plan, int lattice);
 int vet_plan_error_bounds(vet_plan *plan, int lattice, double *table_bound, double *sweep_bound);
 int vet_plan_read_dirs(vet_plan *plan, double *h_xyz );
diff --git a/viewport-entropy-toolkit_amd/csrc/vet_context.hip b/viewport-entropy-toolkit_amd/csrc/vet_context.hip
--- a/viewport-entropy-toolkit_amd/csrc/vet_context.hip
+++ b/viewport-entropy-toolkit_amd/csrc/vet_context.hip
@@ -209,6 +209,11 @@
     c->tune.no_row_cap = on != 0;
     return VET_OK;
 }
+int vet_test_rec8(vet_ctx* c, int on) {
+    if (!c) return fail(VET_ERR_INVALID, "ctx is NULL");
+    c->tune.rec8 = on != 0;
+    return VET_OK;
+}
 int vet_profile_enable(vet_ctx* c, int on) {
     if (!c) return fail(VET_ERR_INVALID, "ctx is NULL");
     c->profiling = on != 0;
diff --git a/viewport-entropy-toolkit_amd/csrc/vet_host.hpp b/viewport-entropy-toolkit_amd/csrc/vet_host.hpp
--- a/viewport-entropy-toolkit_amd/csrc/vet_host.hpp
+++ b/viewport-entropy-toolkit_amd/csrc/vet_host.hpp
@@ -70,6 +70,7 @@
     std::string lut_timeline;
     int no_exact_rows = 0;
     int no_row_cap = 0;
+    int rec8 = 0;
     void from_environment();
 };
 
@@ -147,6 +148,7 @@
     uint32_t* d_alias = nullptr;
     bool mirror = false;
     uint2* d_dirrec = nullptr;
+    uint32_t* d_dirrec32 = nullptr;
     int n_rows = 0;
     int* d_canon = nullptr;
     struct Fused {
@@ -168,6 +170,10 @@
 };
 
 namespace vh {
+
+inline bool use_rec32(const vet_plan* pl) {
+    return pl->d_dirrec32 && !pl->ctx->tune.rec8 && !pl->lat.empty() && pl->lat[0].capped;
+}
 
 struct ProfScope {
     vet_ctx* c;
diff --git a/viewport-entropy-toolkit_amd/csrc/vet_layout.hpp b/viewport-entropy-toolkit_amd/csrc/vet_layout.hpp
--- a/viewport-entropy-toolkit_amd/csrc/vet_layout.hpp
+++ b/viewport-entropy-toolkit_amd/csrc/vet_layout.hpp
@@ -18,6 +18,24 @@
 constexpr int MAX_CAP_BLOCKS = 3;
 constexpr uint32_t META_OVERFLOW = 1u << 15;
 constexpr uint32_t NO_OVERFLOW = 0xFFFFFFFFu;
+
+constexpr int REC32_ROW_BITS = 15;
+constexpr int REC32_TILE_BITS = 10;
+constexpr int REC32_SHIFT_BITS = 5;
+constexpr uint32_t REC32_ROW_MASK = (1u << REC32_ROW_BITS) - 1;
+constexpr uint32_t REC32_KEY_MASK = (1u << (REC32_ROW_BITS + 1)) - 1;
+constexpr int REC32_TILE_POS = REC32_ROW_BITS + 1;
+constexpr int REC32_SHIFT_POS = REC32_TILE_POS + REC32_TILE_BITS;
+constexpr uint32_t REC32_OVERFLOW = 1u << 31;
+constexpr uint32_t REC32_AUX_MASK = ~((1u << REC32_SHIFT_POS) - 1);
+static_assert(REC32_SHIFT_POS + REC32_SHIFT_BITS == 31, "row, mirror, tile, shift and the overflow bit fill 32 bits");
+static_assert(TAB_X < (1 << REC32_SHIFT_BITS), "-shift in [0, TAB_X] fits its field");
+static_assert(REC32_ROW_BITS <= ROW_BITS, "a compact row is a row of the set");
+constexpr int WALK32_CNT_POS = 5, WALK32_CNT_BITS = 11, WALK32_ROW_POS = 16;
+constexpr int REC32_MAX_CHUNK = 1 << WALK32_CNT_BITS;
+constexpr uint32_t WALK32_OVF_TMP = 1u << WALK32_CNT_POS;
+static_assert(WALK32_CNT_POS + WALK32_CNT_BITS == WALK32_ROW_POS && WALK32_ROW_POS + REC32_ROW_BITS + 1 == 32, "walk word");
+static_assert(TAB_X < (1 << WALK32_CNT_POS), "the left shift fits below the multiplicity");
 __host__ __device__ __forceinline__ int lut_ovf_slots(int UC, int n_ovf, bool dedup) {
     if (n_ovf <= 0) return 0;
     const int most = dedup ? (2 * n_ovf > DEDUP_MIN_USERS ? 2 * n_ovf : DEDUP_MIN_USERS) : UC;
diff --git a/viewport-entropy-toolkit_amd/csrc/vet_plan.hip b/viewport-entropy-toolkit_amd/csrc/vet_plan.hip
--- a/viewport-entropy-toolkit_amd/csrc/vet_plan.hip
+++ b/viewport-entropy-toolkit_amd/csrc/vet_plan.hip
@@ -237,9 +237,22 @@
                            L.d_nearest, L.d_tab_meta, (long)pl->n_dirs, pl->d_dirrec);
         HIP_TRY(hipGetLastError());
     }
-    int markers = 0;
-    HIP_TRY(hipMemcpyAsync(&markers, d_max + 1, sizeof(int), hipMemcpyDeviceToHost, s));
+    const bool rec32 = k == 0 && capped && pl->d_dirrec && (uint64_t)pl->n_rows + 1 <= ((uint64_t)1 << vet::REC32_ROW_BITS) &&
+                       L.n <= (1 << vet::REC32_TILE_BITS);
+    if (pl->d_dirrec32) { (void)hipFree(pl->d_dirrec32); pl->d_dirrec32 = nullptr; }
+    if (rec32) {
+        HIP_TRY(hipMalloc((void**)&pl->d_dirrec32, (size_t)pl->n_dirs * sizeof(uint32_t)));
+        HIP_TRY(hipMemsetAsync(d_max, 0, sizeof(int), s));
+        ProfScope ps(c, s, KID_WTAB);
+        hipLaunchKernelGGL(vet::k_dirrec32, dim3(grid_for(pl->n_dirs, 256, c->n_cu)), dim3(256), 0, s, pl->d_alias,
+                           L.d_nearest, L.d_tab_meta, (long)pl->n_dirs, pl->d_dirrec32, d_max);
+        HIP_TRY(hipGetLastError());
+    }
+    int counts[2] = {0, 0};
+    HIP_TRY(hipMemcpyAsync(counts, d_max, sizeof(counts), hipMemcpyDeviceToHost, s));
     HIP_TRY(hipStreamSynchronize(s));
+    const int markers = counts[1];
+    if (rec32 && counts[0] != 0) { (void)hipFree(pl->d_dirrec32); pl->d_dirrec32 = nullptr; }
     guard.armed = false;
     L.markers = markers;
     L.capped = capped; L.n_ovf = capped ? n_ovf : 0;
@@ -591,6 +604,7 @@
     if (pl->d_alias) (void)hipFree(pl->d_alias);
     if (pl->d_canon) (void)hipFree(pl->d_canon);
     if (pl->d_dirrec) (void)hipFree(pl->d_dirrec);
+    if (pl->d_dirrec32) (void)hipFree(pl->d_dirrec32);
     {
         auto& F = pl->fused;
         for (void* q : {(void*)F.d_row_s, (void*)F.d_w, (void*)F.d_i, (void*)F.d_meta, (void*)F.d_dirrec})
@@ -633,6 +647,20 @@
     if (!pl || k < 0 || k >= (int)pl->lat.size() || pl->lat[k].stride <= 0) return 0;
     if (overflow_rows) *overflow_rows = pl->lat[k].n_ovf;
     return pl->lat[k].stride;
+}
+
+int vet_plan_record_bytes(const vet_plan* pl) {
+    if (!pl || pl->lat.empty()) return 0;
+    if (pl->lat[0].stride <= 0 || !pl->d_dirrec) return pl->fused.state == 1 && pl->fused.d_dirrec ? 8 : 0;
+    return vh::use_rec32(pl) ? 4 : 8;
+}
+
+int vet_plan_read_records(vet_plan* pl, uint32_t* h_rec32) {
+    if (!pl || !h_rec32) return fail(VET_ERR_INVALID, "plan or output is NULL");
+    if (!pl->d_dirrec32) return fail(VET_ERR_INVALID, "the plan has no compact record table");
+    HIP_TRY(hipSetDevice(pl->ctx->device));
+    HIP_TRY(hipMemcpy(h_rec32, pl->d_dirrec32, (size_t)pl->n_dirs * 4, hipMemcpyDeviceToHost));
+    return VET_OK;
 }
 
 int vet_plan_read_table(vet_plan* pl, int k, uint32_t* h_w, uint16_t* h_tile, uint32_t* h_meta, uint32_t* h_ovf_w,
diff --git a/viewport-entropy-toolkit_amd/csrc/vet_spatial.hip b/viewport-entropy-toolkit_amd/csrc/vet_spatial.hip
--- a/viewport-entropy-toolkit_amd/csrc/vet_spatial.hip
+++ b/viewport-entropy-toolkit_amd/csrc/vet_spatial.hip
@@ -104,9 +104,12 @@
 }
 
 template <bool FROM_IDS>
-const void* lut_kernel(bool il, bool occ8, bool dedup, bool fpt = false, int nb = 0) {
+const void* lut_kernel(bool il, bool occ8, bool dedup, bool fpt = false, int nb = 0, bool rec32 = false) {
     if (nb) {
-        if (!il || !occ8 || fpt) return nullptr;
+        if (!il || !occ8 || fpt || (rec32 && !dedup)) return nullptr;
+#define VET_PICKR(N) if (rec32 && nb == N) return (const void*)vet::k_spatial_lut<FROM_IDS, 2, true, true, true, false, false, N, true>
+        VET_PICKR(1); VET_PICKR(2); VET_PICKR(3);
+#undef VET_PICKR
 #define VET_PICKC(N, D) if (nb == N && dedup == D) return (const void*)vet::k_spatial_lut<FROM_IDS, 2, true, true, D, false, false, N>
         VET_PICKC(1, false); VET_PICKC(1, true); VET_PICKC(2, false); VET_PICKC(2, true); VET_PICKC(3, false); VET_PICKC(3, true);
 #undef VET_PICKC
@@ -248,6 +251,7 @@
     q.nearest = pl->lat[lat_idx[0]].d_nearest;
     q.alias = pl->d_alias;
     q.dirrec = pl->d_dirrec;
+    q.dirrec32 = pl->d_dirrec32;
     q.rec_meta = lat_idx[0] == 0 ? 1 : 0;
     q.K = K; q.n_sum = 0;
     bool il = false;
@@ -269,6 +273,8 @@
     q.entropy = d_entropy; q.assign = d_assign; q.weights = d_weights; q.present = d_present;
     q.status = d_status;
     const bool dedup = dedup_lattices(pl, d_videos ? batch_max_users : U);
+    const bool rec32 = nb && dedup && use_rec32(pl);
+    static_assert(2048 <= vet::REC32_MAX_CHUNK, "a chunk's multiplicities fit the walk word");
     int blocks = blocks_batch;
     const int threads = 256;
     size_t lds = lds_batch;
@@ -279,7 +285,7 @@
         int fpw = lut_frames_per_wg(U, T, c->n_cu, q.n_sum);
         for (;; fpw /= 2) {
             lds = vet::lut_lds_bytes(U, q.UC, fpw, q.n_sum, dedup, d_resolve != nullptr, fpt ? threads / 64 : 1, q.sort_words,
-                                     nb ? vet::lut_ovf_slots(q.UC, L0.n_ovf, dedup) : 0);
+                                     nb ? vet::lut_ovf_slots(q.UC, L0.n_ovf, dedup) : 0, rec32);
             if (lds <= c->lds_max || fpw == 1) break;
         }
         if (lds > c->lds_max) return VET_OK;
@@ -291,7 +297,7 @@
     }
     ProfScope ps(c, s, KID_SPATIAL);
     void* args[] = {(void*)&q};
-    const void* fn = lut_kernel<FROM_IDS>(il, occ8 && !fpt, dedup, fpt, nb);
+    const void* fn = lut_kernel<FROM_IDS>(il, occ8 && !fpt, dedup, fpt, nb, rec32);
     if (!fn) return fail(VET_ERR_UNSUPPORTED, "no table kernel for this launch");
     HIP_TRY(hipLaunchKernel(fn, dim3((unsigned)blocks), dim3(threads), args, lds, s));
     HIP_TRY(hipGetLastError());
@@ -376,12 +382,12 @@
 }
 
 size_t batch_video_geometry(const vet_ctx* c, int U, long total_frames, int n_sum, bool dedup, int* fpw_out, int* uc_out,
-                            int priv = 1, int sort_words = 0, int n_ovf = 0) {
+                            int priv = 1, int sort_words = 0, int n_ovf = 0, bool rec32 = false) {
     const int UC = U < 2048 ? U : 2048;
     int fpw = lut_frames_per_wg(U, total_frames, c->n_cu, n_sum);
     size_t lds = 0;
     for (;; fpw /= 2) {
-        lds = vet::lut_lds_bytes(U, UC, fpw, n_sum, dedup, false, priv, sort_words, vet::lut_ovf_slots(UC, n_ovf, dedup));
+        lds = vet::lut_lds_bytes(U, UC, fpw, n_sum, dedup, false, priv, sort_words, vet::lut_ovf_slots(UC, n_ovf, dedup), rec32);
         if (lds <= c->lds_max || fpw == 1) break;
     }
     *fpw_out = fpw; *uc_out = UC;
@@ -983,7 +989,8 @@
             d.entropy = x.d_entropy; d.assign = x.d_assign; d.present = x.d_present;
             const size_t lds = batch_video_geometry(c, d.U, total_frames, n_sum, dedup, &d.FPW, &d.UC, form0 == F_FTABLE ? 4 : 1,
                                                     (form0 == F_FTABLE && dedup && 2 * pl->n_rows <= 65536) ? (int)((2 * pl->n_rows + 31) / 32) : 0,
-                                                    pl->lat[0].capped ? pl->lat[0].n_ovf : 0);
+                                                    pl->lat[0].capped ? pl->lat[0].n_ovf : 0,
+                                                    pl->lat[0].capped && dedup && use_rec32(pl));
             if (lds == 0) table = false;
             d.block0 = block; d.pad_ = 0;
             block += (d.T + d.FPW - 1) / d.FPW;
diff --git a/viewport-entropy-toolkit_amd/csrc/vet_spatial_lut.hpp b/viewport-entropy-toolkit_amd/csrc/vet_spatial_lut.hpp
--- a/viewport-entropy-toolkit_amd/csrc/vet_spatial_lut.hpp
+++ b/viewport-entropy-toolkit_amd/csrc/vet_spatial_lut.hpp
@@ -53,7 +53,7 @@
                            __HIP_MEMORY_SCOPE_WORKGROUP);
 }
 
-template <int UN, bool INTERLEAVED, bool DEDUP, bool FPT, int GSL_IL = 4, int NB = 0>
+template <int UN, bool INTERLEAVED, bool DEDUP, bool FPT, int GSL_IL = 4, int NB = 0, bool REC32 = false>
 __device__ __forceinline__ void walk_rows(const uint32_t* frows, const uint32_t* fmeta, int nu,
                                           unsigned long long* hrow, int n,
                                           const uint32_t* __restrict__ tab_w, const uint16_t* __restrict__ tab_i,
@@ -62,6 +62,7 @@
     const int NW = blockDim.x >> 6, lane = lane_id(), wv = wave_id();
     if constexpr (NB > 0) {
         static_assert(!FPT && INTERLEAVED && GSL_IL == 4, "capped rows: integer tables with 16-lane rows");
+        static_assert(!REC32 || DEDUP, "the one-word row list belongs to the kernels with the set");
         constexpr int UPW = WAVE >> 4;
         int lane_here = lane;
         asm volatile("" : "+v"(lane_here));
@@ -73,13 +74,23 @@
             for (int k = 0; k < UN; ++k) {
                 const int j = j0 + k * step + sub;
                 const bool on = j < nu;
-                const uint32_t pk = on ? frows[j] : 0u, m = on ? fmeta[j] : 0u;
-                const uint32_t key = DEDUP ? pk >> 12 : pk;
-                const bool flip = ((DEDUP ? key >> ROW_BITS : key >> 31) & 1u) != 0u;
-                const uint32_t rid = DEDUP ? key & ROW_MASK : key & 0x7FFFFFFFu;
-                row[k] = (on ? rid * (uint32_t)(NB * ROW_BLOCK) : zero_row) + (uint32_t)(4 * sl);
-                const uint32_t cnt = DEDUP ? pk & 0xFFFu : (on ? 1u : 0u);
-                mult[k] = cnt << ((m >> 16) & 0x1Fu);
+                bool flip;
+                if constexpr (REC32) {
+                    const uint32_t pk = on ? frows[j] : 0u;
+                    flip = (int)pk < 0;
+                    const uint32_t rid = (pk >> WALK32_ROW_POS) & REC32_ROW_MASK;
+                    row[k] = (on ? rid * (uint32_t)(NB * ROW_BLOCK) : zero_row) + (uint32_t)(4 * sl);
+                    const uint32_t cnt = on ? ((pk >> WALK32_CNT_POS) & ((1u << WALK32_CNT_BITS) - 1)) + 1u : 0u;
+                    mult[k] = cnt << (pk & 0x1Fu);
+                } else {
+                    const uint32_t pk = on ? frows[j] : 0u, m = on ? fmeta[j] : 0u;
+                    const uint32_t key = DEDUP ? pk >> 12 : pk;
+                    flip = ((DEDUP ? key >> ROW_BITS : key >> 31) & 1u) != 0u;
+                    const uint32_t rid = DEDUP ? key & ROW_MASK : key & 0x7FFFFFFFu;
+                    row[k] = (on ? rid * (uint32_t)(NB * ROW_BLOCK) : zero_row) + (uint32_t)(4 * sl);
+                    const uint32_t cnt = DEDUP ? pk & 0xFFFu : (on ? 1u : 0u);
+                    mult[k] = cnt << ((m >> 16) & 0x1Fu);
+                }
                 sgn[k] = flip ? -8 : 8;
                 hb32[k] = (uint32_t)(size_t)(__attribute__((address_space(3))) char*)((char*)hrow + (flip ? (n - 1) * 8 : 0));
             }
@@ -227,6 +238,7 @@
     unsigned long long* timeline;
     unsigned long long* dbg;
     uint32_t* resolve;
+    const uint32_t* dirrec32;
 };
 
 template <class V>
@@ -318,6 +330,11 @@
     }
 }
 
+__device__ __forceinline__ uint32_t walk32_single(uint32_t key, uint32_t aux) {
+    return (key << WALK32_ROW_POS) | ((uint32_t)TAB_X - ((aux >> REC32_SHIFT_POS) & ((1u << REC32_SHIFT_BITS) - 1))) |
+           ((aux & REC32_OVERFLOW) ? WALK32_OVF_TMP : 0u);
+}
+
 __host__ __device__ __forceinline__ int lut_hash_slots(int UC) {
     int hs = 64;
     while (hs < 2 * UC) hs <<= 1;
@@ -325,17 +342,19 @@
 }
 __host__ __device__ __forceinline__ int lut_marked_words(int n_sum) { return (n_sum + 31) >> 5; }
 __host__ __device__ __forceinline__ size_t lut_lds_bytes(int U, int UC, int FPW, int n_sum, bool dedup, bool marked = false,
-                                                         int priv = 1, int sort_words = 0, int ovf_slots = 0) {
+                                                         int priv = 1, int sort_words = 0, int ovf_slots = 0, bool rec32 = false) {
     const size_t hist = (size_t)FPW * n_sum * 8 * priv, hash = dedup ? (size_t)FPW * lut_hash_slots(UC) * 4 : 0;
     const size_t srt = sort_words ? ((size_t)sort_words + 256) * 4 : 0;
     size_t a = (dedup && U <= UC) ? (hist > hash ? hist : hash) : hist + hash;
     if (dedup && U <= UC && srt > a) a = srt;
-    return ((a + 15) & ~(size_t)15) + (size_t)FPW * UC * 8 + (size_t)2 * FPW * 4 + 64 +
-           (marked ? (size_t)FPW * lut_marked_words(n_sum) * 4 : 0) + (ovf_slots ? (size_t)FPW * (4 + (size_t)ovf_slots * 8) : 0);
-}
-
-template <bool FROM_IDS, int UN, bool IL, bool OCC8, bool DEDUP, bool FPT, bool FUSED = false, int NB = 0>
+    const size_t per_row = rec32 ? 4 : 8;
+    return ((a + 15) & ~(size_t)15) + (size_t)FPW * UC * per_row + (size_t)2 * FPW * 4 + 64 +
+           (marked ? (size_t)FPW * lut_marked_words(n_sum) * 4 : 0) + (ovf_slots ? (size_t)FPW * (4 + (size_t)ovf_slots * per_row) : 0);
+}
+
+template <bool FROM_IDS, int UN, bool IL, bool OCC8, bool DEDUP, bool FPT, bool FUSED = false, int NB = 0, bool REC32 = false>
 __global__ __launch_bounds__(256, OCC8 ? 8 : (FPT ? 6 : 7)) void k_spatial_lut(const LutParams p) {
+    static_assert(!REC32 || (NB > 0 && DEDUP && !FPT && !FUSED), "the compact record serves the capped kernels with the set");
     extern __shared__ __attribute__((aligned(16))) unsigned char smem[];
     SampleSrc src = p.src;
     int U = p.U, T = p.T, FPW = p.FPW, UC = p.UC;
@@ -368,7 +387,7 @@
     uint32_t* hash = (uint32_t*)(smem + (overlay ? 0 : hist_bytes));
     uint32_t* rows = (uint32_t*)(smem + ((a_bytes + 15) & ~(size_t)15));
     uint32_t* meta = rows + (size_t)FPW * UC;
-    int* cnt_chunk = (int*)(meta + (size_t)FPW * UC);
+    int* cnt_chunk = (int*)(meta + (REC32 ? (size_t)0 : (size_t)FPW * UC));
     int* cnt_frame = cnt_chunk + FPW;
     const int MW = lut_marked_words(p.n_sum);
     uint32_t* marked = (FPT && p.resolve) ? (uint32_t*)(cnt_frame + FPW) : nullptr;
@@ -378,6 +397,12 @@
         if (!(m & META_OVERFLOW)) return;
         const int OC = ovf_slots();
         uint32_t* ovf_rows = (uint32_t*)(ovf_cnt + FPW);
+        if constexpr (REC32) {
+            const uint32_t o = p.lat[0].ovf_of_row[(word >> WALK32_ROW_POS) & REC32_ROW_MASK];
+            const int pos = atomicAdd(&ovf_cnt[fl], 1);
+            if (pos < OC) ovf_rows[(size_t)fl * OC + pos] = (word & ~(REC32_ROW_MASK << WALK32_ROW_POS)) | (o << WALK32_ROW_POS);
+            return;
+        }
         const uint32_t o = p.lat[0].ovf_of_row[DEDUP ? (word >> 12) & ROW_MASK : word & 0x7FFFFFFFu];
         const int pos = atomicAdd(&ovf_cnt[fl], 1);
         if (pos < OC) {
@@ -468,7 +493,12 @@
             for (int k = 0; k < SPT; ++k) {
                 row[k] = 0u; near[k] = -1; m0[k] = 0u;
                 if (id[k] >= 0) {
-                    if (DEDUP) {
+                    if constexpr (REC32) {
+                        const uint32_t rec = p.dirrec32[id[k]];
+                        row[k] = rec & REC32_KEY_MASK;
+                        near[k] = (int)((rec >> REC32_TILE_POS) & ((1u << REC32_TILE_BITS) - 1));
+                        m0[k] = rec & REC32_AUX_MASK;
+                    } else if (DEDUP) {
                         const uint2 rec = p.dirrec[id[k]];
                         row[k] = (rec.x & ROW_MASK) | ((rec.x >> 31) << ROW_BITS);
                         near[k] = (int)(((rec.x >> ROW_BITS) & 0xFFFu) | ((rec.y >> 28) << 12));
@@ -525,15 +555,23 @@
                     base = __builtin_amdgcn_readfirstlane(base);
                     if (won) {
                         const size_t pos = (size_t)fl0 * UC + base + below(mw);
-                        rows[pos] = merge ? h : (DEDUP ? (row[k] << 12) | 1u : row[k]);
-                        meta[pos] = m0[k];
+                        if constexpr (REC32) {
+                            rows[pos] = merge ? h | m0[k] : walk32_single(row[k], m0[k]);
+                        } else {
+                            rows[pos] = merge ? h : (DEDUP ? (row[k] << 12) | 1u : row[k]);
+                            meta[pos] = m0[k];
+                        }
                     }
                 } else {
                     if (valid) atomicAdd(&cnt_frame[fl], 1);
                     if (won) {
                         const size_t pos = (size_t)fl * UC + atomicAdd(&cnt_chunk[fl], 1);
-                        rows[pos] = merge ? h : (DEDUP ? (row[k] << 12) | 1u : row[k]);
-                        meta[pos] = m0[k];
+                        if constexpr (REC32) {
+                            rows[pos] = merge ? h | m0[k] : walk32_single(row[k], m0[k]);
+                        } else {
+                            rows[pos] = merge ? h : (DEDUP ? (row[k] << 12) | 1u : row[k]);
+                            meta[pos] = m0[k];
+                        }
                     }
                 }
             }
@@ -545,6 +583,15 @@
             if (merge)
                 for (int i = tid; i < nf * UC; i += blockDim.x) {
                     const int fl = i / UC, j = i - fl * UC;
+                    if constexpr (REC32) {
+                        if (j < cnt_chunk[fl]) {
+                            const uint32_t r = rows[i], slot = hash[(size_t)fl * HS + (r & ~REC32_AUX_MASK)];
+                            const uint32_t word = ((slot >> 12) << WALK32_ROW_POS) | (((slot & 0xFFFu) - 1u) << WALK32_CNT_POS) |
+                                                  ((uint32_t)TAB_X - ((r >> REC32_SHIFT_POS) & ((1u << REC32_SHIFT_BITS) - 1)));
+                            rows[i] = word;
+                            if (r & REC32_OVERFLOW) note_overflow(fl, word, META_OVERFLOW);
+                        }
+                    } else
                     if (j < cnt_chunk[fl]) {
                         const uint32_t word = hash[(size_t)fl * HS + rows[i]];
                         rows[i] = word;
@@ -640,7 +687,7 @@
         for (int k = 0; k < p.K; ++k) {
             const LutLattice& L = p.lat[k];
             if (k) __syncthreads();
-            if (!(k == 0 && p.rec_meta && (DEDUP || p.dirrec)))
+            if (!REC32 && !(k == 0 && p.rec_meta && (DEDUP || p.dirrec)))
                 for (int i = tid; i < nf * UC; i += blockDim.x) {
                     const int fl = i / UC, j = i - fl * UC;
                     if (j < cnt_chunk[fl]) meta[i] = L.tab_meta[DEDUP ? (rows[i] >> 12) & ROW_MASK : rows[i] & 0x7FFFFFFFu];
@@ -648,6 +695,13 @@
             if (NB && !merge)
                 for (int i = tid; i < nf * UC; i += blockDim.x) {
                     const int fl = i / UC, j = i - fl * UC;
+                    if constexpr (REC32) {
+                        if (j < cnt_chunk[fl] && (rows[i] & WALK32_OVF_TMP)) {
+                            const uint32_t word = rows[i] & ~WALK32_OVF_TMP;
+                            rows[i] = word;
+                            note_overflow(fl, word, META_OVERFLOW);
+                        }
+                    } else
                     if (j < cnt_chunk[fl]) note_overflow(fl, rows[i], meta[i]);
                 }
             __syncthreads();
@@ -655,11 +709,11 @@
             for (int fl = 0; fl < nf; ++fl)
                 if constexpr (NB > 0) {
                     unsigned long long* hrow = hist + (size_t)fl * p.n_sum + hoff;
-                    walk_rows<UN, true, DEDUP, false, 4, NB>(rows + (size_t)fl * UC, meta + (size_t)fl * UC, cnt_chunk[fl], hrow, L.n,
+                    walk_rows<UN, true, DEDUP, false, 4, NB, REC32>(rows + (size_t)fl * UC, meta + (size_t)fl * UC, cnt_chunk[fl], hrow, L.n,
                                                              L.tab_w, L.tab_i, L.stride, 4, L.zrow * (uint32_t)(NB * ROW_BLOCK));
                     if (const int OC = ovf_slots()) {
                         const uint32_t* ovf_rows = (const uint32_t*)(ovf_cnt + FPW);
-                        walk_rows<UN, true, DEDUP, false, 4, 1>(ovf_rows + (size_t)fl * OC, ovf_rows + (size_t)(FPW + fl) * OC,
+                        walk_rows<UN, true, DEDUP, false, 4, 1, REC32>(ovf_rows + (size_t)fl * OC, ovf_rows + (size_t)(FPW + fl) * OC,
                                                                 min(ovf_cnt[fl], OC), hrow, L.n, L.ovf_w, L.ovf_i, ROW_BLOCK, 4,
                                                                 (uint32_t)L.n_ovf * (uint32_t)ROW_BLOCK);
                     }
diff --git a/viewport-entropy-toolkit_amd/csrc/vet_weight_table.hpp b/viewport-entropy-toolkit_amd/csrc/vet_weight_table.hpp
--- a/viewport-entropy-toolkit_amd/csrc/vet_weight_table.hpp
+++ b/viewport-entropy-toolkit_amd/csrc/vet_weight_table.hpp
@@ -332,4 +332,15 @@
     }
 }
 
-}
+__global__ void k_dirrec32(const uint32_t* __restrict__ alias, const uint16_t* __restrict__ nearest,
+                           const uint32_t* __restrict__ meta0, long D, uint32_t* __restrict__ rec, int* __restrict__ unfit) {
+    for (long d = blockIdx.x * (long)blockDim.x + threadIdx.x; d < D; d += (long)gridDim.x * blockDim.x) {
+        const uint32_t a = alias[d], near = nearest[d], row = a & 0x7FFFFFFFu;
+        const uint32_t m = row <= REC32_ROW_MASK ? meta0[row] : 0u, left = m >> 16;
+        if (row > REC32_ROW_MASK || near >= (1u << REC32_TILE_BITS) || left > (uint32_t)TAB_X) { atomicAdd(unfit, 1); continue; }
+        rec[d] = row | ((a >> 31) << REC32_ROW_BITS) | (near << REC32_TILE_POS) | (((uint32_t)TAB_X - left) << REC32_SHIFT_POS) |
+                 ((m & META_OVERFLOW) ? REC32_OVERFLOW : 0u);
+    }
+}
+
+}
diff --git a/viewport-entropy-toolkit_amd/viewport_entropy_toolkit/_native.py b/viewport-entropy-toolkit_amd/viewport_entropy_toolkit/_native.py
--- a/viewport-entropy-toolkit_amd/viewport_entropy_toolkit/_native.py
+++ b/viewport-entropy-toolkit_amd/viewport_entropy_toolkit/_native.py
@@ -68,6 +68,7 @@
     "vet_device_pci_bus_id": (_I, [_P, C.c_char_p, _I]),
     "vet_profile_enable": (_I, [_P, _I]),
     "vet_test_no_row_cap": (_I, [_P, _I]),
+    "vet_test_rec8": (_I, [_P, _I]),
     "vet_profile_reset": (_I, [_P]),
     "vet_profile_get": (_I, [_P, _I, C.POINTER(_D), C.POINTER(_I64)]),
     "vet_kernel_name": (C.c_char_p, [_I]),
@@ -84,6 +85,8 @@
     "vet_plan_table_stride": (_I, [_P, _I]),
     "vet_plan_table_rows": (_I64, [_P]),
     "vet_plan_table_cap": (_I, [_P, _I, C.POINTER(_I64)]),
+    "vet_plan_record_bytes": (_I, [_P]),
+    "vet_plan_read_records": (_I, [_P, _P]),
     "vet_plan_last_formulation": (_I, [_P, _I]),
     "vet_plan_error_bounds": (_I, [_P, _I, C.POINTER(_D), C.POINTER(_D)]),
     "vet_plan_read_dirs": (_I, [_P, _P]),
@@ -296,6 +299,9 @@
 
     def test_no_row_cap(self, on: bool = True):
         _check(self.lib, self.lib.vet_test_no_row_cap(self.handle, int(on)))
+
+    def test_rec8(self, on: bool = True):
+        _check(self.lib, self.lib.vet_test_rec8(self.handle, int(on)))
 
     def profile_enable(self, on: bool = True):
         _check(self.lib, self.lib.vet_profile_enable(self.handle, int(on)))
@@ -418,6 +424,14 @@
         n = C.c_int64()
         return int(self.lib.vet_plan_table_cap(self.handle, lattice, C.byref(n))), int(n.value)
 
+    def record_bytes(self) -> int:
+        return int(self.lib.vet_plan_record_bytes(self.handle))
+
+    def read_records(self) -> np.ndarray:
+        out = np.empty(self.n_dirs, dtype=np.uint32)
+        _check(self.lib, self.lib.vet_plan_read_records(self.handle, _ptr(out)))
+        return out
+
     def last_formulation(self, lattice: int = 0) -> str:
         return FORMULATIONS.get(int(self.lib.vet_plan_last_formulation(self.handle, lattice)), "")
 
```

New measurement: 30.05 billion samples/s, median of 6. 1.8% higher.
